# baurst/rbrt

Hardware: AMD Instinct MI355X
Metric: Mray-samples/sec (WxHxspp/s) on bunny scene; achieved HBM GB/s vs peak (higher is better)
Workload: dtype f32; 1 GPU; example_scene.yaml, 69451-triangle stand-in mesh, 1024x768, 50 spp, seed 1; parallelism=pixel tiles 8x8 dealt round-robin along skew lines over 1 GPU(s)

## Files before the change

include/rbrt_hip_debug.h:

```cpp
#ifndef RBRT_HIP_DEBUG_H
#define RBRT_HIP_DEBUG_H

#include "rbrt_hip.h"

#ifdef __cplusplus
extern "C" {
#endif

int rbrt_hip_scene_last_batching(rbrt_hip_scene_t* scene, uint32_t* samples_per_batch, uint32_t* n_batches);

int rbrt_hip_scene_adaptive_rounds(rbrt_hip_scene_t* scene, uint32_t* active_tiles, size_t n, uint32_t* n_rounds);

#define RBRT_DENOISE_TILE 16u

#define RBRT_GUIDED_TILE 16u
#define RBRT_GUIDED_STAGED_MAX_STEP 4u
int rbrt_hip_debug_guided_staging(int max_step);

#define RBRT_TEMPORAL_BLOCK 256u

#define RBRT_UPSAMPLE_TILE_W 32u
#define RBRT_UPSAMPLE_TILE_H 8u

#define RBRT_DESPIKE_TILE_W 32u
#define RBRT_DESPIKE_TILE_H 8u

#define RBRT_TONEMAP_BLOCK_PIXELS 1024u
#define RBRT_TONEMAP_MAX_BLOCKS 512u

#define RBRT_GLARE_TILE_W 16u
#define RBRT_GLARE_TILE_H 16u

int rbrt_hip_trace_rays(rbrt_hip_scene_t* scene, const float* rays, size_t n, float min_dist,
                        float max_dist, float* out_t, int32_t* out_obj, int32_t* out_tri,
                        float* out_dist);

int rbrt_hip_selftest_gate(const float lo[3], const float hi[3], const float* rays, size_t n, uint8_t* out_fast,
                           uint8_t* out_exact);

int rbrt_hip_selftest_ieee(uint64_t seed, size_t n, uint64_t counts[3]);

int rbrt_hip_debug_ieee(const float* x, size_t n, const float* v, size_t m, float* out_sqrt, uint8_t* out_sqrt_short,
                        float* out_norm, uint8_t* out_norm_short);

int rbrt_hip_selftest_sqrt_sweep(uint32_t first_bits, uint64_t n, uint64_t counts[3]);

int rbrt_hip_scene_debug_counters(rbrt_hip_scene_t* scene, uint64_t* out, size_t n);

int rbrt_hip_scene_debug_set_counter(rbrt_hip_scene_t* scene, size_t index, uint64_t value);

int rbrt_hip_bvh_build_host(const rbrt_mesh_t* mesh, void** nodes_out, size_t* n_nodes, void** tris_out,
                            size_t* n_tris, uint32_t* max_depth, float* max_e12);
void rbrt_hip_free_host(void* p);
int rbrt_hip_bvh_build_host_records(const void* records, size_t n, void** nodes_out, size_t* n_nodes, void** tris_out,
                                    size_t* n_tris, uint32_t* max_depth, float* max_e12);
int rbrt_hip_bvh_build_device(const rbrt_mesh_t* mesh, void** nodes_out, size_t* n_nodes, void** tris_out,
                              size_t* n_tris, uint32_t* max_depth, float* max_e12, int* built);

int rbrt_hip_debug_scatter(const rbrt_material_t* mats, const float* in_dir, const float* p, const float* normal,
                           const uint32_t* rng_state, size_t n, float* out_dir, uint8_t* out_ok, uint32_t* out_rng_state);

int rbrt_hip_debug_primary_cull(rbrt_hip_scene_t* scene, const rbrt_camera_t* cam, uint32_t* out_words, size_t n_words);
int rbrt_hip_debug_primary_cull_lens(rbrt_hip_scene_t* scene, const rbrt_camera_lens_t* lens, uint32_t* out_words, size_t n_words);
int rbrt_hip_debug_primary_cull_shutter(rbrt_hip_scene_t* scene, const rbrt_camera_t* cam, const rbrt_camera_lens_t* lens,
                                        const float travel[3], uint32_t* out_words, size_t n_words);
int rbrt_hip_debug_primary_cull_opts(rbrt_hip_scene_t* scene, const rbrt_camera_t* cam, const rbrt_render_opts_t* opts,
                                     uint32_t* out_words, size_t n_words);

int rbrt_hip_debug_shading_normals(rbrt_hip_scene_t* scene, const float* rays, size_t n, float min_dist, float max_dist,
                                   float* out_normal);

int rbrt_hip_debug_surface_albedo(rbrt_hip_scene_t* scene, const float* rays, size_t n, float min_dist, float max_dist,
                                  float* out_albedo);

int rbrt_hip_debug_environment(rbrt_hip_scene_t* scene, const float* dirs, size_t n, float* out_rgb);

int rbrt_hip_scene_set_timing(rbrt_hip_scene_t* scene, int enable);
int rbrt_hip_scene_kernel_ms(rbrt_hip_scene_t* scene, float* trace_ms_total, float* resolve_ms_total,
                             uint32_t* n_trace_launches);

int rbrt_hip_scene_launch_mix(rbrt_hip_scene_t* scene, uint32_t* n_full_grid, uint32_t* n_half_grid);

int rbrt_hip_scene_helper_launches(rbrt_hip_scene_t* scene, uint32_t* n);

int rbrt_hip_scene_set_short_paths(rbrt_hip_scene_t* scene, int mode);
int rbrt_hip_debug_short_masks(rbrt_hip_scene_t* scene, uint64_t* out_masks, size_t n, size_t* n_chunks);

typedef struct rbrt_hip_call_times {
    double hip_init_s;
    double upload_s;
    double bvh_build_s;
    double lanes_s;
    double create_s;
    double render_s;
    double copy_s;
    double destroy_s;
    double total_s;
    uint32_t meshes_device_built, meshes_host_built;
} rbrt_hip_call_times_t;
int rbrt_hip_scene_create_times(rbrt_hip_scene_t* scene, rbrt_hip_call_times_t* out);
int rbrt_hip_last_render_times(rbrt_hip_call_times_t* out);

int rbrt_hip_scene_refine_wait(rbrt_hip_scene_t* scene, double timeout_s, int* state, double* build_seconds);

#ifdef __cplusplus
}
#endif
#endif
```

rbrt_amd/__init__.py:

```python
from __future__ import annotations

import ctypes as C

import numpy as np

from . import abi
from .abi import (Camera, CameraLens, Material, RenderOpts, RbrtError, SceneData, MeshData, default_opts, load_hip,
                  material, MAT_DIELECTRIC, MAT_LAMBERTIAN, MAT_METAL)

__all__ = ["render_scene", "HipScene", "abi", "device_count"]


def device_count() -> int:
    return int(load_hip().rbrt_hip_device_count())


def _cam_arg(cam: abi.Camera, lens, opts: abi.RenderOpts):
    if lens is None:
        return C.byref(cam), cam
    if isinstance(lens, abi.CameraLens):
        lens = (tuple(lens.lens_u), tuple(lens.lens_v), lens.focus_scale)
    L = abi.camera_lens(cam, *lens)
    opts.flags |= abi.FLAG_THIN_LENS
    return C.byref(L.cam), L
# ... 19 lines not shown
    return rad, rgb


def _shading_ptr(scene):
    f = getattr(scene, "shading_ptr", None)
    return f() if f is not None else None


def _patterns_ptr(scene):
    f = getattr(scene, "patterns_ptr", None)
    return f() if f is not None else None


def last_render_times() -> dict:
    t = abi.CallTimes()
    abi.check(load_hip().rbrt_hip_last_render_times(C.byref(t)))
    return t.as_dict()


class HipScene:

    def __init__(self, scene: abi.SceneData, device: int = 0):
        self._lib = load_hip()
        self._h = C.c_void_p()
        self.device = device
        self.scene = scene
        shading, patterns = _shading_ptr(scene), _patterns_ptr(scene)
        if patterns is not None:
            abi.check(self._lib.rbrt_hip_scene_create_patterned(scene.ptr(), shading, patterns, device, C.byref(self._h)))
        elif shading is None:
            abi.check(self._lib.rbrt_hip_scene_create(scene.ptr(), device, C.byref(self._h)))
        else:
            abi.check(self._lib.rbrt_hip_scene_create_shaded(scene.ptr(), shading, device, C.byref(self._h)))

    def close(self):
        if self._h:
            self._lib.rbrt_hip_scene_destroy(self._h)
            self._h = C.c_void_p()

    def __del__(self):
        try:
            self.close()
        except Exception:
            pass

    def __enter__(self):
        return self

    def __exit__(self, *a):
        self.close()

    def render_device(self, cam: abi.Camera, opts: abi.RenderOpts, d_radiance: int | None, d_rgb8: int | None = None,
                      stream: int | None = None, lens=None):
        opts = _opts_copy(opts)
        cam_p, _keep = _cam_arg(cam, lens, opts)
        abi.check(self._lib.rbrt_hip_render_device(self._h, cam_p, C.byref(opts), C.c_void_p(stream or 0),
                                                   C.c_void_p(d_radiance or 0), C.c_void_p(d_rgb8 or 0)))

    def render_pass(self, cam: abi.Camera, opts: abi.RenderOpts, sample_begin: int, sample_end: int, d_accum: int,
                    d_radiance: int | None = None, d_rgb8: int | None = None, stream: int | None = None, lens=None):
        opts = _opts_copy(opts)
        cam_p, _keep = _cam_arg(cam, lens, opts)
        abi.check(self._lib.rbrt_hip_render_pass(self._h, cam_p, C.byref(opts), C.c_void_p(stream or 0), sample_begin,
                                                 sample_end, C.c_void_p(d_accum), C.c_void_p(d_radiance or 0),
                                                 C.c_void_p(d_rgb8 or 0)))

    def render_adaptive(self, cam: abi.Camera, opts: abi.RenderOpts, threshold: float, min_samples: int = 16, step: int = 64,
                        d_radiance: int | None = None, d_rgb8: int | None = None, d_tile_samples: int | None = None,
                        d_tile_error: int | None = None, stream: int | None = None, lens=None, reserved: int = 0) -> dict:
        opts = _opts_copy(opts)
        cam_p, _keep = _cam_arg(cam, lens, opts)
        a = abi.AdaptiveOpts(float(threshold), int(min_samples), int(step), int(reserved))
        res = abi.AdaptiveResult()
        abi.check(self._lib.rbrt_hip_render_adaptive(self._h, cam_p, C.byref(opts), C.byref(a), C.c_void_p(stream or 0),
                                                     C.c_void_p(d_radiance or 0), C.c_void_p(d_rgb8 or 0),
                                                     C.c_void_p(d_tile_samples or 0), C.c_void_p(d_tile_error or 0), C.byref(res)))
        return dict(rounds=int(res.rounds), samples=int(res.samples), samples_fixed=int(res.samples_fixed))

    def adaptive_rounds(self) -> list:
        n = C.c_uint32()
        abi.check(self._lib.rbrt_hip_scene_adaptive_rounds(self._h, None, 0, C.byref(n)))
        buf = (C.c_uint32 * max(n.value, 1))()
        abi.check(self._lib.rbrt_hip_scene_adaptive_rounds(self._h, buf, n.value, C.byref(n)))
        return [int(buf[i]) for i in range(n.value)]

    def denoise(self, d_radiance: int | None = None, d_rgb8: int | None = None, d_half_a: int | None = None,
                d_half_b: int | None = None, window_radius: int | None = None, patch_radius: int | None = None,
                strength: float | None = None, stream: int | None = None, reserved: int = 0):
        d = denoise_opts(window_radius, patch_radius, strength, reserved)
        abi.check(self._lib.rbrt_hip_scene_denoise(self._h, C.byref(d), C.c_void_p(stream or 0), C.c_void_p(d_radiance or 0),
                                                   C.c_void_p(d_rgb8 or 0), C.c_void_p(d_half_a or 0), C.c_void_p(d_half_b or 0)))

    def denoise_guided(self, d_albedo: int, d_normal: int, d_depth: int, d_coverage: int, d_workspace: int,
                       d_radiance: int | None = None, d_rgb8: int | None = None, opts: abi.GuidedOpts | None = None,
                       stream: int | None = None):
        g = opts if opts is not None else guided_opts()
        abi.check(self._lib.rbrt_hip_scene_denoise_guided(self._h, C.byref(g), C.c_void_p(stream or 0), C.c_void_p(d_albedo or 0),
                                                          C.c_void_p(d_normal or 0), C.c_void_p(d_depth or 0), C.c_void_p(d_coverage or 0),
                                                          C.c_void_p(d_workspace or 0), C.c_void_p(d_radiance or 0), C.c_void_p(d_rgb8 or 0)))

    def render_features(self, cam: abi.Camera, opts: abi.RenderOpts, samples: int | None = None, d_albedo: int | None = None,
                        d_normal: int | None = None, d_depth: int | None = None, d_coverage: int | None = None,
                        d_object: int | None = None, lens=None, stream: int | None = None, reserved=(0, 0, 0)):
        opts = _opts_copy(opts)
        cam_p, _keep = _cam_arg(cam, lens, opts)
        f = feature_opts(samples, reserved)
        abi.check(self._lib.rbrt_hip_render_features(self._h, cam_p, C.byref(opts), C.byref(f), C.c_void_p(stream or 0),
                                                     C.c_void_p(d_albedo or 0), C.c_void_p(d_normal or 0), C.c_void_p(d_depth or 0),
                                                     C.c_void_p(d_coverage or 0), C.c_void_p(d_object or 0)))

    def set_environment(self, nodes, *, n: int | None = None, reserved: int = 0):
        if nodes is None and n is None:
            abi.check(self._lib.rbrt_hip_scene_set_environment(self._h, None))
            return
        env = abi.Environment()
        if nodes is not None:
            nodes = np.ascontiguousarray(nodes, np.float32)
            if n is None:
                if nodes.ndim != 3 or nodes.shape[0] != nodes.shape[1] or nodes.shape[2] != 3 or nodes.shape[0] < 2:
                    raise ValueError("set_environment: nodes must have shape (N + 1, N + 1, 3)")
                n = nodes.shape[0] - 1
            env.nodes = abi.fptr(nodes)
        env.n, env.reserved = int(n), int(reserved)
        abi.check(self._lib.rbrt_hip_scene_set_environment(self._h, C.byref(env)))

    def set_shutter(self, travel, *, reserved: int = 0):
        if travel is None:
            abi.check(self._lib.rbrt_hip_scene_set_shutter(self._h, None))
            return
        sh = abi.Shutter()
        sh.travel[:] = [float(np.float32(v)) for v in travel]
        sh.reserved = int(reserved)
        abi.check(self._lib.rbrt_hip_scene_set_shutter(self._h, C.byref(sh)))

    def environment_lookup(self, dirs):
        dirs = np.ascontiguousarray(dirs, np.float32).reshape(-1, 3)
        out = np.zeros((dirs.shape[0], 3), np.float32)
        abi.check(self._lib.rbrt_hip_debug_environment(self._h, abi.fptr(dirs), dirs.shape[0], abi.fptr(out)))
        return out

    def set_pipeline(self, depth: int):
        abi.check(self._lib.rbrt_hip_scene_set_pipeline(self._h, int(depth)))

    def set_short_paths(self, mode: int = 1):
        abi.check(self._lib.rbrt_hip_scene_set_short_paths(self._h, int(mode)))

    def short_masks(self):
        n = C.c_size_t()
        abi.check(self._lib.rbrt_hip_debug_short_masks(self._h, None, 0, C.byref(n)))
        out = np.zeros(n.value, np.uint64)
        if n.value:
            abi.check(self._lib.rbrt_hip_debug_short_masks(self._h, out.ctypes.data_as(C.POINTER(C.c_uint64)), n.value, C.byref(n)))
        return out

    def set_timing(self, on: bool = True):
        abi.check(self._lib.rbrt_hip_scene_set_timing(self._h, int(on)))

    def kernel_ms(self):
        t, r, n = C.c_float(), C.c_float(), C.c_uint32()
        abi.check(self._lib.rbrt_hip_scene_kernel_ms(self._h, C.byref(t), C.byref(r), C.byref(n)))
        return t.value, r.value, n.value

    def launch_mix(self):
        a, b = C.c_uint32(), C.c_uint32()
        abi.check(self._lib.rbrt_hip_scene_launch_mix(self._h, C.byref(a), C.byref(b)))
        return a.value, b.value

    def helper_launches(self) -> int:
        n = C.c_uint32()
        abi.check(self._lib.rbrt_hip_scene_helper_launches(self._h, C.byref(n)))
        return n.value

    def create_times(self) -> dict:
        t = abi.CallTimes()
        abi.check(self._lib.rbrt_hip_scene_create_times(self._h, C.byref(t)))
        return t.as_dict()

    def refine_wait(self, timeout_s: float = 60.0):
        st, sec = C.c_int(), C.c_double()
        abi.check(self._lib.rbrt_hip_scene_refine_wait(self._h, float(timeout_s), C.byref(st), C.byref(sec)))
        return st.value, sec.value

    def info(self) -> dict:
        i = abi.SceneInfo()
        abi.check(self._lib.rbrt_hip_scene_info(self._h, C.byref(i)))
        return {k: int(getattr(i, k)) for k, _ in abi.SceneInfo._fields_}

    def check(self):
        abi.check(self._lib.rbrt_hip_scene_check(self._h))

    def last_batches(self):
        b, n = C.c_uint32(), C.c_uint32()
        abi.check(self._lib.rbrt_hip_scene_last_batching(self._h, C.byref(b), C.byref(n)))
        return b.value, n.value

    def stats(self) -> dict:
        st = abi.Stats()
        abi.check(self._lib.rbrt_hip_scene_stats(self._h, C.byref(st)))
        return {k: int(getattr(st, k)) for k, _ in abi.Stats._fields_}

    def set_debug_counter(self, index: int, value: int):
        abi.check(self._lib.rbrt_hip_scene_debug_set_counter(self._h, int(index), int(value)))

    def raw_debug_counters(self) -> list:
        buf = (C.c_uint64 * 64)()
        abi.check(self._lib.rbrt_hip_scene_debug_counters(self._h, buf, 64))
        return [int(x) for x in buf]

    def debug_counters(self) -> dict:
        buf = (C.c_uint64 * 64)()
        abi.check(self._lib.rbrt_hip_scene_debug_counters(self._h, buf, 64))
        names = ("empty", "trav", "term", "lamb", "metal", "diel")
        d = {f"passes_{n}": int(buf[i]) for i, n in enumerate(names)}
        d.update({f"slots_{n}": int(buf[6 + i]) for i, n in enumerate(names)})
        d.update(trav_wave_steps=int(buf[12]), trav_lane_steps=int(buf[13]), refill_rounds=int(buf[14]),
                 sched_rounds=int(buf[15]), cycles_trav=int(buf[16]), cycles_shade=int(buf[17]),
                 cycles_total=int(buf[18]), leaf_rounds=int(buf[19]), leaf_lanes=int(buf[20]),
                 walk_rounds=int(buf[21]), walk_lanes=int(buf[22]), shading_pass_free_lanes=int(buf[23]),
                 rt_first_start=int(buf[24]), rt_last_workout=int(buf[25]), rt_last_end=int(buf[26]),
                 rt_sum_wave_time=int(buf[27]), rt_first_workout=int(buf[28]),
                 path_len_hist=[int(buf[32 + i]) for i in range(8)],
                 long_path_objects=[int(buf[40 + i]) for i in range(8)],
                 long_path_total=int(buf[48]), long_path_dielectric=int(buf[47]), shade_extra_rounds=int(buf[29]),
                 drain_slowest=dict(us=int(buf[50]) >> 44, rounds=(int(buf[50]) >> 32) & 0xFFF,
                                    trav_steps=(int(buf[50]) >> 16) & 0xFFFF, passes=int(buf[50]) & 0xFFFF),
                 drain_sum=dict(rounds=int(buf[51]), trav_steps=int(buf[52]), passes=int(buf[53]),
                                lane_steps=int(buf[54])),
                 stack_pushes_beyond_lds=int(buf[30]), stack_deepest=int(buf[31]),
                 parked_at_burst_entry=int(buf[55]), fullest_shading_kind_at_burst_entry=int(buf[56]),
                 shared_entries_given=int(buf[59]), share_rounds=int(buf[60]), traversals_ending_at_root=int(buf[61]),
                 sphere_tail_runs=int(buf[62]), sphere_tail_lanes=int(buf[63]),
                 mixed_pass_8=dict(passes=int(buf[49]) >> 32, lanes=int(buf[49]) & 0xFFFFFFFF),
                 mixed_pass_16=dict(passes=int(buf[58]) >> 32, lanes=int(buf[58]) & 0xFFFFFFFF))
        return d

    def primary_cull(self, cam, opts=None, lens=None):
        tx, ty = (cam.img_width_pix + 7) // 8, (cam.img_height_pix + 7) // 8
        out = np.zeros(tx * ty, np.uint32)
        words = out.ctypes.data_as(C.POINTER(C.c_uint32))
        if opts is None and lens is None:
            abi.check(self._lib.rbrt_hip_debug_primary_cull(self._h, C.byref(cam), words, out.size))
        else:
            opts = _opts_copy(opts if opts is not None else abi.default_opts())
            cam_p, _keep = _cam_arg(cam, lens, opts)
            abi.check(self._lib.rbrt_hip_debug_primary_cull_opts(self._h, cam_p, C.byref(opts), words, out.size))
        return out.reshape(ty, tx)

    def primary_cull_lens(self, cam, lens):
        if not isinstance(lens, abi.CameraLens):
            lens = abi.camera_lens(cam, *lens)
        else:
            lens = abi.camera_lens(cam, tuple(lens.lens_u), tuple(lens.lens_v), lens.focus_scale)
        tx, ty = (cam.img_width_pix + 7) // 8, (cam.img_height_pix + 7) // 8
        out = np.zeros(tx * ty, np.uint32)
        abi.check(self._lib.rbrt_hip_debug_primary_cull_lens(self._h, C.byref(lens), out.ctypes.data_as(C.POINTER(C.c_uint32)),
                                                             out.size))
        return out.reshape(ty, tx)

    def primary_cull_shutter(self, cam, lens, travel):
        if lens is not None:
            if not isinstance(lens, abi.CameraLens):
                lens = abi.camera_lens(cam, *lens)
            else:
                lens = abi.camera_lens(cam, tuple(lens.lens_u), tuple(lens.lens_v), lens.focus_scale)
        tv = (C.c_float * 3)(*[float(np.float32(v)) for v in travel])
        tx, ty = (cam.img_width_pix + 7) // 8, (cam.img_height_pix + 7) // 8
        out = np.zeros(tx * ty, np.uint32)
        abi.check(self._lib.rbrt_hip_debug_primary_cull_shutter(self._h, C.byref(cam), C.byref(lens) if lens is not None else None, tv,
                                                                out.ctypes.data_as(C.POINTER(C.c_uint32)), out.size))
        return out.reshape(ty, tx)

    def surface_albedo(self, rays, min_dist=0.001, max_dist=2000.0):
        rays = np.ascontiguousarray(rays, np.float32).reshape(-1, 6)
        out = np.zeros((rays.shape[0], 3), np.float32)
        abi.check(self._lib.rbrt_hip_debug_surface_albedo(self._h, rays.ctypes.data_as(abi.f32p), rays.shape[0], min_dist,
                                                          max_dist, out.ctypes.data_as(abi.f32p)))
        return out

    def shading_normals(self, rays, min_dist=0.001, max_dist=2000.0):
        rays = np.ascontiguousarray(rays, np.float32).reshape(-1, 6)
        out = np.zeros((rays.shape[0], 3), np.float32)
        abi.check(self._lib.rbrt_hip_debug_shading_normals(self._h, rays.ctypes.data_as(abi.f32p), rays.shape[0], min_dist,
                                                           max_dist, out.ctypes.data_as(abi.f32p)))
        return out

    def trace_rays(self, rays, min_dist=0.001, max_dist=2000.0):
        rays = np.ascontiguousarray(rays, np.float32).reshape(-1, 6)
        n = rays.shape[0]
        t = np.zeros(n, np.float32)
        dist = np.zeros(n, np.float32)
        obj = np.zeros(n, np.int32)
        tri = np.zeros(n, np.int32)
        abi.check(self._lib.rbrt_hip_trace_rays(self._h, rays.ctypes.data_as(abi.f32p), n, min_dist, max_dist,
                                                t.ctypes.data_as(abi.f32p), obj.ctypes.data_as(abi.i32p),
                                                tri.ctypes.data_as(abi.i32p), dist.ctypes.data_as(abi.f32p)))
        return t, obj, tri, dist


def _opts_copy(opts: abi.RenderOpts) -> abi.RenderOpts:
    o = abi.RenderOpts()
    C.memmove(C.byref(o), C.byref(opts), C.sizeof(o))
    return o


def supported_flags() -> int:
    return int(load_hip().rbrt_hip_supported_flags())
# ... 249 lines not shown
```

rbrt_amd/abi.py:

```python
from __future__ import annotations

import ctypes as C
import os
from pathlib import Path

import numpy as np

ROOT = Path(__file__).resolve().parent.parent
LIB_HIP = ROOT / "rbrt_amd" / "lib" / "librbrt_hip.so"
LIB_HOST = ROOT / "rbrt_amd" / "lib" / "librbrt_host.so"

RBRT_OK = 0
RBRT_ERR_INVALID_ARG = -1
RBRT_ERR_NO_DEVICE = -2
RBRT_ERR_HIP = -3
RBRT_ERR_OOM = -4
RBRT_ERR_UNSUPPORTED = -5
RBRT_ERR_NAN = -6

MAT_LAMBERTIAN = 0
MAT_METAL = 1
MAT_DIELECTRIC = 2
MAT_EMISSIVE = 3

# ... 100 lines not shown
    _fields_ = [
        ("position", C.c_float * 3),
        ("right", C.c_float * 3),
        ("up", C.c_float * 3),
        ("img_center_point", C.c_float * 3),
        ("mm_per_pix_hor", C.c_float),
        ("mm_per_pix_vert", C.c_float),
        ("img_width_pix", C.c_uint32),
        ("img_height_pix", C.c_uint32),
    ]


class CameraLens(C.Structure):
    _fields_ = [
        ("cam", Camera),
        ("lens_u", C.c_float * 3),
        ("lens_v", C.c_float * 3),
        ("focus_scale", C.c_float),
        ("reserved", C.c_uint32),
    ]


def camera_lens(cam: Camera, lens_u, lens_v, focus_scale: float) -> CameraLens:
    L = CameraLens()
    C.memmove(C.byref(L.cam), C.byref(cam), C.sizeof(Camera))
    L.lens_u = _f3(lens_u)
    L.lens_v = _f3(lens_v)
    L.focus_scale = float(focus_scale)
    L.reserved = 0
    return L


class RenderOpts(C.Structure):
    _fields_ = [
        ("spp", C.c_uint32),
        ("max_depth", C.c_uint32),
        ("min_dist", C.c_float),
        ("max_dist", C.c_float),
        ("bg", C.c_float * 3),
        ("seed", C.c_uint64),
        ("tile_rank", C.c_uint32),
        ("tile_world", C.c_uint32),
        ("flags", C.c_uint32),
        ("reserved", C.c_uint32),
    ]


class AdaptiveOpts(C.Structure):
    _fields_ = [("threshold", C.c_float), ("min_samples", C.c_uint32), ("step", C.c_uint32), ("reserved", C.c_uint32)]


class AdaptiveResult(C.Structure):
    _fields_ = [("rounds", C.c_uint32), ("reserved", C.c_uint32), ("samples", C.c_uint64), ("samples_fixed", C.c_uint64)]


class DenoiseOpts(C.Structure):
    _fields_ = [("window_radius", C.c_uint32), ("patch_radius", C.c_uint32), ("strength", C.c_float), ("reserved", C.c_uint32)]


class TonemapOpts(C.Structure):
    _fields_ = [("curve", C.c_uint32), ("exposure", C.c_float), ("key", C.c_float), ("key_permille", C.c_uint32),
                ("white", C.c_float), ("white_permille", C.c_uint32), ("reserved", C.c_uint32 * 2)]


class TonemapResult(C.Structure):
    _fields_ = [("exposure", C.c_float), ("white", C.c_float), ("l_key", C.c_float), ("l_white", C.c_float),
                ("counted", C.c_uint32), ("reserved", C.c_uint32), ("pixels", C.c_uint64)]


class GlareOpts(C.Structure):
    _fields_ = [("threshold", C.c_float), ("intensity", C.c_float), ("levels", C.c_uint32), ("spread", C.c_float),
                ("reserved", C.c_uint32 * 4)]


class FeatureOpts(C.Structure):
    _fields_ = [("samples", C.c_uint32), ("reserved", C.c_uint32 * 3)]


class GuidedOpts(C.Structure):
    _fields_ = [("levels", C.c_uint32), ("colour", C.c_float), ("normal", C.c_float), ("depth", C.c_float), ("albedo", C.c_float),
                ("flags", C.c_uint32), ("reserved", C.c_uint32 * 2)]


class TemporalOpts(C.Structure):
    _fields_ = [("max_history", C.c_float), ("depth", C.c_float), ("normal", C.c_float), ("flags", C.c_uint32),
                ("reserved", C.c_uint32 * 4)]


class UpsampleOpts(C.Structure):
    _fields_ = [("factor", C.c_uint32), ("normal", C.c_float), ("depth", C.c_float), ("albedo", C.c_float), ("flags", C.c_uint32),
                ("reserved", C.c_uint32 * 3)]


class DespikeOpts(C.Structure):
    _fields_ = [("radius", C.c_uint32), ("rank", C.c_uint32), ("threshold", C.c_float), ("floor", C.c_float), ("flags", C.c_uint32),
                ("reserved", C.c_uint32 * 3)]


class DespikeResult(C.Structure):
    _fields_ = [("spikes_a", C.c_uint32), ("spikes_b", C.c_uint32), ("reserved", C.c_uint32 * 2)]


class CompareOpts(C.Structure):
    _fields_ = [("epsilon", C.c_float), ("flags", C.c_uint32), ("reserved", C.c_uint32 * 2)]


class CompareResult(C.Structure):
    _fields_ = [("sum_se", C.c_double), ("sum_ae", C.c_double), ("sum_rel", C.c_double), ("sum_ssim", C.c_double), ("max_abs", C.c_float),
                ("usable", C.c_uint32), ("skipped", C.c_uint32), ("reserved", C.c_uint32 * 5)]


class CompareSummary(C.Structure):
    _fields_ = [("mse", C.c_double), ("mae", C.c_double), ("relmse", C.c_double), ("psnr_db", C.c_double), ("ssim", C.c_double)]


class Environment(C.Structure):
    _fields_ = [("n", C.c_uint32), ("reserved", C.c_uint32), ("nodes", f32p)]


class Shutter(C.Structure):
    _fields_ = [("travel", C.c_float * 3), ("reserved", C.c_uint32)]


class Stats(C.Structure):
    _fields_ = [
        ("rays", C.c_uint64),
        ("mesh_gate_pass", C.c_uint64),
        ("nodes_visited", C.c_uint64),
        ("tris_tested", C.c_uint64),
        ("mesh_hits", C.c_uint64),
        ("samples", C.c_uint64),
        ("nan_discriminants", C.c_uint64),
        ("node_bytes", C.c_uint32),
        ("tri_bytes", C.c_uint32),
    ]


class SceneInfo(C.Structure):
    _fields_ = [
        ("n_spheres", C.c_uint32), ("n_meshes", C.c_uint32),
        ("n_meshes_device_built", C.c_uint32), ("bvh_stack_need", C.c_uint32),
        ("n_nodes", C.c_uint64), ("n_triangles", C.c_uint64),
        ("trace_waves", C.c_uint32), ("lds_bytes_per_wave", C.c_uint32),
        ("occupancy_api_waves_per_cu", C.c_uint32), ("n_cus", C.c_uint32),
    ]


class CallTimes(C.Structure):
    _fields_ = [(k, C.c_double) for k in ("hip_init_s", "upload_s", "bvh_build_s", "lanes_s", "create_s", "render_s", "copy_s",
                                          "destroy_s", "total_s")] + [("meshes_device_built", C.c_uint32), ("meshes_host_built", C.c_uint32)]

    def as_dict(self) -> dict:
        return {k: getattr(self, k) for k, _ in self._fields_}


HIP_SYMBOLS = {
    "rbrt_hip_render": (C.c_int, [C.POINTER(Camera), C.POINTER(Scene), C.POINTER(RenderOpts), f32p, u8p]),
    "rbrt_hip_scene_create": (C.c_int, [C.POINTER(Scene), C.c_int, C.POINTER(C.c_void_p)]),
    "rbrt_hip_scene_destroy": (C.c_int, [C.c_void_p]),
    "rbrt_hip_packed_pixels": (C.c_size_t, [C.c_uint32, C.c_uint32, C.c_uint32, C.c_uint32]),
    "rbrt_hip_tile_xy": (None, [C.c_uint32, C.c_uint32, C.POINTER(C.c_uint32), C.POINTER(C.c_uint32)]),
    "rbrt_hip_tile_number": (C.c_uint32, [C.c_uint32, C.c_uint32, C.c_uint32]),
    "rbrt_hip_render_device": (C.c_int, [C.c_void_p, C.POINTER(Camera), C.POINTER(RenderOpts), C.c_void_p,
                                         C.c_void_p, C.c_void_p]),
    "rbrt_hip_render_pass": (C.c_int, [C.c_void_p, C.POINTER(Camera), C.POINTER(RenderOpts), C.c_void_p, C.c_uint32, C.c_uint32,
                                       C.c_void_p, C.c_void_p, C.c_void_p]),
    "rbrt_hip_unpack_tiles": (C.c_int, [C.c_int, C.c_void_p, C.c_void_p, C.c_uint32, C.c_uint32, C.c_uint32,
                                        C.c_void_p, C.c_void_p]),
    "rbrt_hip_unpack_tiles_strided": (C.c_int, [C.c_int, C.c_void_p, C.c_void_p, C.c_uint32, C.c_uint32, C.c_uint32,
                                                C.c_size_t, C.c_void_p, C.c_void_p]),
    "rbrt_hip_scene_stats": (C.c_int, [C.c_void_p, C.POINTER(Stats)]),
    "rbrt_hip_scene_check": (C.c_int, [C.c_void_p]),
    "rbrt_render_opts_default": (None, [C.POINTER(RenderOpts)]),
    "rbrt_hip_device_count": (C.c_int, []),
    "rbrt_hip_last_error": (C.c_char_p, []),
    "rbrt_hip_abi_version": (C.c_int, []),
    "rbrt_hip_scene_set_pipeline": (C.c_int, [C.c_void_p, C.c_uint32]),
    "rbrt_hip_scene_info": (C.c_int, [C.c_void_p, C.POINTER(SceneInfo)]),
    "rbrt_hip_supported_flags": (C.c_uint32, []),
    "rbrt_hip_scene_create_shaded": (C.c_int, [C.POINTER(Scene), C.POINTER(SceneShading), C.c_int, C.POINTER(C.c_void_p)]),
    "rbrt_hip_scene_create_patterned": (C.c_int, [C.POINTER(Scene), C.POINTER(SceneShading), C.POINTER(ScenePatterns), C.c_int,
                                                  C.POINTER(C.c_void_p)]),
    "rbrt_hip_render_patterned": (C.c_int, [C.POINTER(Camera), C.POINTER(Scene), C.POINTER(SceneShading), C.POINTER(ScenePatterns),
                                            C.POINTER(RenderOpts), f32p, u8p]),
    "rbrt_hip_render_shaded": (C.c_int, [C.POINTER(Camera), C.POINTER(Scene), C.POINTER(SceneShading), C.POINTER(RenderOpts),
                                         f32p, u8p]),
    "rbrt_hip_render_adaptive": (C.c_int, [C.c_void_p, C.POINTER(Camera), C.POINTER(RenderOpts), C.POINTER(AdaptiveOpts), C.c_void_p,
                                           C.c_void_p, C.c_void_p, C.c_void_p, C.c_void_p, C.POINTER(AdaptiveResult)]),
    "rbrt_denoise_opts_default": (None, [C.POINTER(DenoiseOpts)]),
    "rbrt_hip_denoise_halves": (C.c_int, [C.c_int, C.c_void_p, C.c_void_p, C.c_void_p, C.c_void_p, C.c_uint32, C.c_uint32,
                                          C.POINTER(DenoiseOpts), C.c_void_p, C.c_void_p]),
    "rbrt_tonemap_opts_default": (None, [C.POINTER(TonemapOpts)]),
    "rbrt_hip_tonemap": (C.c_int, [C.c_int, C.c_void_p, C.c_void_p, C.c_size_t, C.POINTER(TonemapOpts), C.c_void_p, C.c_void_p,
                                   C.c_void_p]),
    "rbrt_glare_opts_default": (None, [C.POINTER(GlareOpts)]),
    "rbrt_hip_glare_workspace_bytes": (C.c_size_t, [C.c_uint32, C.c_uint32, C.c_uint32]),
    "rbrt_hip_glare": (C.c_int, [C.c_int, C.c_void_p, C.c_void_p, C.c_uint32, C.c_uint32, C.POINTER(GlareOpts), C.c_void_p, C.c_void_p,
                                 C.c_void_p]),
    "rbrt_hip_scene_denoise": (C.c_int, [C.c_void_p, C.POINTER(DenoiseOpts), C.c_void_p, C.c_void_p, C.c_void_p, C.c_void_p, C.c_void_p]),
    "rbrt_hip_scene_set_environment": (C.c_int, [C.c_void_p, C.POINTER(Environment)]),
    "rbrt_hip_scene_set_shutter": (C.c_int, [C.c_void_p, C.POINTER(Shutter)]),
    "rbrt_feature_opts_default": (None, [C.POINTER(FeatureOpts)]),
    "rbrt_hip_render_features": (C.c_int, [C.c_void_p, C.POINTER(Camera), C.POINTER(RenderOpts), C.POINTER(FeatureOpts), C.c_void_p,
                                           C.c_void_p, C.c_void_p, C.c_void_p, C.c_void_p, C.c_void_p]),
    "rbrt_guided_opts_default": (None, [C.POINTER(GuidedOpts)]),
    "rbrt_hip_guided_workspace_bytes": (C.c_size_t, [C.c_uint32, C.c_uint32]),
    "rbrt_hip_denoise_guided": (C.c_int, [C.c_int, C.c_void_p, C.c_void_p, C.c_void_p, C.c_void_p, C.c_void_p, C.c_void_p, C.c_void_p,
                                          C.c_void_p, C.c_uint32, C.c_uint32, C.POINTER(GuidedOpts), C.c_void_p, C.c_void_p, C.c_void_p]),
    "rbrt_hip_scene_denoise_guided": (C.c_int, [C.c_void_p, C.POINTER(GuidedOpts), C.c_void_p, C.c_void_p, C.c_void_p, C.c_void_p,
                                                C.c_void_p, C.c_void_p, C.c_void_p, C.c_void_p]),
    "rbrt_temporal_opts_default": (None, [C.POINTER(TemporalOpts)]),
    "rbrt_hip_temporal_history_bytes": (C.c_size_t, [C.c_uint32, C.c_uint32]),
    "rbrt_hip_temporal_accumulate": (C.c_int, [C.c_int, C.c_void_p, C.c_void_p, C.c_void_p, C.c_void_p, C.c_void_p, C.c_void_p,
                                               C.POINTER(Camera), C.POINTER(Camera), C.POINTER(TemporalOpts), C.c_void_p, C.c_void_p,
                                               C.c_void_p, C.c_void_p, C.c_void_p]),
    "rbrt_upsample_opts_default": (None, [C.POINTER(UpsampleOpts)]),
    "rbrt_hip_upsample_camera": (C.c_int, [C.POINTER(Camera), C.c_uint32, C.POINTER(Camera)]),
    "rbrt_hip_upsample_workspace_bytes": (C.c_size_t, [C.c_uint32, C.c_uint32, C.c_uint32]),
    "rbrt_hip_upsample_halves": (C.c_int, [C.c_int, C.c_void_p, C.c_void_p, C.c_void_p, C.c_void_p, C.c_void_p, C.c_void_p, C.c_void_p,
                                           C.c_void_p, C.c_uint32, C.c_uint32, C.POINTER(UpsampleOpts), C.c_void_p, C.c_void_p, C.c_void_p,
                                           C.c_void_p]),
    "rbrt_despike_opts_default": (None, [C.POINTER(DespikeOpts)]),
    "rbrt_hip_despike_halves": (C.c_int, [C.c_int, C.c_void_p, C.c_void_p, C.c_void_p, C.c_uint32, C.c_uint32, C.POINTER(DespikeOpts), C.c_void_p,
                                          C.c_void_p, C.c_void_p, C.c_void_p]),
    "rbrt_compare_opts_default": (None, [C.POINTER(CompareOpts)]),
    "rbrt_hip_compare_workspace_bytes": (C.c_size_t, [C.c_uint32, C.c_uint32]),
    "rbrt_hip_compare_images": (C.c_int, [C.c_int, C.c_void_p, C.c_void_p, C.c_void_p, C.c_uint32, C.c_uint32, C.POINTER(CompareOpts), C.c_void_p,
                                          C.c_void_p, C.c_void_p, C.c_void_p]),
    "rbrt_compare_summary": (None, [C.POINTER(CompareResult), C.c_uint32, C.c_uint32, C.c_double, C.POINTER(CompareSummary)]),
}
DEBUG_SYMBOLS = {
    "rbrt_hip_debug_guided_staging": (C.c_int, [C.c_int]),
    "rbrt_hip_scene_last_batching": (C.c_int, [C.c_void_p, C.POINTER(C.c_uint32), C.POINTER(C.c_uint32)]),
    "rbrt_hip_trace_rays": (C.c_int, [C.c_void_p, f32p, C.c_size_t, C.c_float, C.c_float, f32p, i32p, i32p, f32p]),
    "rbrt_hip_selftest_ieee": (C.c_int, [C.c_uint64, C.c_size_t, C.POINTER(C.c_uint64)]),
    "rbrt_hip_debug_ieee": (C.c_int, [f32p, C.c_size_t, f32p, C.c_size_t, f32p, u8p, f32p, u8p]),
    "rbrt_hip_selftest_sqrt_sweep": (C.c_int, [C.c_uint32, C.c_uint64, C.POINTER(C.c_uint64)]),
    "rbrt_hip_selftest_gate": (C.c_int, [f32p, f32p, f32p, C.c_size_t, u8p, u8p]),
    "rbrt_hip_bvh_build_host": (C.c_int, [C.POINTER(Mesh), C.POINTER(C.c_void_p), C.POINTER(C.c_size_t),
                                          C.POINTER(C.c_void_p), C.POINTER(C.c_size_t), C.POINTER(C.c_uint32),
                                          f32p]),
    "rbrt_hip_free_host": (None, [C.c_void_p]),
    "rbrt_hip_bvh_build_host_records": (C.c_int, [C.c_void_p, C.c_size_t, C.POINTER(C.c_void_p), C.POINTER(C.c_size_t),
                                                  C.POINTER(C.c_void_p), C.POINTER(C.c_size_t), C.POINTER(C.c_uint32), f32p]),
    "rbrt_hip_bvh_build_device": (C.c_int, [C.POINTER(Mesh), C.POINTER(C.c_void_p), C.POINTER(C.c_size_t),
                                            C.POINTER(C.c_void_p), C.POINTER(C.c_size_t), C.POINTER(C.c_uint32),
                                            f32p, C.POINTER(C.c_int)]),
    "rbrt_hip_scene_debug_counters": (C.c_int, [C.c_void_p, C.POINTER(C.c_uint64), C.c_size_t]),
    "rbrt_hip_scene_set_timing": (C.c_int, [C.c_void_p, C.c_int]),
    "rbrt_hip_scene_kernel_ms": (C.c_int, [C.c_void_p, f32p, f32p, C.POINTER(C.c_uint32)]),
    "rbrt_hip_scene_debug_set_counter": (C.c_int, [C.c_void_p, C.c_size_t, C.c_uint64]),
    "rbrt_hip_scene_launch_mix": (C.c_int, [C.c_void_p, C.POINTER(C.c_uint32), C.POINTER(C.c_uint32)]),
    "rbrt_hip_debug_scatter": (C.c_int, [C.POINTER(Material), f32p, f32p, f32p, C.POINTER(C.c_uint32), C.c_size_t, f32p, u8p,
                                        C.POINTER(C.c_uint32)]),
    "rbrt_hip_debug_primary_cull": (C.c_int, [C.c_void_p, C.POINTER(Camera), C.POINTER(C.c_uint32), C.c_size_t]),
    "rbrt_hip_debug_primary_cull_lens": (C.c_int, [C.c_void_p, C.POINTER(CameraLens), C.POINTER(C.c_uint32), C.c_size_t]),
    "rbrt_hip_debug_primary_cull_shutter": (C.c_int, [C.c_void_p, C.POINTER(Camera), C.POINTER(CameraLens), C.POINTER(C.c_float),
                                                      C.POINTER(C.c_uint32), C.c_size_t]),
    "rbrt_hip_debug_primary_cull_opts": (C.c_int, [C.c_void_p, C.POINTER(Camera), C.POINTER(RenderOpts), C.POINTER(C.c_uint32), C.c_size_t]),
    "rbrt_hip_scene_helper_launches": (C.c_int, [C.c_void_p, C.POINTER(C.c_uint32)]),
    "rbrt_hip_scene_create_times": (C.c_int, [C.c_void_p, C.POINTER(CallTimes)]),
    "rbrt_hip_last_render_times": (C.c_int, [C.POINTER(CallTimes)]),
    "rbrt_hip_scene_refine_wait": (C.c_int, [C.c_void_p, C.c_double, C.POINTER(C.c_int), C.POINTER(C.c_double)]),
    "rbrt_hip_debug_shading_normals": (C.c_int, [C.c_void_p, f32p, C.c_size_t, C.c_float, C.c_float, f32p]),
    "rbrt_hip_debug_surface_albedo": (C.c_int, [C.c_void_p, f32p, C.c_size_t, C.c_float, C.c_float, f32p]),
    "rbrt_hip_scene_adaptive_rounds": (C.c_int, [C.c_void_p, C.POINTER(C.c_uint32), C.c_size_t, C.POINTER(C.c_uint32)]),
    "rbrt_hip_debug_environment": (C.c_int, [C.c_void_p, f32p, C.c_size_t, f32p]),
    "rbrt_hip_scene_set_short_paths": (C.c_int, [C.c_void_p, C.c_int]),
    "rbrt_hip_debug_short_masks": (C.c_int, [C.c_void_p, C.POINTER(C.c_uint64), C.c_size_t, C.POINTER(C.c_size_t)]),
}


class RbrtError(RuntimeError):
    def __init__(self, code: int, msg: str):
        super().__init__(f"rbrt_hip error {code}: {msg}")
        self.code = code


_hip = None


def _preload_torch_hip_runtime() -> None:
    if os.environ.get("RBRT_NO_TORCH_PRELOAD"):
        return
    try:
        import importlib.util
        spec = importlib.util.find_spec("torch")
        if spec is None or not spec.origin:
            return
        cand = Path(spec.origin).parent / "lib" / "libamdhip64.so"
        if cand.exists():
            C.CDLL(str(cand), mode=getattr(os, "RTLD_GLOBAL", 0x100) | getattr(os, "RTLD_NOW", 2))
    except OSError:
        pass


def load_hip() -> C.CDLL:
    global _hip
    if _hip is not None:
        return _hip
    lib_path = Path(os.environ.get("RBRT_HIP_LIB", LIB_HIP))
    if not lib_path.exists():
        raise FileNotFoundError(
            f"{lib_path} is missing: build it with `make` (or __graft_entry__.build()). "
            "rbrt_amd has no CPU or pure-Python render path.")
    _preload_torch_hip_runtime()
    lib = C.CDLL(str(lib_path), mode=getattr(os, "RTLD_NOW", 2))
    for name, (res, args) in {**HIP_SYMBOLS, **DEBUG_SYMBOLS}.items():
        fn = getattr(lib, name)
        fn.restype = res
        fn.argtypes = args
    _hip = lib
    return lib


def check(code: int) -> None:
    if code != RBRT_OK:
        raise RbrtError(code, load_hip().rbrt_hip_last_error().decode(errors="replace"))



def _f3(v):
    return (C.c_float * 3)(*[float(x) for x in v])


def material(kind: int, albedo=(0.0, 0.0, 0.0), param: float = 0.0) -> Material:
    return Material(kind, _f3(albedo), float(param))


def fptr(a: np.ndarray):
    assert a.dtype == np.float32 and a.flags["C_CONTIGUOUS"]
    return a.ctypes.data_as(f32p)


class SceneData:

    def __init__(self, spheres=(), meshes=(), triangles=(), element_order=None, patterns=None):
        self.spheres = list(spheres)
        self.meshes = list(meshes)
        self.triangles = list(triangles)
        self.element_order = None if element_order is None else [int(x) for x in element_order]
        self._sph = (Sphere * max(1, len(self.spheres)))()
        for i, (c, r, m) in enumerate(self.spheres):
            self._sph[i] = Sphere(_f3(c), float(r), m)
        self._msh = (Mesh * max(1, len(self.meshes)))()
        for i, md in enumerate(self.meshes):
            self._msh[i] = md.struct
        self._tri = (Triangle * max(1, len(self.triangles)))()
        for i, (corners, m) in enumerate(self.triangles):
            for a in range(3):
                for b in range(3):
                    self._tri[i].corners[a][b] = float(corners[a][b])
            self._tri[i].mat = m
        self._order = None if self.element_order is None else (C.c_uint32 * len(self.element_order))(*self.element_order)
        self.struct = Scene(len(self.spheres), self._sph, len(self.meshes), self._msh, len(self.triangles), self._tri,
                            self._order if self._order is not None else C.POINTER(C.c_uint32)())
        self._nrm = (MeshNormals * max(1, len(self.meshes)))()
        for i, md in enumerate(self.meshes):
            if md.normals is not None:
                self._nrm[i] = md.normals_struct
        self.shading = (SceneShading(len(self.meshes), 0, self._nrm)
                        if any(md.normals is not None for md in self.meshes) else None)
        self.pattern_of = dict(patterns or {})
        n_obj = len(self.spheres) + len(self.triangles) + len(self.meshes)
        self._pat = (Pattern * max(1, n_obj))()
        for k, p in self.pattern_of.items():
            self._pat[int(k)] = p
        self.patterns = ScenePatterns(n_obj, 0, self._pat) if self.pattern_of else None

    def ptr(self):
        return C.byref(self.struct)

    def shading_ptr(self):
        return None if self.shading is None else C.byref(self.shading)

    def patterns_ptr(self):
        return None if self.patterns is None else C.byref(self.patterns)


class MeshData:

    FIELDS = ("v0x", "v0y", "v0z", "e1x", "e1y", "e1z", "e2x", "e2y", "e2z", "nx", "ny", "nz")

    def __init__(self, arrays: dict, is_padding: np.ndarray, n_real: int, bbox_lo, bbox_hi, mat: Material, normals=None):
        self.arrays = {k: np.ascontiguousarray(arrays[k], dtype=np.float32) for k in self.FIELDS}
        self.is_padding = np.ascontiguousarray(is_padding, dtype=np.uint8)
        n_total = len(self.is_padding)
        for k in self.FIELDS:
            assert len(self.arrays[k]) == n_total, k
        self.n_total, self.n_real = n_total, int(n_real)
        self.bbox_lo, self.bbox_hi = np.float32(bbox_lo), np.float32(bbox_hi)
        self.struct = Mesh()
        self.struct.n_total = n_total
        self.struct.n_real = self.n_real
        for k in self.FIELDS:
            setattr(self.struct, k, fptr(self.arrays[k]))
        self.struct.is_padding = self.is_padding.ctypes.data_as(u8p)
        self.struct.bbox_lo = _f3(bbox_lo)
        self.struct.bbox_hi = _f3(bbox_hi)
        self.struct.mat = mat
        self.normals = None
        self.normals_struct = MeshNormals()
        if normals is not None:
            self.normals = {k: np.ascontiguousarray(normals[k], dtype=np.float32) for k in NORMAL_FIELDS}
            for k in NORMAL_FIELDS:
                assert len(self.normals[k]) == n_total, k
                setattr(self.normals_struct, k, fptr(self.normals[k]))

    def with_normals(self, normals):
        return MeshData(self.arrays, self.is_padding, self.n_real, self.bbox_lo, self.bbox_hi, self.struct.mat, normals)


def default_opts(spp: int = 5, seed: int = 1, **kw) -> RenderOpts:
    o = RenderOpts()
    o.spp, o.max_depth, o.min_dist, o.max_dist = spp, 50, 0.001, 2000.0
    o.bg = _f3((0.05, 0.05, 0.8))
    o.seed, o.tile_rank, o.tile_world, o.flags, o.reserved = seed, 0, 1, 0, 0
    for k, v in kw.items():
        if k == "bg":
            o.bg = _f3(v)
        else:
            setattr(o, k, v)
# ... 202 lines not shown
```

rbrt_amd/csrc/api.cpp:

```cpp
#include <hip/hip_runtime_api.h>

#include <algorithm>
#include <chrono>
#include <cmath>
#include <cstdio>
#include <cstdlib>
#include <cstring>
#include <atomic>
#include <condition_variable>
#include <limits>
#include <memory>
#include <mutex>
#include <string>
#include <thread>
#include <vector>

#include "api_common.h"
#include "bvh.h"
#include "bvh_device.h"
#include "device_types.h"
#include "../../include/rbrt_hip_debug.h"

namespace rbrt {
hipError_t launch_trace_megakernel(const TraceParams& P, uint32_t n_waves, bool stats, hipStream_t stream);
hipError_t launch_trace_helper(const TraceParams& P, uint32_t n_waves, hipStream_t stream);
size_t megakernel_gseq_bytes(uint32_t n_waves);
size_t megakernel_gstack_bytes(uint32_t n_waves);
size_t megakernel_lds_bytes(uint32_t stack_entries, uint32_t n_spheres, uint32_t n_meshes, uint32_t n_elem_tris, uint32_t thin_lens,
                            uint32_t environment, uint32_t pattern_dw, uint32_t shutter);
int megakernel_occupancy_per_cu(size_t lds_bytes);
hipError_t launch_primary_cull(const TraceParams& P, hipStream_t stream);
hipError_t launch_sky_resolve(const TraceParams& P, const ResolveParams& R, hipStream_t stream);
hipError_t launch_short_paths(const TraceParams& P, uint32_t n_waves, hipStream_t stream);
hipError_t launch_code_load(hipStream_t stream);
hipError_t launch_resolve(const ResolveParams& R, hipStream_t stream);
hipError_t launch_resolve_even(const TraceParams& P, const ResolveParams& R, uint32_t n_active_tiles, hipStream_t stream);
hipError_t launch_adaptive_lists(const AdaptiveParams& A, hipStream_t stream);
hipError_t launch_tile_error(const AdaptiveParams& A, uint32_t n_active_tiles, hipStream_t stream);
hipError_t launch_adaptive_finish(const AdaptiveParams& A, hipStream_t stream);
hipError_t launch_denoise_halves(const DenoiseHalvesParams& Q, hipStream_t stream);
hipError_t launch_unpack(const float* gathered, uint32_t width, uint32_t height, uint32_t world,
                         size_t rank_stride_pixels, float* out_radiance, uint8_t* out_rgb8, hipStream_t stream);
hipError_t launch_trace_rays(const TraceParams& P, const float* rays, size_t n, float* out_t, int32_t* out_obj,
                             int32_t* out_tri, float* out_dist, hipStream_t stream);
hipError_t launch_shading_normals(const TraceParams& P, const float* rays, size_t n, float* out_normal, hipStream_t stream);
hipError_t launch_surface_albedo(const TraceParams& P, const float* rays, size_t n, float* out_albedo, hipStream_t stream);
hipError_t launch_environment_lookup(const EnvTexel* nodes, uint32_t n_env, const float* dirs, size_t n, float* out_rgb, hipStream_t stream);
hipError_t launch_features(const TraceParams& P, const FeatureParams& F, hipStream_t stream);
hipError_t launch_scatter_debug(const DevMaterial* d_mats, const float* d_in_dir, const float* d_p, const float* d_normal,
                                 const uint32_t* d_rng, size_t n, float* d_out_dir, uint8_t* d_out_ok, uint32_t* d_out_rng);
uint64_t host_splitmix64(uint64_t x);
}

using namespace rbrt;

namespace {
thread_local std::string g_last_error;
}

namespace rbrt {

int fail(int code, const std::string& msg) {
    g_last_error = msg;
    return code;
}

int hip_fail(hipError_t e, const std::string& what) {
    const int code = (e == hipErrorOutOfMemory) ? RBRT_ERR_OOM
                     : (e == hipErrorNoDevice || e == hipErrorInvalidDevice) ? RBRT_ERR_NO_DEVICE
                                                                             : RBRT_ERR_HIP;
    return fail(code, what + ": " + hipGetErrorString(e));
}

int hook_result(hipError_t e, const char* who) {
    return e == hipSuccess ? RBRT_OK : fail(RBRT_ERR_HIP, std::string(who) + ": " + hipGetErrorString(e));
}

int ensure_device(int device) {
    int n = 0;
    hipError_t e = hipGetDeviceCount(&n);
    if (e != hipSuccess || n <= 0)
        return fail(RBRT_ERR_NO_DEVICE, std::string("no HIP device available: ") +
                                            (e != hipSuccess ? hipGetErrorString(e) : "device count is 0"));
    if (device < 0 || device >= n) return fail(RBRT_ERR_INVALID_ARG, "device index out of range");
    HIP_TRY(hipSetDevice(device));
    return RBRT_OK;
}

}

namespace {

thread_local rbrt_hip_call_times_t g_last_render_times{};

const uint32_t g_hw_queues_at_load = [] {
    if (const char* q = std::getenv("GPU_MAX_HW_QUEUES")) {
        char* end = nullptr;
        const long v = std::strtol(q, &end, 10);
        if (end != q && *end == '\0' && v >= 1 && v <= 64) return uint32_t(v);
    }
    return 4u;
}();

double now_s() { return std::chrono::duration<double>(std::chrono::steady_clock::now().time_since_epoch()).count(); }

uint32_t local_tiles_of(uint32_t n_tiles, uint32_t rank, uint32_t world) {
    return rank < n_tiles ? (n_tiles - rank + world - 1u) / world : 0u;
}

const char* lab_env(const char* name) {
    const char* lab = std::getenv("RBRT_HIP_LAB");
    return (lab && lab[0] == '1') ? std::getenv(name) : nullptr;
}
bool lab_u32(const char* name, long long lo, long long hi, uint32_t& dst, std::string& err) {
    const char* e = lab_env(name);
    if (!e) return true;
    char* end = nullptr;
    const long long v = std::strtoll(e, &end, 10);
    if (end == e || *end != '\0' || v < lo || v > hi) {
        err = std::string("lab knob ") + name + "=" + e + " is not valid (see include/rbrt_hip_debug.h)";
        return false;
    }
    dst = uint32_t(v);
    return true;
}
bool lab_f32(const char* name, float lo, bool lo_open, float hi, float& dst, std::string& err) {
    const char* e = lab_env(name);
    if (!e) return true;
    char* end = nullptr;
    const float v = std::strtof(e, &end);
    if (end == e || *end != '\0' || !std::isfinite(v) || v < lo || (lo_open && v == lo) || v > hi) {
        err = std::string("lab knob ") + name + "=" + e + " is not valid (see include/rbrt_hip_debug.h)";
        return false;
    }
    dst = v;
    return true;
}

struct BvhKnobs {
    BvhBuildOptions host;
    int device_algo = 0;
    uint32_t ploc_radius = kPlocRadius;
};
bool lab_bvh_knobs(BvhKnobs& k, std::string& err) {
    if (!lab_f32("RBRT_BVH_CT", 0.0f, true, 1000.0f, k.host.cost_traverse, err) ||
        !lab_f32("RBRT_BVH_SPATIAL", 0.0f, false, kSpatialBudget, k.host.spatial_budget, err) ||
        !lab_u32("RBRT_PLOC_RADIUS", 1, 256, k.ploc_radius, err))
        return false;
    if (const char* a = lab_env("RBRT_BVH_DEVICE_ALGO")) {
        if (!std::strcmp(a, "ploc") || !std::strcmp(a, "lbvh")) {
            k.device_algo = a[0] == 'l' ? 1 : 0;
        } else {
            err = std::string("lab knob RBRT_BVH_DEVICE_ALGO=") + a + " is not valid (see include/rbrt_hip_debug.h)";
            return false;
        }
    }
    return true;
}

size_t workspace_cap_bytes() {
    size_t mb = 1024;
    if (const char* e = std::getenv("RBRT_HIP_WORKSPACE_MB")) {
        long v = std::atol(e);
        if (v > 0) mb = size_t(v);
    }
    return mb << 20;
}

void rebase_leaf_links(std::vector<BvhNode4>& nodes, uint32_t tri_base) {
    if (tri_base == 0) return;
    for (BvhNode4& nd : nodes)
        for (int c = 0; c < 4; ++c)
            if (nd.child[c] < 0 && nd.child[c] != kNoChild) {
                const uint32_t leaf = uint32_t(~nd.child[c]);
                nd.child[c] = ~int32_t((((leaf >> kLeafBits) + tri_base) << kLeafBits) | (leaf & uint32_t(kLeafMax - 1)));
            }
}

int copy_out(const BvhBuildResult& r, const char* who, void** nodes_out, size_t* n_nodes, void** tris_out, size_t* n_tris,
             uint32_t* max_depth, float* max_e12) {
    *n_nodes = r.nodes.size(), *n_tris = r.tris.size();
    *nodes_out = std::malloc(std::max<size_t>(1, r.nodes.size() * sizeof(BvhNode4)));
    *tris_out = std::malloc(std::max<size_t>(1, r.tris.size() * sizeof(BvhTri)));
    if (!*nodes_out || !*tris_out) {
        std::free(*nodes_out), std::free(*tris_out);
        *nodes_out = *tris_out = nullptr;
        return fail(RBRT_ERR_OOM, std::string(who) + ": malloc failed");
    }
    std::memcpy(*nodes_out, r.nodes.data(), r.nodes.size() * sizeof(BvhNode4));
    std::memcpy(*tris_out, r.tris.data(), r.tris.size() * sizeof(BvhTri));
    if (max_depth) *max_depth = r.max_depth;
    if (max_e12) *max_e12 = r.max_e12;
    return RBRT_OK;
}

void set_tree(DevMesh& dm, const BvhNode4* d_nodes, float max_e12, size_t n_nodes, size_t n_tris) {
    dm.nodes = d_nodes, dm.max_e12 = max_e12, dm.n_nodes = uint32_t(n_nodes), dm.n_tris = uint32_t(n_tris);
}

}

constexpr uint32_t kStripesAuto = 0xFFFFFFFFu;

struct rbrt_hip_scene {
    int device = 0;
    uint32_t n_spheres = 0, n_meshes = 0, n_elem_tris = 0;
    uint32_t n_patterns = 0;
    std::vector<void*> allocs;
    char* slab_cur = nullptr;
    size_t slab_left = 0;
    DevSphere* d_spheres = nullptr;
    DevTriangle* d_elem_tris = nullptr;
    uint32_t* d_elems = nullptr;
    DevMaterial* d_materials = nullptr;
    DevMesh* d_meshes = nullptr;
    BvhTri* d_tris = nullptr;
    DevCounters* d_counters = nullptr;
    EnvTexel* d_env = nullptr;
    uint32_t env_n = 0;
    bool has_shutter = false;
    float travel[3] = {0.0f, 0.0f, 0.0f};
    struct Lane {
        hipStream_t stream = nullptr;
        int stream_pool_key = -1;
        struct Buf {
            float* d_sample_buf = nullptr;
            size_t sample_buf_bytes = 0;
            unsigned long long* d_work_counter = nullptr;
            unsigned long long* d_short_masks = nullptr;
            hipEvent_t ev_resolved = nullptr;
            bool in_use = false;
        } bufs[1];
        uint32_t* d_gseq = nullptr;
        uint32_t* d_gstack = nullptr;
        struct TileKey {
            rbrt_camera_t cam;
            uint32_t rank, world;
            uint32_t list_mode;
            float min_dist;
            uint32_t thin_lens;
            float lens_u[3], lens_v[3], focus_scale;
            uint32_t shutter;
            float travel[3];
        };
        struct TileSet {
            uint32_t* d_cull = nullptr;
            uint32_t* d_lists = nullptr;
            hipEvent_t ev_lists = nullptr;
            hipEvent_t ev_free = nullptr;
            bool free_recorded = false;
            bool key_valid = false;
            TileKey key;
            uint64_t last_used = 0;
        } tiles[2];
        size_t tile_cull_words = 0, tile_lists_words = 0;
        hipEvent_t ev_traced = nullptr;
        bool in_use = false;
        uint32_t* d_helper_words = nullptr;
        uint32_t seq = 0;
        hipEvent_t ev_helper = nullptr;
        hipEvent_t ev_carried = nullptr;
        bool helper_carried = false;
        bool helper_pending = false;
        hipEvent_t ev_ready = nullptr;
        struct Open {
            bool valid = false;
            TraceParams P;
            uint32_t grid = 0, helper_waves = 0, rounds = 0;
            uint64_t seq = 0;
        } open;
    };
    std::vector<Lane> lanes;
    std::mutex mu;
    std::condition_variable cv;
    std::thread watcher;
    bool watcher_stop = false;
    double last_call_s = 0.0;
    uint64_t open_seq = 0;
    uint32_t helpers_mode = 1;
    uint32_t n_helper_launches = 0;
    uint32_t helper_min_items = 4096;
    uint32_t helper_min_free_per_cu = 1;
    uint32_t helper_min_launch_mi = 16;
    uint32_t helper_rounds = 4;
    hipStream_t prep_stream = nullptr;
    bool one_shot = false;
    hipStream_t aux_stream = nullptr;
    void* h_zeros = nullptr;
    uint64_t launch_no = 0;
    bool streaming_hint = false;
    uint32_t pipeline = 0;
    uint32_t scratch_waves = 0;
    uint32_t n_cus = 256;
    uint32_t hw_queues = 4;
    bool waves_fixed = false;
    uint32_t overlap_waves_per_cu = 0;
    uint32_t next_lane = 0;
    float* d_acc = nullptr;
    size_t acc_bytes = 0;
    struct Adaptive {
        float *d_sum = nullptr, *d_sum_even = nullptr;
        size_t sum_floats = 0;
        uint32_t *d_cull = nullptr, *d_lists = nullptr, *d_active = nullptr, *d_tile_samples = nullptr, *d_n_active = nullptr;
        float* d_tile_error = nullptr;
        size_t cull_words = 0, local_tiles = 0;
        hipEvent_t ev_lists = nullptr;
        std::vector<uint32_t> round_active;
        struct Last {
            bool any = false, complete = false;
            uint32_t width = 0, height = 0, world = 1, spp = 0, tiles_x = 0;
        } last;
        float *d_half_a = nullptr, *d_half_b = nullptr, *d_wa = nullptr;
        size_t half_pixels = 0;
    } adaptive;
    bool poison_samples = false;
    struct Bound {
        float lo[3], hi[3];
    };
    std::vector<Bound> h_bounds;
    uint32_t stack_need = 1;
    uint32_t n_waves = 0;
    uint32_t stack_entries = kLdsStack;
    uint32_t y_low_water = 28;
    uint32_t y_high_water = 28, y_high_min_parked = 16;
    uint32_t leaf_round = 6;
    uint32_t leaf_leaves = 16;
    uint32_t share_idle = 4;
    uint32_t work_stripes = 16;
    uint32_t work_stripes_overlap = kStripesAuto;
    bool trace_launches = false;
    bool trace_create = false;
    uint32_t tile_tail_div = 8;
    uint32_t primary_cull = 1;
    uint32_t short_paths = 1;
    struct LastShort {
        const unsigned long long* d_masks = nullptr;
        const uint32_t* d_lists = nullptr;
        uint32_t batch = 0;
    } last_short;
    uint32_t shade_rounds = 1;
    uint32_t shade_cont_min = 8;
    rbrt_hip_stats_t stats{};
    bool stats_pending = false;
    bool timing = false;
    std::vector<hipEvent_t> events;
    size_t events_used = 0;
    bool timing_overflow = false;
    uint32_t last_batch = 0, last_n_batches = 0;
    uint32_t n_full_grid = 0, n_half_grid = 0;
    uint64_t total_nodes = 0, total_tris = 0;
    uint32_t n_device_built = 0;
    rbrt_hip_call_times_t create_times{};
    std::unique_ptr<struct Refine> refine;
    uint32_t n_refined = 0;
};

struct Refine {
    std::thread th;
    std::atomic<int> state{0};
    std::atomic<bool> cancel{false};
    int device = 0;
    const BvhTri* d_tris = nullptr;
    size_t tri_total = 0;
    std::vector<DevMesh> meshes;
    std::vector<uint32_t> tri_base, n_valid;
    std::vector<uint8_t> wanted;
    unsigned max_threads = 0;
    BvhBuildOptions shape;
    std::vector<void*> allocs;
    BvhTri* d_tris_new = nullptr;
    DevMesh* d_meshes_new = nullptr;
    uint32_t stack_need = 1, n_done = 0;
    uint64_t nodes_delta_plus = 0, nodes_delta_minus = 0;
    double seconds = 0.0;
    std::string error;

    void run() {
        const double t0 = now_s();
        hipStream_t st = nullptr;
        std::vector<BvhTri> h;
        const auto finish = [&](const std::string& why) {
            if (st) (void)hipStreamDestroy(st);
            if (!why.empty()) {
                for (void* p : allocs) (void)hipFree(p);
                allocs.clear();
                error = why;
            }
            seconds = now_s() - t0;
            state.store(why.empty() ? 1 : 2, std::memory_order_release);
        };
        const auto hip = [&](hipError_t e, const char* what) -> bool {
            if (e == hipSuccess) return true;
            finish(std::string(what) + ": " + hipGetErrorString(e));
            return false;
        };
        if (!hip(hipSetDevice(device), "hipSetDevice")) return;
        if (!hip(hipStreamCreateWithFlags(&st, hipStreamNonBlocking), "hipStreamCreate")) return;
        h.resize(tri_total);
        if (!hip(hipMemcpyAsync(h.data(), d_tris, tri_total * sizeof(BvhTri), hipMemcpyDeviceToHost, st), "read-back of the records")) return;
        if (!hip(hipStreamSynchronize(st), "read-back of the records")) return;
        std::vector<BvhBuildResult> built(meshes.size());
        BvhBuildOptions opt = shape;
        opt.max_threads = max_threads, opt.cancel = &cancel;
        for (size_t i = 0; i < meshes.size(); ++i) {
            if (!wanted[i]) continue;
            built[i] = build_bvh_from_records(h.data() + tri_base[i], n_valid[i], opt);
            if (built[i].cancelled || cancel.load()) return finish("cancelled");
            BvhBuildResult& b = built[i];
            const size_t cap = size_t(i + 1 < meshes.size() ? tri_base[i + 1] : uint32_t(tri_total)) - tri_base[i];
            if (b.tris.size() > cap || b.nodes.empty()) return finish("the host builder's tree does not fit the mesh's records");
            rebase_leaf_links(b.nodes, tri_base[i]);
            void* p = nullptr;
            if (!hip(hipMalloc(&p, b.nodes.size() * sizeof(BvhNode4)), "hipMalloc(nodes)")) return;
            allocs.push_back(p);
            if (!hip(hipMemcpyAsync(p, b.nodes.data(), b.nodes.size() * sizeof(BvhNode4), hipMemcpyHostToDevice, st), "upload of the nodes")) return;
            std::copy(b.tris.begin(), b.tris.end(), h.begin() + tri_base[i]);
            nodes_delta_minus += meshes[i].n_nodes, nodes_delta_plus += b.nodes.size();
            set_tree(meshes[i], static_cast<const BvhNode4*>(p), b.max_e12, b.nodes.size(), b.tris.size());
            stack_need = std::max(stack_need, b.stack_need);
            ++n_done;
        }
        void* p = nullptr;
        if (!hip(hipMalloc(&p, std::max<size_t>(tri_total * sizeof(BvhTri), 64)), "hipMalloc(records)")) return;
        allocs.push_back(p);
        d_tris_new = static_cast<BvhTri*>(p);
        if (!hip(hipMemcpyAsync(p, h.data(), tri_total * sizeof(BvhTri), hipMemcpyHostToDevice, st), "upload of the records")) return;
        for (DevMesh& dm : meshes) dm.tris = d_tris_new;
        if (!hip(hipMalloc(&p, std::max<size_t>(meshes.size() * sizeof(DevMesh), 16)), "hipMalloc(mesh table)")) return;
        allocs.push_back(p);
        d_meshes_new = static_cast<DevMesh*>(p);
        if (!hip(hipMemcpyAsync(p, meshes.data(), meshes.size() * sizeof(DevMesh), hipMemcpyHostToDevice, st), "upload of the mesh table")) return;
        if (!hip(hipStreamSynchronize(st), "upload of the refined trees")) return;
        finish("");
    }
};

namespace {

constexpr size_t kSlabBytes = 32u << 20, kSlabMaxPiece = 8u << 20, kSlabAlign = 512;
hipError_t dev_alloc(rbrt_hip_scene* s, size_t bytes, void** out, bool own_piece = false) {
    bytes = (std::max<size_t>(bytes, 1) + kSlabAlign - 1) & ~(kSlabAlign - 1);
    *out = nullptr;
    if (bytes > kSlabMaxPiece || own_piece) {
        const hipError_t e = hipMalloc(out, bytes);
        if (e == hipSuccess) s->allocs.push_back(*out);
        return e;
    }
    if (bytes > s->slab_left) {
        void* p = nullptr;
        const hipError_t e = hipMalloc(&p, kSlabBytes);
        if (e != hipSuccess) return e;
        s->allocs.push_back(p);
        s->slab_cur = static_cast<char*>(p), s->slab_left = kSlabBytes;
    }
    *out = s->slab_cur;
    s->slab_cur += bytes, s->slab_left -= bytes;
    return hipSuccess;
}

hipError_t dev_release(rbrt_hip_scene* s, void* p) {
    const auto it = std::find(s->allocs.begin(), s->allocs.end(), p);
    if (it == s->allocs.end()) return hipErrorInvalidValue;
    s->allocs.erase(it);
    return hipFree(p);
}

template <class T>
int upload(rbrt_hip_scene* s, const std::vector<T>& host, T** out) {
    void* d = nullptr;
    size_t bytes = std::max<size_t>(host.size() * sizeof(T), 16);
    HIP_TRY(dev_alloc(s, bytes, &d));
    if (!host.empty()) HIP_TRY(hipMemcpy(d, host.data(), host.size() * sizeof(T), hipMemcpyHostToDevice));
    *out = static_cast<T*>(d);
    return RBRT_OK;
}

hipError_t device_build_mesh(const rbrt_mesh_t& m, BvhTri* d_tris_out, uint32_t tri_base, Normal4* d_normals, DeviceBvhResult* r,
                             const BvhKnobs& knobs, double* upload_s = nullptr) {
    const double t_up0 = now_s();
    const float* src[12] = {m.v0x, m.v0y, m.v0z, m.e1x, m.e1y, m.e1z, m.e2x, m.e2y, m.e2z, m.nx, m.ny, m.nz};
    DevBuf<float> soa_buf;
    DevBuf<uint8_t> pad_buf;
    const size_t stride = (size_t(m.n_total) + 63u) & ~size_t(63);
    hipError_t e = soa_buf.alloc(stride * 12u);
    if (e == hipSuccess) e = pad_buf.alloc(m.n_total);
    float* const d_soa = soa_buf.get();
    uint8_t* const d_pad = pad_buf.get();
// ... 875 lines not shown
    if (s->h_zeros) (void)hipHostFree(s->h_zeros);
    if (s->adaptive.ev_lists) (void)hipEventDestroy(s->adaptive.ev_lists);
    const double td4 = now_s();
    for (void* p : s->allocs) (void)hipFree(p);
    if (s->d_acc) (void)hipFree(s->d_acc);
    const double td5 = now_s();
    for (hipEvent_t e : s->events) (void)hipEventDestroy(e);
    if (trace_destroy)
        std::fprintf(stderr, "[rbrt_hip] scene_destroy: sync %.3f ms, lanes %.3f (sample buffers %.3f), streams %.3f, pinned %.3f, %zu allocations %.3f, %zu events %.3f\n",
                     (td1 - td0) * 1e3, (td2 - td1) * 1e3, t_big * 1e3, (td3 - td2) * 1e3, (td4 - td3) * 1e3, s->allocs.size(), (td5 - td4) * 1e3,
                     s->events.size(), (now_s() - td5) * 1e3);
    delete s;
    return RBRT_OK;
}

int rbrt_hip_scene_set_timing(rbrt_hip_scene_t* s, int enable) {
    if (!s) return fail(RBRT_ERR_INVALID_ARG, "null scene");
    std::lock_guard<std::mutex> watcher_lock(s->mu);
    s->timing = enable != 0;
    s->timing_overflow = false;
    s->events_used = 0;
    s->n_full_grid = s->n_half_grid = 0;
    s->n_helper_launches = 0;
    return RBRT_OK;
}

int rbrt_hip_scene_launch_mix(rbrt_hip_scene_t* s, uint32_t* n_full_grid, uint32_t* n_half_grid) {
    if (!s) return fail(RBRT_ERR_INVALID_ARG, "null scene");
    if (n_full_grid) *n_full_grid = s->n_full_grid;
    if (n_half_grid) *n_half_grid = s->n_half_grid;
    return RBRT_OK;
}

int rbrt_hip_scene_helper_launches(rbrt_hip_scene_t* s, uint32_t* n) {
    if (!s || !n) return fail(RBRT_ERR_INVALID_ARG, "helper_launches: null argument");
    std::lock_guard<std::mutex> watcher_lock(s->mu);
    *n = s->n_helper_launches;
    return RBRT_OK;
}

int rbrt_hip_scene_kernel_ms(rbrt_hip_scene_t* s, float* trace_ms, float* resolve_ms, uint32_t* n_launches) {
    if (!s) return fail(RBRT_ERR_INVALID_ARG, "null scene");
    if (!s->timing) return fail(RBRT_ERR_INVALID_ARG, "timing is not enabled on this scene");
    HIP_TRY(hipSetDevice(s->device));
    float tsum = 0.0f, rsum = 0.0f;
    uint32_t n = 0;
    for (size_t b = 0; b + 3 <= s->events_used; b += 3) {
        HIP_TRY(hipEventSynchronize(s->events[b + 2]));
        float t = 0.0f, r = 0.0f;
        HIP_TRY(hipEventElapsedTime(&t, s->events[b], s->events[b + 1]));
        HIP_TRY(hipEventElapsedTime(&r, s->events[b + 1], s->events[b + 2]));
        tsum += t;
        rsum += r;
        ++n;
    }
    if (trace_ms) *trace_ms = tsum;
    if (resolve_ms) *resolve_ms = rsum;
    if (n_launches) *n_launches = n;
    return RBRT_OK;
}

namespace {

struct CallPlan {
    hipStream_t stream = nullptr;
    uint32_t s_begin = 0, s_end = 0, world = 1, tiles_x = 0, tiles_y = 0, n_tiles = 0, n_local = 0, depth = 1;
    size_t npix = 0, per_sample = 0, batch = 0, need = 0, n_batches = 0;
    bool stats = false, busy_at_call = false, streams_now = false, tile_pass = false, timing = false;
    const struct AdaptiveRound* round = nullptr;
};

struct AdaptiveRound {
    uint32_t* d_cull;
    uint32_t* d_lists;
    float* d_sum_even;
    uint32_t n_active;
    hipEvent_t ev_lists;
};

bool plan_call(const rbrt_hip_scene* s, const rbrt_camera_t* cam, const rbrt_render_opts_t* o, CallPlan& c) {
    c.world = o->tile_world ? o->tile_world : 1;
    c.tiles_x = (cam->img_width_pix + RBRT_TILE - 1) / RBRT_TILE, c.tiles_y = (cam->img_height_pix + RBRT_TILE - 1) / RBRT_TILE;
    c.n_tiles = c.tiles_x * c.tiles_y, c.n_local = local_tiles_of(c.n_tiles, o->tile_rank, c.world);
    c.npix = size_t(c.n_local) * 64u;
    if (c.npix == 0) return false;
    c.per_sample = c.npix * 3u * sizeof(float);
    c.batch = workspace_cap_bytes() / c.per_sample;
    if (c.batch * c.npix > 0xFFF00000ull) c.batch = 0xFFF00000ull / c.npix;
    if (c.batch < 1) c.batch = 1;
    if (c.batch > c.s_end - c.s_begin) c.batch = c.s_end - c.s_begin;
    c.need = c.batch * c.per_sample, c.n_batches = (size_t(c.s_end - c.s_begin) + c.batch - 1) / c.batch;
    c.stats = (o->flags & RBRT_FLAG_COLLECT_STATS) != 0;
    const uint32_t depth_full = depth_for(s, c.need);
    c.busy_at_call = other_launch_in_flight(s, nullptr);
    c.streams_now = !c.stats && depth_full > 1 && (s->streaming_hint || c.busy_at_call);
    c.depth = c.streams_now ? depth_full : std::min<uint32_t>(depth_full, uint32_t(std::max<size_t>(s->lanes.size(), 1)));
    c.tile_pass = s->primary_cull != 0;
    return true;
}

int sync_lanes(rbrt_hip_scene* s, hipStream_t stream) {
    HIP_TRY(hipStreamSynchronize(stream));
    for (auto& L : s->lanes) HIP_TRY(hipStreamSynchronize(L.stream));
    if (s->aux_stream) HIP_TRY(hipStreamSynchronize(s->aux_stream));
    return RBRT_OK;
}

int prepare_call(rbrt_hip_scene* s, CallPlan& c, const float* acc) {
    const hipStream_t stream = c.stream;
    const size_t per_sample = c.per_sample;
    if (!acc && c.batch < c.s_end - c.s_begin && per_sample > s->acc_bytes) {
        if (s->d_acc) {
            if (int rc = sync_lanes(s, stream)) return rc;
            HIP_TRY(hipFree(s->d_acc));
            s->d_acc = nullptr, s->acc_bytes = 0;
        }
        void* p = nullptr;
        HIP_TRY(hipMalloc(&p, per_sample));
        s->d_acc = static_cast<float*>(p), s->acc_bytes = per_sample;
    }
    if (c.stats) {
        HIP_TRY(hipMemsetAsync(s->d_counters, 0, sizeof(DevCounters), stream));
        const unsigned long long ones = ~0ull;
        HIP_TRY(hipMemcpyAsync(&s->d_counters->diag[24], &ones, sizeof(ones), hipMemcpyHostToDevice, stream));
        HIP_TRY(hipMemcpyAsync(&s->d_counters->diag[28], &ones, sizeof(ones), hipMemcpyHostToDevice, stream));
        s->stats_pending = true;
    }
    s->last_batch = uint32_t(c.batch), s->last_n_batches = uint32_t(c.n_batches);
    if (s->timing && s->events_used + 3 * c.n_batches > kMaxTimedLaunches * 3) s->timing_overflow = true;
    c.timing = s->timing && !s->timing_overflow;
    while (c.timing && s->events.size() < s->events_used + 3 * c.n_batches) {
        hipEvent_t e;
        HIP_TRY(hipEventCreate(&e));
        s->events.push_back(e);
    }
    return RBRT_OK;
}

TraceParams call_params(const rbrt_hip_scene* s, const rbrt_camera_t* cam, const rbrt_render_opts_t* o, const CallPlan& c) {
    TraceParams P;
    fill_trace_params(s, cam, o, P);
    P.tiles_x = c.tiles_x, P.tiles_y = c.tiles_y, P.n_tiles = c.n_tiles, P.tiles_x_magic = div_magic_of(c.tiles_x);
    P.tiles_reversed = empty_end_is_first(s, *cam, c.tiles_x, o->tile_rank, c.world, c.n_local) ? 1u : 0u;
    P.tile_rank = o->tile_rank, P.tile_world = c.world, P.n_local_tiles = c.n_local, P.tile_tail_div = s->tile_tail_div;
    P.stack_entries = s->stack_entries, P.share_idle = s->share_idle;
    P.y_low_water = s->y_low_water, P.y_high_min_parked = s->y_high_min_parked;
    P.y_high_water = s->y_high_water < s->y_low_water ? s->y_low_water : s->y_high_water;
    P.leaf_round = s->leaf_round, P.leaf_leaves = s->leaf_leaves;
    P.work_stripes = s->work_stripes;
    P.shade_rounds = s->shade_rounds, P.shade_cont_min = s->shade_cont_min;
    return P;
}

int size_lane(rbrt_hip_scene* s, const CallPlan& c, uint32_t li) {
    rbrt_hip_scene::Lane& L = s->lanes[li];
    const size_t need = c.need, n_tiles = c.n_tiles, lists_need = size_t(kTileListHeader) + 2u * size_t(c.n_local);
    if (!L.d_gseq) {
        void* p = nullptr;
        const size_t gseq_bytes = (megakernel_gseq_bytes(s->scratch_waves) + kSlabAlign - 1) & ~(kSlabAlign - 1);
        HIP_TRY(dev_alloc(s, gseq_bytes + megakernel_gstack_bytes(s->scratch_waves), &p));
        L.d_gseq = static_cast<uint32_t*>(p);
        L.d_gstack = reinterpret_cast<uint32_t*>(static_cast<char*>(p) + gseq_bytes);
    }
    for (auto& B : L.bufs) {
        if (need <= B.sample_buf_bytes) continue;
        if (B.d_sample_buf) {
            if (int rc = sync_lanes(s, c.stream)) return rc;
            HIP_TRY(hipFree(B.d_sample_buf));
            if (s->last_short.d_masks == B.d_short_masks) s->last_short = {};
            B.d_sample_buf = nullptr, B.sample_buf_bytes = 0, B.d_short_masks = nullptr;
        }
        void* p = nullptr;
        const size_t chunk_bytes = 64u * 3u * sizeof(float);
        HIP_TRY(hipMalloc(&p, need + need / chunk_bytes * sizeof(unsigned long long)));
        B.d_sample_buf = static_cast<float*>(p), B.sample_buf_bytes = need;
        B.d_short_masks = reinterpret_cast<unsigned long long*>(static_cast<char*>(p) + need);
    }
    if (c.tile_pass && !c.round && (n_tiles > L.tile_cull_words || lists_need > L.tile_lists_words)) {
        if (L.tiles[0].d_cull || L.tiles[0].d_lists) {
            if (int rc = sync_lanes(s, c.stream)) return rc;
            if (s->prep_stream) HIP_TRY(hipStreamSynchronize(s->prep_stream));
        }
        for (auto& T : L.tiles) {
            T.d_cull = T.d_lists = nullptr;
            T.key_valid = false, T.free_recorded = false;
            void* p = nullptr;
            HIP_TRY(dev_alloc(s, size_t(n_tiles) * sizeof(uint32_t), &p));
            T.d_cull = static_cast<uint32_t*>(p);
            HIP_TRY(dev_alloc(s, lists_need * sizeof(uint32_t), &p));
            T.d_lists = static_cast<uint32_t*>(p);
            if (!T.ev_lists) HIP_TRY(hipEventCreateWithFlags(&T.ev_lists, hipEventDisableTiming));
            if (!T.ev_free) HIP_TRY(hipEventCreateWithFlags(&T.ev_free, hipEventDisableTiming));
        }
        L.tile_cull_words = n_tiles, L.tile_lists_words = lists_need;
    }
    return RBRT_OK;
}

int ensure_prep_stream(rbrt_hip_scene* s) {
    if (s->prep_stream) return RBRT_OK;
    int prio_low = 0, prio_high = 0;
    (void)hipDeviceGetStreamPriorityRange(&prio_low, &prio_high);
    HIP_TRY(hipStreamCreateWithPriority(&s->prep_stream, hipStreamNonBlocking, prio_high));
    return RBRT_OK;
}

rbrt_hip_scene::Lane::TileKey tile_key(const TraceParams& P, uint32_t list_mode) {
    rbrt_hip_scene::Lane::TileKey k;
    std::memset(&k, 0, sizeof(k));
    k.cam = P.cam, k.rank = P.tile_rank, k.world = P.tile_world, k.list_mode = list_mode, k.min_dist = P.min_dist;
    k.thin_lens = P.thin_lens, k.focus_scale = P.focus_scale;
    for (int c = 0; c < 3; ++c) k.lens_u[c] = P.lens_u[c], k.lens_v[c] = P.lens_v[c];
    k.shutter = P.shutter;
    for (int c = 0; c < 3; ++c) k.travel[c] = P.travel[c];
    return k;
}

rbrt_hip_scene::Lane::TileSet* find_tile_set(rbrt_hip_scene::Lane& L, const rbrt_hip_scene::Lane::TileKey& k) {
    rbrt_hip_scene::Lane::TileSet* S = nullptr;
    for (auto& C : L.tiles)
        if (C.key_valid && std::memcmp(&k, &C.key, sizeof(k)) == 0) S = &C;
    return S;
}

int fill_tile_set(rbrt_hip_scene::Lane::TileSet* S, const TraceParams& base, uint32_t list_mode, bool wide, hipStream_t cs) {
    if (S->free_recorded) HIP_TRY(hipStreamWaitEvent(cs, S->ev_free, 0));
    if (S->key_valid) HIP_TRY(hipStreamWaitEvent(cs, S->ev_lists, 0));
    TraceParams P = base;
    P.tile_cull = S->d_cull, P.tile_lists = S->d_lists, P.tile_list_mode = list_mode, P.tile_lists_wide = wide ? 1u : 0u;
    HIP_TRY(launch_primary_cull(P, cs));
    HIP_TRY(hipEventRecord(S->ev_lists, cs));
    S->key = tile_key(P, list_mode), S->key_valid = true;
    return RBRT_OK;
}

int warm_tile_tables(rbrt_hip_scene* s, const CallPlan& c, const TraceParams& P) {
    const uint32_t mode = list_mode_for(true), iso_mode = list_mode_for(false);
    for (uint32_t li = 0; li < c.depth; ++li) {
        rbrt_hip_scene::Lane& L = s->lanes[li];
        if (L.tiles[0].key_valid || L.tiles[1].key_valid) continue;
        if (int rc = fill_tile_set(&L.tiles[0], P, mode, false, c.stream)) return rc;
        if (li == s->next_lane % c.depth && iso_mode != mode)
            if (int rc = fill_tile_set(&L.tiles[1], P, iso_mode, false, c.stream)) return rc;
    }
    return RBRT_OK;
}

int issue_batches(rbrt_hip_scene* s, const CallPlan& c, const rbrt_render_opts_t* o, const TraceParams& P_call, ResolveParams R) {
    const hipStream_t stream = c.stream;
    const bool stats = c.stats, piped = c.depth > 1 && !stats;
    const size_t ev0 = s->events_used;
    bool call_streams = false;
    uint32_t prev_lane = ~0u;
    for (size_t b = 0; b < c.n_batches; ++b) {
        const uint32_t base = c.s_begin + uint32_t(b * c.batch);
        const uint32_t nb = uint32_t(std::min<size_t>(c.batch, c.s_end - base));
        TraceParams P = P_call;
        uint32_t lane_no = stats ? 0u : s->next_lane % c.depth;
        if (!stats && c.depth > 1 && c.tile_pass && !c.round && !s->streaming_hint && b == 0 && !c.busy_at_call) {
            const auto want = tile_key(P, list_mode_for(false));
            for (uint32_t li = 0; li < c.depth; ++li)
                if (find_tile_set(s->lanes[li], want)) lane_no = li;
        } else if (!stats) {
            ++s->next_lane;
            if (b != 0 && c.depth > 1 && lane_no == prev_lane) lane_no = s->next_lane++ % c.depth;
        }
        prev_lane = lane_no;
        if (int rc = size_lane(s, c, lane_no)) return rc;
        rbrt_hip_scene::Lane& L = s->lanes[lane_no];
        hipStream_t ts = piped ? L.stream : stream;
        rbrt_hip_scene::Lane::Buf& B = L.bufs[0];
        if (piped) {
            if (B.in_use) HIP_TRY(hipStreamWaitEvent(L.stream, B.ev_resolved, 0));
        } else if (c.depth > 1) {
            if (int rc = sync_lanes(s, stream)) return rc;
        }
        L.open.valid = false;
        if (L.helper_pending) {
            constexpr size_t counter_bytes = sizeof(unsigned long long) * kWorkShards * kWorkCounterStride;
            if (!s->h_zeros) {
                HIP_TRY(hipHostMalloc(&s->h_zeros, counter_bytes, hipHostMallocDefault));
                std::memset(s->h_zeros, 0, counter_bytes);
            }
            HIP_TRY(hipStreamWaitEvent(ts, L.ev_helper, 0));
            HIP_TRY(hipMemcpyAsync(B.d_work_counter, s->h_zeros, counter_bytes, hipMemcpyHostToDevice, ts));
            L.helper_pending = false;
        }
        P.sample_base = base, P.batch = nb, P.batch_magic = div_magic_of(nb);
        P.n_items = (c.round ? uint64_t(c.round->n_active) * 64u : uint64_t(c.npix)) * nb;
        const bool busy = piped && other_launch_in_flight(s, &L);
        if (b == 0) call_streams = busy || (piped && s->streaming_hint);
        const uint32_t to_come = uint32_t(c.n_batches - 1 - b);
        const bool overlapped = call_streams || (piped && to_come != 0u);
        if (b == 0) s->streaming_hint = busy;
        P.work_stripes = !overlapped ? s->work_stripes
                         : s->work_stripes_overlap != kStripesAuto ? s->work_stripes_overlap
                         : 0u;
        P.sample_buf = B.d_sample_buf, P.work_counter = B.d_work_counter, P.gseq = L.d_gseq, P.gstack = L.d_gstack;
        P.helper_words = L.d_helper_words, P.helper_seq = ++L.seq, P.wave_base = 0u;
        rbrt_hip_scene::Lane::TileSet* S = nullptr;
        if (c.round) {
            P.tile_cull = c.round->d_cull, P.tile_lists = c.round->d_lists, P.tile_list_mode = 0u;
            if (piped) HIP_TRY(hipStreamWaitEvent(ts, c.round->ev_lists, 0));
        } else if (c.tile_pass) {
            const uint32_t list_mode = list_mode_for(overlapped && !stats);
            S = find_tile_set(L, tile_key(P, list_mode));
            if (!S) {
                S = L.tiles[0].last_used <= L.tiles[1].last_used ? &L.tiles[0] : &L.tiles[1];
                if (overlapped)
                    if (int rc = ensure_prep_stream(s)) return rc;
                if (int rc = fill_tile_set(S, P, list_mode, !overlapped, overlapped ? s->prep_stream : ts)) return rc;
                if (s->trace_launches) std::fprintf(stderr, "[rbrt_hip] tile pass on the prep stream: lane %u set %d list_mode %u\n",
                                                    unsigned(&L - s->lanes.data()), int(S - L.tiles), list_mode);
            }
            S->last_used = ++s->launch_no;
            if (s->trace_launches)
                std::fprintf(stderr, "[rbrt_hip] t %.3f ms launch %llu lane %u %s grid list_mode %u set %d\n", now_s() * 1e3, (unsigned long long)s->launch_no,
                             unsigned(&L - s->lanes.data()), overlapped ? "half" : "full", S->key.list_mode, int(S - L.tiles));
            P.tile_cull = S->d_cull, P.tile_lists = S->d_lists, P.tile_list_mode = S->key.list_mode;
            if (S->key.list_mode != 0u) P.tiles_reversed = 0u;
        }
        if (s->poison_samples) HIP_TRY(hipMemsetAsync(B.d_sample_buf, 0xFF, B.sample_buf_bytes, ts));
        if (c.timing) HIP_TRY(hipEventRecord(s->events[ev0 + 3 * b], ts));
        if (S) HIP_TRY(hipStreamWaitEvent(ts, S->ev_lists, 0));
        uint32_t grid = stats ? s->n_waves : grid_for(s, overlapped, c.depth, call_streams, to_come, P.n_items);
        if (c.round) grid = uint32_t(std::min<uint64_t>(grid, std::max<uint64_t>(P.n_items / 64u, 1u)));
        (grid < s->n_waves ? s->n_half_grid : s->n_full_grid) += 1;
        if (s->trace_launches)
            std::fprintf(stderr, "[rbrt_hip] trace launch: grid %u waves on %u CUs (%u waves per CU)\n", grid, s->n_cus, s->n_waves / s->n_cus);
        if (S && !stats && s->n_meshes <= 7u && (s->short_paths == 2u || (s->short_paths == 1u && overlapped))) {
            P.short_masks = B.d_short_masks;
            HIP_TRY(launch_short_paths(P, std::min<uint32_t>(c.n_local, kShortMaxWaves), ts));
            s->last_short.d_masks = B.d_short_masks, s->last_short.d_lists = P.tile_lists, s->last_short.batch = nb;
        }
        if (piped) HIP_TRY(hipEventRecord(L.ev_ready, ts));
        HIP_TRY(launch_trace_megakernel(P, grid, stats, ts));
        if (piped && s->helpers_mode != 0u && !c.round) {
            L.open.valid = true, L.open.P = P, L.open.grid = grid, L.open.helper_waves = 0u, L.open.rounds = 0u, L.open.seq = ++s->open_seq;
            if (s->helpers_mode == 2u) {
                if (!s->aux_stream) HIP_TRY(hipStreamCreateWithFlags(&s->aux_stream, hipStreamNonBlocking));
                if (int rc = issue_helper(s, L, s->n_cus, s->aux_stream)) return rc;
            }
        }
        if (c.timing) HIP_TRY(hipEventRecord(s->events[ev0 + 3 * b + 1], ts));
        R.sample_buf = B.d_sample_buf, R.work_counter = B.d_work_counter, R.tile_lists = P.tile_lists;
        R.batch = nb, R.first_batch = base == 0, R.last_batch = !c.round && base + nb == o->spp;
        R.sample_base = base;
        R.helper_words = P.helper_words, R.helper_seq = P.helper_seq;
        if (piped) {
            HIP_TRY(hipEventRecord(L.ev_traced, ts));
            L.in_use = true;
            HIP_TRY(hipStreamWaitEvent(stream, L.ev_traced, 0));
        }
        if (c.round) HIP_TRY(launch_resolve_even(P, R, c.round->n_active, stream));
        else HIP_TRY(launch_resolve(R, stream));
        if (c.tile_pass && !c.round) HIP_TRY(launch_sky_resolve(P, R, stream));
        if (S) {
            HIP_TRY(hipEventRecord(S->ev_free, stream));
            S->free_recorded = true;
        }
        if (c.depth > 1) {
            HIP_TRY(hipEventRecord(B.ev_resolved, stream));
            B.in_use = true;
        }
        if (c.timing) {
            HIP_TRY(hipEventRecord(s->events[ev0 + 3 * b + 2], stream));
            s->events_used = ev0 + 3 * (b + 1);
        }
    }
    return RBRT_OK;
}

}

static int check_render_args(const rbrt_hip_scene_t* s, const rbrt_camera_t* cam, const rbrt_render_opts_t* o, uint32_t s_begin,
                             uint32_t s_end) {
    if (!s || !cam || !o) return fail(RBRT_ERR_INVALID_ARG, "render: null argument");
    if (o->spp == 0) return fail(RBRT_ERR_INVALID_ARG, "spp must be >= 1");
    if (s_begin >= s_end || s_end > o->spp) return fail(RBRT_ERR_INVALID_ARG, "sample range must satisfy begin < end <= spp");
    if (o->max_depth > uint32_t(kMaxPathDepth))
        return fail(RBRT_ERR_UNSUPPORTED, "max_depth above the kernel limit of 64");
    if (cam->img_width_pix == 0 || cam->img_height_pix == 0)
        return fail(RBRT_ERR_INVALID_ARG, "image has zero pixels");
    if (uint64_t(cam->img_width_pix) * cam->img_height_pix >= (1ull << 32))
        return fail(RBRT_ERR_UNSUPPORTED, "image has 2^32 or more pixels");
    if (o->tile_rank >= (o->tile_world ? o->tile_world : 1)) return fail(RBRT_ERR_INVALID_ARG, "tile_rank >= tile_world");
    return lens_invalid(cam, o);
}

static int render_samples(rbrt_hip_scene_t* s, const rbrt_camera_t* cam, const rbrt_render_opts_t* o, void* stream_v,
                   uint32_t s_begin, uint32_t s_end, float* acc, float* d_radiance, uint8_t* d_rgb8,
                   const AdaptiveRound* round = nullptr) {
    if (int rc = check_render_args(s, cam, o, s_begin, s_end)) return rc;
    HIP_TRY(hipSetDevice(s->device));
    std::lock_guard<std::mutex> watcher_lock(s->mu);
    adopt_refined(s);
    CallPlan c{static_cast<hipStream_t>(stream_v), s_begin, s_end};
    c.round = round;
    if (!plan_call(s, cam, o, c)) return RBRT_OK;
    if (int rc = ensure_lanes(s, c.depth)) return rc;
    if (int rc = prepare_call(s, c, acc)) return rc;
    const TraceParams P = call_params(s, cam, o, c);
    ResolveParams R;
    std::memset(&R, 0, sizeof(R));
    R.width = cam->img_width_pix, R.height = cam->img_height_pix, R.tiles_x = c.tiles_x, R.n_tiles = c.n_tiles;
    R.tile_rank = o->tile_rank, R.tile_world = c.world, R.n_local_tiles = c.n_local;
    R.inv_spp = 1.0f / float(o->spp);
    R.acc = acc ? acc : s->d_acc, R.out_radiance = d_radiance, R.out_rgb8 = d_rgb8;
    R.acc_even = round ? round->d_sum_even : nullptr;
    R.counters = c.stats ? s->d_counters : nullptr, R.error_flag = &s->d_counters->diag[57];
    if (c.streams_now)
        for (uint32_t li = 0; li < c.depth; ++li)
            if (int rc = size_lane(s, c, li)) return rc;
    if (c.tile_pass && !s->one_shot)
        if (int rc = ensure_prep_stream(s)) return rc;
    if (c.tile_pass && c.streams_now && !round)
        if (int rc = warm_tile_tables(s, c, P)) return rc;
    if (int rc = issue_batches(s, c, o, P, R)) return rc;

    s->last_call_s = now_s();
    if (s->helpers_mode == 1u && c.depth > 1 && !c.stats && !round) {
        if (!s->watcher.joinable() && c.streams_now) {
            try {
                s->watcher = std::thread([s]() {
                    try {
                        watcher_main(s);
                    } catch (...) {
                    }
                });
            } catch (...) {
            }
        }
        s->cv.notify_one();
    }
    return RBRT_OK;
}

int rbrt_hip_render_device(rbrt_hip_scene_t* s, const rbrt_camera_t* cam, const rbrt_render_opts_t* o,
                           void* stream, float* d_radiance, uint8_t* d_rgb8) {
    return render_samples(s, cam, o, stream, 0, o ? o->spp : 0, nullptr, d_radiance, d_rgb8);
}

int rbrt_hip_render_pass(rbrt_hip_scene_t* s, const rbrt_camera_t* cam, const rbrt_render_opts_t* o, void* stream,
                         uint32_t sample_begin, uint32_t sample_end, float* d_accum, float* d_radiance, uint8_t* d_rgb8) {
    if (!d_accum) return fail(RBRT_ERR_INVALID_ARG, "render_pass: d_accum is null");
    return render_samples(s, cam, o, stream, sample_begin, sample_end, d_accum, d_radiance, d_rgb8);
}

namespace {

int size_adaptive(rbrt_hip_scene* s, const CallPlan& c) {
    auto& A = s->adaptive;
    void* p = nullptr;
    const size_t sum_floats = c.npix * 3u;
    if (sum_floats > A.sum_floats) {
        HIP_TRY(dev_alloc(s, sum_floats * sizeof(float), &p));
        A.d_sum = static_cast<float*>(p);
        HIP_TRY(dev_alloc(s, sum_floats * sizeof(float), &p));
        A.d_sum_even = static_cast<float*>(p);
        A.sum_floats = sum_floats;
    }
    if (c.n_tiles > A.cull_words) {
        HIP_TRY(dev_alloc(s, size_t(c.n_tiles) * sizeof(uint32_t), &p));
        A.d_cull = static_cast<uint32_t*>(p), A.cull_words = c.n_tiles;
    }
    if (c.n_local > A.local_tiles) {
        const size_t n = c.n_local, words = size_t(kTileListHeader) + 2u * n + 3u * n + 1u;
        HIP_TRY(dev_alloc(s, words * sizeof(uint32_t), &p));
        A.d_lists = static_cast<uint32_t*>(p);
        A.d_active = A.d_lists + kTileListHeader + 2u * n;
        A.d_tile_samples = A.d_active + n;
        A.d_tile_error = reinterpret_cast<float*>(A.d_tile_samples + n);
// ... 49 lines not shown
    A.n_max = N, A.threshold = a->threshold;
    A.tile_cull = c.tile_pass ? S.d_cull : nullptr, A.tile_lists = S.d_lists, A.active = S.d_active, A.n_active = S.d_n_active;
    A.tile_samples = S.d_tile_samples, A.tile_error = S.d_tile_error, A.acc = S.d_sum, A.acc_even = S.d_sum_even;
    A.out_radiance = d_radiance, A.out_rgb8 = d_rgb8;

    uint32_t n_prev = 0, n_k = std::min(a->min_samples, N), n_active = c.n_local;
    for (;;) {
        A.n = n_k, A.first_round = res.rounds == 0u ? 1u : 0u;
        HIP_TRY(launch_adaptive_lists(A, stream));
        HIP_TRY(hipEventRecord(S.ev_lists, stream));
        const AdaptiveRound round{A.tile_cull ? S.d_cull : nullptr, S.d_lists, S.d_sum_even, n_active, S.ev_lists};
        if (int rc = render_samples(s, cam, o, stream_v, n_prev, n_k, S.d_sum, nullptr, nullptr, &round)) return rc;
        HIP_TRY(launch_tile_error(A, n_active, stream));
        S.round_active.push_back(n_active);
        ++res.rounds;
        uint32_t left = 0;
        HIP_TRY(hipMemcpyAsync(&left, S.d_n_active, sizeof(left), hipMemcpyDeviceToHost, stream));
        HIP_TRY(hipStreamSynchronize(stream));
        n_active = left;
        if (n_active == 0u || n_k >= N) break;
        n_prev = n_k, n_k = uint32_t(std::min<uint64_t>(uint64_t(n_k) + a->step, N));
    }
    HIP_TRY(launch_adaptive_finish(A, stream));
    const size_t n = c.n_local;
    if (d_tile_samples) HIP_TRY(hipMemcpyAsync(d_tile_samples, S.d_tile_samples, n * sizeof(uint32_t), hipMemcpyDeviceToDevice, stream));
    if (d_tile_error) HIP_TRY(hipMemcpyAsync(d_tile_error, S.d_tile_error, n * sizeof(float), hipMemcpyDeviceToDevice, stream));
    std::vector<uint32_t> counts(n);
    HIP_TRY(hipMemcpyAsync(counts.data(), S.d_tile_samples, n * sizeof(uint32_t), hipMemcpyDeviceToHost, stream));
    HIP_TRY(hipStreamSynchronize(stream));
    for (size_t tl = 0; tl < n; ++tl) {
        uint32_t ty = 0, tx = 0;
        rbrt_hip_tile_xy(uint32_t(tl) * c.world + o->tile_rank, c.tiles_x, &ty, &tx);
        const uint64_t inside = uint64_t(std::min(RBRT_TILE, A.height - ty * RBRT_TILE)) * std::min(RBRT_TILE, A.width - tx * RBRT_TILE);
        res.samples += inside * counts[tl], res.samples_fixed += inside * N;
    }
    if (out) *out = res;
    S.last.complete = true;
    return RBRT_OK;
}

static int check_last_adaptive(rbrt_hip_scene_t* s, const char* call) {
    const auto& S = s->adaptive;
    const std::string c(call);
    if (!S.last.any) return fail(RBRT_ERR_INVALID_ARG, c + ": no adaptive render on this scene yet");
    if (S.last.world > 1u)
        return fail(RBRT_ERR_UNSUPPORTED, c + ": the last adaptive render had tile_world > 1 (a rank lacks its neighbours' pixels)");
    if (S.last.spp < 2u) return fail(RBRT_ERR_INVALID_ARG, c + ": the last adaptive render had spp < 2 (a half would be empty)");
    if (!S.last.complete) return fail(RBRT_ERR_INVALID_ARG, c + ": the last adaptive render did not complete");
    return RBRT_OK;
}

static int scene_halves(rbrt_hip_scene_t* s, hipStream_t stream, float* d_half_a, float* d_half_b) {
    auto& S = s->adaptive;
    HIP_TRY(hipSetDevice(s->device));
    const size_t npix = size_t(S.last.width) * S.last.height;
    {
        std::lock_guard<std::mutex> watcher_lock(s->mu);
        if (npix > S.half_pixels) {
            void* p = nullptr;
            HIP_TRY(dev_alloc(s, npix * 7u * sizeof(float), &p));
            S.d_half_a = static_cast<float*>(p), S.d_half_b = S.d_half_a + npix * 3u, S.d_wa = S.d_half_b + npix * 3u;
            S.half_pixels = npix;
        }
    }
    DenoiseHalvesParams Q;
    std::memset(&Q, 0, sizeof(Q));
    Q.acc = S.d_sum, Q.acc_even = S.d_sum_even, Q.tile_samples = S.d_tile_samples;
    Q.width = S.last.width, Q.height = S.last.height, Q.tiles_x = S.last.tiles_x;
    Q.a = S.d_half_a, Q.b = S.d_half_b, Q.wa = S.d_wa, Q.out_a = d_half_a, Q.out_b = d_half_b;
    HIP_TRY(launch_denoise_halves(Q, stream));
    return RBRT_OK;
}

int rbrt_hip_scene_denoise(rbrt_hip_scene_t* s, const rbrt_denoise_opts_t* d, void* stream_v, float* d_radiance, uint8_t* d_rgb8,
                           float* d_half_a, float* d_half_b) {
    if (!s || !d) return fail(RBRT_ERR_INVALID_ARG, "scene_denoise: null argument");
    if (int rc = check_denoise_opts(d)) return rc;
    if (int rc = check_last_adaptive(s, "scene_denoise")) return rc;
    auto& S = s->adaptive;
    const hipStream_t stream = static_cast<hipStream_t>(stream_v);
    if (int rc = scene_halves(s, stream, d_half_a, d_half_b)) return rc;
    if (!d_radiance && !d_rgb8) return RBRT_OK;
    HIP_TRY(launch_denoise(denoise_params(S.d_half_a, S.d_half_b, S.d_wa, S.last.width, S.last.height, d, d_radiance, d_rgb8), stream));
    return RBRT_OK;
}

int rbrt_hip_scene_denoise_guided(rbrt_hip_scene_t* s, const rbrt_guided_opts_t* g, void* stream_v, const float* d_albedo,
                                  const float* d_normal, const float* d_depth, const float* d_coverage, void* d_workspace,
                                  float* d_radiance, uint8_t* d_rgb8) {
    if (!s) return fail(RBRT_ERR_INVALID_ARG, "scene_denoise_guided: null argument");
    if (int rc = check_guided_args(g, d_albedo, d_normal, d_depth, d_coverage, d_workspace)) return rc;
    if (int rc = check_last_adaptive(s, "scene_denoise_guided")) return rc;
    auto& S = s->adaptive;
    if (uint64_t(S.last.width) * S.last.height >= (1ull << 31)) return fail(RBRT_ERR_UNSUPPORTED, "scene_denoise_guided: 2^31 or more pixels");
    if (!d_radiance && !d_rgb8) return RBRT_OK;
    const hipStream_t stream = static_cast<hipStream_t>(stream_v);
    if (int rc = scene_halves(s, stream, nullptr, nullptr)) return rc;
    HIP_TRY(launch_guided(guided_params(S.d_half_a, S.d_half_b, S.d_wa, d_albedo, d_normal, d_depth, d_coverage, S.last.width, S.last.height, g,
                                        d_workspace, d_radiance, d_rgb8),
                          guided_staged_max_step(), stream));
    return RBRT_OK;
}

void rbrt_feature_opts_default(rbrt_feature_opts_t* f) {
    if (!f) return;
    f->samples = 4u;
    f->reserved[0] = f->reserved[1] = f->reserved[2] = 0u;
}

int rbrt_hip_render_features(rbrt_hip_scene_t* s, const rbrt_camera_t* cam, const rbrt_render_opts_t* o, const rbrt_feature_opts_t* f,
                             void* stream, float* d_albedo, float* d_normal, float* d_depth, float* d_coverage, int32_t* d_object) {
    if (!s || !cam || !o || !f) return fail(RBRT_ERR_INVALID_ARG, "render_features: null argument");
    if (f->samples == 0u || f->samples > 65536u) return fail(RBRT_ERR_INVALID_ARG, "render_features: samples must be 1..65536");
    if (f->reserved[0] != 0u || f->reserved[1] != 0u || f->reserved[2] != 0u)
        return fail(RBRT_ERR_INVALID_ARG, "render_features: reserved must be 0");
    if (o->flags & RBRT_FLAG_COLLECT_STATS)
        return fail(RBRT_ERR_INVALID_ARG, "render_features: RBRT_FLAG_COLLECT_STATS belongs to the render calls");
    if (cam->img_width_pix == 0 || cam->img_height_pix == 0) return fail(RBRT_ERR_INVALID_ARG, "render_features: image has zero pixels");
    if (o->tile_rank >= (o->tile_world ? o->tile_world : 1)) return fail(RBRT_ERR_INVALID_ARG, "render_features: tile_rank >= tile_world");
    if (int rc = lens_invalid(cam, o)) return rc;
    if (o->tile_world > 1u) return fail(RBRT_ERR_UNSUPPORTED, "render_features: tile_world > 1 (features are made of the whole frame)");
    if (uint64_t(cam->img_width_pix) * cam->img_height_pix >= (1ull << 32))
        return fail(RBRT_ERR_UNSUPPORTED, "render_features: image has 2^32 or more pixels");
    if (!d_albedo && !d_normal && !d_depth && !d_coverage && !d_object) return RBRT_OK;
    HIP_TRY(hipSetDevice(s->device));
    TraceParams P;
    fill_trace_params(s, cam, o, P);
    P.tiles_x = (cam->img_width_pix + RBRT_TILE - 1) / RBRT_TILE, P.tiles_y = (cam->img_height_pix + RBRT_TILE - 1) / RBRT_TILE;
    P.n_tiles = P.tiles_x * P.tiles_y;
    FeatureParams F;
    std::memset(&F, 0, sizeof(F));
    F.samples = f->samples, F.inv_n = 1.0f / float(f->samples), F.stack_entries = s->stack_need;
    F.albedo = d_albedo, F.normal = d_normal, F.depth = d_depth, F.coverage = d_coverage, F.object = d_object;
    HIP_TRY(launch_features(P, F, static_cast<hipStream_t>(stream)));
    return RBRT_OK;
}

int rbrt_hip_scene_adaptive_rounds(rbrt_hip_scene_t* s, uint32_t* active_tiles, size_t n, uint32_t* n_rounds) {
    if (!s || !n_rounds || (n != 0 && !active_tiles)) return fail(RBRT_ERR_INVALID_ARG, "adaptive_rounds: null argument");
    const auto& r = s->adaptive.round_active;
    *n_rounds = uint32_t(r.size());
    for (size_t i = 0; i < n && i < r.size(); ++i) active_tiles[i] = r[i];
    return RBRT_OK;
}

int rbrt_hip_scene_set_short_paths(rbrt_hip_scene_t* s, int mode) {
    if (!s) return fail(RBRT_ERR_INVALID_ARG, "set_short_paths: null scene");
    if (mode < 0 || mode > 2) return fail(RBRT_ERR_INVALID_ARG, "set_short_paths: mode must be 0 (off), 1 (automatic) or 2 (every launch)");
    std::lock_guard<std::mutex> watcher_lock(s->mu);
    s->short_paths = uint32_t(mode);
    return RBRT_OK;
}

int rbrt_hip_debug_short_masks(rbrt_hip_scene_t* s, uint64_t* out_masks, size_t n, size_t* n_chunks) {
    if (!s || !n_chunks || (n != 0 && !out_masks)) return fail(RBRT_ERR_INVALID_ARG, "debug_short_masks: null argument");
    HIP_TRY(hipSetDevice(s->device));
    std::lock_guard<std::mutex> watcher_lock(s->mu);
    *n_chunks = 0;
    const auto& ls = s->last_short;
    if (!ls.d_masks) return RBRT_OK;
    HIP_TRY(hipDeviceSynchronize());
    uint32_t n_work = 0;
    HIP_TRY(hipMemcpy(&n_work, ls.d_lists, sizeof(n_work), hipMemcpyDeviceToHost));
    *n_chunks = size_t(n_work) * ls.batch;
    const size_t m = std::min(n, *n_chunks);
    if (m != 0) HIP_TRY(hipMemcpy(out_masks, ls.d_masks, m * sizeof(uint64_t), hipMemcpyDeviceToHost));
    return RBRT_OK;
}

int rbrt_hip_scene_set_pipeline(rbrt_hip_scene_t* s, uint32_t depth) {
    if (!s) return fail(RBRT_ERR_INVALID_ARG, "set_pipeline: null scene");
    if (depth > kMaxPipeline) return fail(RBRT_ERR_INVALID_ARG, "set_pipeline: depth must be 0 (automatic) or 1..8");
    HIP_TRY(hipSetDevice(s->device));
    std::lock_guard<std::mutex> watcher_lock(s->mu);
    HIP_TRY(hipDeviceSynchronize());
    s->pipeline = depth;
    s->next_lane = 0;
    return ensure_lanes(s, depth ? depth : 2u);
}

int rbrt_hip_scene_set_environment(rbrt_hip_scene_t* s, const rbrt_environment_t* env) {
    if (!s) return fail(RBRT_ERR_INVALID_ARG, "set_environment: null scene");
    std::vector<EnvTexel> texels;
    if (env) {
        if (env->n == 0u || env->n > 4096u) return fail(RBRT_ERR_INVALID_ARG, "set_environment: n must be 1..4096");
        if (env->reserved != 0u) return fail(RBRT_ERR_INVALID_ARG, "set_environment: reserved must be 0");
        if (!env->nodes) return fail(RBRT_ERR_INVALID_ARG, "set_environment: null nodes");
        const size_t count = size_t(env->n + 1u) * (env->n + 1u);
        texels.resize(count);
        for (size_t k = 0; k < count; ++k) {
            const float* v = env->nodes + 3 * k;
            for (int c = 0; c < 3; ++c)
                if (!std::isfinite(v[c]) || v[c] < 0.0f)
                    return fail(RBRT_ERR_INVALID_ARG, "set_environment: node " + std::to_string(k) + " has a non-finite or negative component");
            texels[k] = EnvTexel{v[0], v[1], v[2], 0.0f};
        }
    }
    HIP_TRY(hipSetDevice(s->device));
    std::lock_guard<std::mutex> watcher_lock(s->mu);
    HIP_TRY(hipDeviceSynchronize());
    void* p = nullptr;
    if (env) {
        const hipError_t e = dev_alloc(s, texels.size() * sizeof(EnvTexel), &p, true);
        if (e != hipSuccess) return fail(e == hipErrorOutOfMemory ? RBRT_ERR_OOM : RBRT_ERR_HIP, std::string("set_environment: ") + hipGetErrorString(e));
        const hipError_t c = hipMemcpy(p, texels.data(), texels.size() * sizeof(EnvTexel), hipMemcpyHostToDevice);
        if (c != hipSuccess) {
            (void)dev_release(s, p);
            return fail(RBRT_ERR_HIP, std::string("set_environment: ") + hipGetErrorString(c));
        }
    }
    if (s->d_env) HIP_TRY(dev_release(s, s->d_env));
    s->d_env = static_cast<EnvTexel*>(p), s->env_n = env ? env->n : 0u;
    return RBRT_OK;
}

static int travel_invalid(const float* travel, const char* who) {
    for (int c = 0; c < 3; ++c)
        if (!std::isfinite(travel[c])) return fail(RBRT_ERR_INVALID_ARG, std::string(who) + ": travel must be finite");
    return RBRT_OK;
}
int rbrt_hip_scene_set_shutter(rbrt_hip_scene_t* s, const rbrt_shutter_t* shutter) {
    if (!s) return fail(RBRT_ERR_INVALID_ARG, "set_shutter: null scene");
    if (shutter) {
        if (int rc = travel_invalid(shutter->travel, "set_shutter")) return rc;
        if (shutter->reserved != 0u) return fail(RBRT_ERR_INVALID_ARG, "set_shutter: reserved must be 0");
    }
    std::lock_guard<std::mutex> watcher_lock(s->mu);
    s->has_shutter = shutter != nullptr;
    for (int c = 0; c < 3; ++c) s->travel[c] = shutter ? shutter->travel[c] : 0.0f;
    return RBRT_OK;
}

int rbrt_hip_scene_stats(rbrt_hip_scene_t* s, rbrt_hip_stats_t* out) {
    if (!s || !out) return fail(RBRT_ERR_INVALID_ARG, "stats: null argument");
    HIP_TRY(hipSetDevice(s->device));
    HIP_TRY(hipDeviceSynchronize());
    DevCounters c;
    HIP_TRY(hipMemcpy(&c, s->d_counters, sizeof(c), hipMemcpyDeviceToHost));
    s->stats.rays = c.rays;
    s->stats.mesh_gate_pass = c.mesh_gate_pass;
    s->stats.nodes_visited = c.nodes_visited;
    s->stats.tris_tested = c.tris_tested;
    s->stats.mesh_hits = c.mesh_hits;
    s->stats.samples = c.samples;
    s->stats.nan_discriminants = c.nan_discriminants;
    s->stats.node_bytes = sizeof(BvhNode4);
    s->stats.tri_bytes = sizeof(BvhTri);
    *out = s->stats;
    if (c.diag[57])
        return fail(RBRT_ERR_HIP, "the trace kernel detected corrupt internal state (a path slot without a valid sample index)");
    return RBRT_OK;
}

int rbrt_hip_scene_check(rbrt_hip_scene_t* s) {
    if (!s) return fail(RBRT_ERR_INVALID_ARG, "check: null scene");
    HIP_TRY(hipSetDevice(s->device));
    HIP_TRY(hipDeviceSynchronize());
    unsigned long long nan = 0, corrupt = 0;
    HIP_TRY(hipMemcpy(&nan, &s->d_counters->nan_discriminants, sizeof(nan), hipMemcpyDeviceToHost));
    HIP_TRY(hipMemcpy(&corrupt, &s->d_counters->diag[57], sizeof(corrupt), hipMemcpyDeviceToHost));
    if (nan) HIP_TRY(hipMemset(&s->d_counters->nan_discriminants, 0, sizeof(nan)));
    if (corrupt) HIP_TRY(hipMemset(&s->d_counters->diag[57], 0, sizeof(corrupt)));
    if (corrupt)
        return fail(RBRT_ERR_HIP, "the trace kernel detected corrupt internal state (a path slot without a valid sample index)");
    if (nan)
        return fail(RBRT_ERR_NAN, "a sphere discriminant was NaN " + std::to_string(nan) +
                                      " times (the reference panics: sphere.rs:33); those rays were treated as misses");
    return RBRT_OK;
}

int rbrt_hip_scene_create_times(rbrt_hip_scene_t* s, rbrt_hip_call_times_t* out) {
    if (!s || !out) return fail(RBRT_ERR_INVALID_ARG, "create_times: null argument");
    *out = s->create_times;
    return RBRT_OK;
}

int rbrt_hip_last_render_times(rbrt_hip_call_times_t* out) {
    if (!out) return fail(RBRT_ERR_INVALID_ARG, "last_render_times: null argument");
    *out = g_last_render_times;
    return RBRT_OK;
}

int rbrt_hip_scene_refine_wait(rbrt_hip_scene_t* s, double timeout_s, int* state, double* build_seconds) {
    if (!s) return fail(RBRT_ERR_INVALID_ARG, "refine_wait: null scene");
    int st = 0;
    if (Refine* r = s->refine.get()) {
        const double t0 = now_s();
        while (r->state.load(std::memory_order_acquire) == 0 && now_s() - t0 < timeout_s) std::this_thread::sleep_for(std::chrono::microseconds(200));
        HIP_TRY(hipSetDevice(s->device));
        adopt_refined(s);
        const int rs = r->state.load(std::memory_order_acquire);
        st = rs == 0 ? 3 : s->n_refined != 0 ? 1 : 2;
        if (build_seconds) *build_seconds = rs == 0 ? 0.0 : r->seconds;
        if (st == 2 && r->th.joinable()) r->th.join();
        if (st == 2) g_last_error = "background BVH build: " + r->error;
    } else if (build_seconds) {
        *build_seconds = 0.0;
    }
    if (state) *state = st;
    return RBRT_OK;
}

int rbrt_hip_scene_info(rbrt_hip_scene_t* s, rbrt_hip_scene_info_t* out) {
    if (!s || !out) return fail(RBRT_ERR_INVALID_ARG, "scene_info: null argument");
    adopt_refined(s);
    std::memset(out, 0, sizeof(*out));
// ... 365 lines not shown
```

rbrt_amd/csrc/device_types.h:

```cpp
#pragma once
#include <stdint.h>

#include "../../include/rbrt_hip.h"

namespace rbrt {

#if defined(__HIPCC__)
#define RBRT_HOST_DEVICE __host__ __device__
#else
#define RBRT_HOST_DEVICE
#endif
RBRT_HOST_DEVICE inline void tile_xy(uint32_t tile, uint32_t tiles_x, uint32_t& ty, uint32_t& tx) {
    ty = tile / tiles_x;
    tx = uint32_t((uint64_t(tile - ty * tiles_x) + uint64_t(RBRT_TILE_SKEW) * ty) % tiles_x);
}
RBRT_HOST_DEVICE inline uint32_t tile_number(uint32_t ty, uint32_t tx, uint32_t tiles_x) {
    const uint32_t rot = uint32_t((uint64_t(RBRT_TILE_SKEW) * ty) % tiles_x);
    return ty * tiles_x + (tx + tiles_x - rot) % tiles_x;
}
constexpr uint32_t kTileListHeader = 4;
constexpr int kBlock = 256;
constexpr int kSmallBlock = 64;
constexpr int kMaxBvhDepth = 20;
constexpr int kStackMax = 3 * (kMaxBvhDepth + 1) + 1;
constexpr int kMaxPathDepth = 64;
constexpr int kMaxObjects = 255;
constexpr int kLeafBits = 2;
constexpr int kLeafMax = 1 << kLeafBits;
constexpr int kPool = 128;
constexpr uint32_t kWorkShards = 8;
constexpr uint32_t kWorkCounterStride = 16;
constexpr uint32_t kMaxShadeRounds = 64;
constexpr int kLdsStack = 8;

constexpr int32_t kNoChild = INT32_MIN;
struct alignas(128) BvhNode4 {
    float lo_x[4], lo_y[4], lo_z[4];
    float hi_x[4], hi_y[4], hi_z[4];
    int32_t child[4];
    float max_e12[4];
};
static_assert(sizeof(BvhNode4) == 128, "node must be 128 B");

struct alignas(16) BvhTri {
    float v0[3];
    float e1x;
    float e1yz[2];
    float e2xy[2];
    float e2z;
    uint32_t index;
    uint32_t pad[2];
};
static_assert(sizeof(BvhTri) == 48, "tri must be 48 B");

struct alignas(16) Normal4 {
    float x, y, z, w;
};
struct alignas(16) SmoothRec {
    float v0[3], e1[3], e2[3];
    float n0[3], n1[3], n2[3];
    float pad[2];
};
static_assert(sizeof(SmoothRec) == 80 && sizeof(SmoothRec) % sizeof(Normal4) == 0, "smooth record must be 80 B");

struct DevSphere {
    float center[3];
    float radius;
};

struct DevTriangle {
    float v0[3], e0[3], e1[3], normal[3];
};

struct DevMaterial {
    float albedo[3];
    float param;
    int32_t kind;
};
constexpr int32_t kDevMatEmissive = -1;
RBRT_HOST_DEVICE inline int32_t dev_material_kind(int32_t kind) { return kind == RBRT_MAT_EMISSIVE ? kDevMatEmissive : kind; }

struct DevPattern {
    float origin[3];
    float inv;
};
constexpr uint32_t kPatternLinkShift = 8;
RBRT_HOST_DEVICE inline uint32_t pattern_table_dwords(uint32_t n_pat) {
    return n_pat * uint32_t((sizeof(DevMaterial) + sizeof(DevPattern)) / 4);
}
constexpr int kMaxMaterialEntries = 256;

struct DevMesh {
    const BvhNode4* nodes;
    const BvhTri* tris;
    const Normal4* normals;
    float bbox_lo[3];
    float bbox_hi[3];
    float center[3];
    float radius;
    float max_e12;
    uint32_t n_nodes;
    uint32_t n_tris;
};

struct DevCounters {
    unsigned long long rays, mesh_gate_pass, nodes_visited, tris_tested, mesh_hits, samples,
        nan_discriminants;
    unsigned long long diag[64];
};

struct alignas(16) EnvTexel {
    float r, g, b, pad;
};

struct TraceParams {
    rbrt_camera_t cam;
    float min_dist, max_dist, eps_frac;
    float bg[3];
    uint32_t max_depth;
    uint32_t constant_bg;
    uint64_t seed_key;
    uint32_t n_spheres, n_meshes;
    uint32_t n_elem_tris;
    const DevSphere* spheres;
    const DevTriangle* elem_tris;
    const uint32_t* elems;
    const DevMaterial* materials;
    const DevMesh* meshes;
    const BvhTri* tris;
    uint32_t tiles_x, tiles_y, n_tiles;
    uint32_t tile_rank, tile_world, n_local_tiles;
    uint32_t sample_base;
    uint32_t batch;
    uint32_t tiles_reversed;
    uint32_t batch_magic, tiles_x_magic;
    uint64_t n_items;
    float* sample_buf;
    DevCounters* counters;
    unsigned long long* work_counter;
    uint32_t* gseq;
    uint32_t stack_entries;
    uint32_t* gstack;
    uint32_t y_low_water;
    uint32_t y_high_water, y_high_min_parked;
    uint32_t leaf_round;
    uint32_t share_idle;
    uint32_t leaf_leaves;
    uint32_t work_stripes;
    uint32_t shade_rounds;
    uint32_t shade_cont_min;
    uint32_t* tile_cull;
    uint32_t* tile_lists;
    uint32_t tile_list_mode;
    uint32_t tile_tail_div;
    uint32_t tile_lists_wide;
    uint32_t* helper_words;
    uint32_t helper_seq;
    uint32_t wave_base;
    uint32_t helper_min_items;
    uint32_t thin_lens;
    float lens_u[3], lens_v[3], focus_scale;
    uint32_t shutter;
    float travel[3];
    const EnvTexel* env_nodes;
    uint32_t env_n;
    unsigned long long* short_masks;
    uint32_t pattern_dw;
};

struct ResolveParams {
    uint32_t width, height, tiles_x, n_tiles;
    uint32_t tile_rank, tile_world, n_local_tiles;
    uint32_t batch;
    uint32_t first_batch, last_batch;
    float inv_spp;
    const float* sample_buf;
    float* acc;
    float* out_radiance;
    uint8_t* out_rgb8;
    unsigned long long* work_counter;
    const uint32_t* tile_lists;
    DevCounters* counters;
    uint32_t* helper_words;
    uint32_t helper_seq;
    unsigned long long* error_flag;
    float* acc_even;
    uint32_t sample_base;
};

struct FeatureParams {
    uint32_t samples;
    float inv_n;
    uint32_t stack_entries;
    float* albedo;
    float* normal;
    float* depth;
    float* coverage;
    int32_t* object;
};

struct AdaptiveParams {
    uint32_t width, height, tiles_x;
    uint32_t tile_rank, tile_world, n_local_tiles;
    uint32_t n, n_max;
    float threshold;
    uint32_t first_round;
    const uint32_t* tile_cull;
    uint32_t* tile_lists;
    uint32_t* active;
    uint32_t* n_active;
    uint32_t* tile_samples;
    float* tile_error;
    const float* acc;
    const float* acc_even;
    float* out_radiance;
    uint8_t* out_rgb8;
};

struct DenoiseParams {
    const float* a;
    const float* b;
    const float* wa;
    uint32_t width, height;
    int32_t window_radius, patch_radius;
    float k2;
    float* out_radiance;
    uint8_t* out_rgb8;
};

struct DenoiseHalvesParams {
    const float* acc;
    const float* acc_even;
    const uint32_t* tile_samples;
    uint32_t width, height, tiles_x;
    float* a;
    float* b;
    float* wa;
    float* out_a;
    float* out_b;
};

struct TonemapParams {
    const float* in;
    uint32_t n;
    uint32_t curve;
    float exposure, white;
    float key;
    uint32_t key_permille, white_permille;
    uint32_t* hist;
    float* out_radiance;
    uint8_t* out_rgb8;
};

struct GlareParams {
    const float* in;
    uint32_t width, height;
    uint32_t levels;
    float threshold, intensity, spread;
    float a;
    void* workspace;
    float* out_radiance;
    uint8_t* out_rgb8;
};

struct GuidedParams {
    const float* a;
    const float* b;
    const float* wa;
    const float* albedo;
    const float* normal;
    const float* depth;
    const float* coverage;
    uint32_t width, height;
    uint32_t levels;
    uint32_t flags;
    float kc2, kz2, in, ia;
    void* workspace;
    float* out_radiance;
    uint8_t* out_rgb8;
};

struct TemporalParams {
    const float* a;
    const float* b;
    const float* normal;
    const float* depth;
    const float* coverage;
    const void* history_in;
    void* history_out;
    float* out_a;
    float* out_b;
    float* out_length;
    uint32_t width, height;
    float max_history, kz, kn2;
    float pos[3], right[3], up[3], center[3];
    float mm_hor, mm_vert;
    float pos_prev[3], right_prev[3], up_prev[3];
    float n[3], w[3];
    float wn, rr, uu, ru, det, sx, sy, hx, hy;
};

struct UpsampleParams {
    const float* a;
    const float* b;
    const float* wa;
    const float* albedo;
    const float* normal;
    const float* depth;
    const float* coverage;
    void* workspace;
    float* out_a;
    float* out_b;
    float* out_wa;
    uint32_t width, height;
    uint32_t low_width, low_height;
    uint32_t factor, flags;
    float in, ia, kz2, invf;
};

struct DespikeParams {
    const float* a;
// ... 32 lines not shown
```

rbrt_amd/csrc/kernels.hip:

```cpp
#include <hip/hip_runtime.h>
#include <stdint.h>

#include "device_types.h"

#pragma clang fp contract(off)

namespace rbrt {

struct V3 {
    float x, y, z;
};
__device__ __forceinline__ V3 mk(float x, float y, float z) { return V3{x, y, z}; }
__device__ __forceinline__ V3 mk(const float* p) { return V3{p[0], p[1], p[2]}; }
__device__ __forceinline__ V3 operator+(V3 a, V3 b) { return V3{a.x + b.x, a.y + b.y, a.z + b.z}; }
__device__ __forceinline__ V3 operator-(V3 a, V3 b) { return V3{a.x - b.x, a.y - b.y, a.z - b.z}; }
__device__ __forceinline__ V3 operator*(V3 a, V3 b) { return V3{a.x * b.x, a.y * b.y, a.z * b.z}; }
__device__ __forceinline__ V3 operator*(float s, V3 b) { return V3{s * b.x, s * b.y, s * b.z}; }
__device__ __forceinline__ V3 operator*(V3 a, float s) { return V3{a.x * s, a.y * s, a.z * s}; }
__device__ __forceinline__ float dot(V3 a, V3 b) { return (a.x * b.x + a.y * b.y) + a.z * b.z; }

__device__ __forceinline__ float sqrt_core(float x) {
    const float r = __builtin_amdgcn_sqrtf(x);
    const float r_dn = __uint_as_float(__float_as_uint(r) - 1u), r_up = __uint_as_float(__float_as_uint(r) + 1u);
    const float e_dn = __builtin_fmaf(-r_dn, r, x), e_up = __builtin_fmaf(-r_up, r, x);
// ... 629 lines not shown
    } else if (!R.last_batch || !packed) {
        return;
    }
    const size_t o = packed ? j * 3u : (size_t(row) * R.width + col) * 3u;
    if (R.out_radiance) {
        R.out_radiance[o + 0] = ax;
        R.out_radiance[o + 1] = ay;
        R.out_radiance[o + 2] = az;
    }
    if (R.out_rgb8) {
        R.out_rgb8[o + 0] = quantise(ax);
        R.out_rgb8[o + 1] = quantise(ay);
        R.out_rgb8[o + 2] = quantise(az);
    }
}

__global__ __launch_bounds__(kSmallBlock) void resolve_kernel(const ResolveParams R) {
    const size_t npix = size_t(R.tile_lists ? R.tile_lists[0] : R.n_local_tiles) * 64u;
    const size_t i = size_t(blockIdx.x) * kSmallBlock + threadIdx.x;
    if (R.helper_words) {
        if (threadIdx.x == 0 && __hip_atomic_load(R.helper_words, __ATOMIC_RELAXED, __HIP_MEMORY_SCOPE_AGENT) != 0u) {
            uint32_t spins = 0;
            while (__hip_atomic_load(R.helper_words, __ATOMIC_ACQUIRE, __HIP_MEMORY_SCOPE_AGENT) != 0u) {
                __builtin_amdgcn_s_sleep(16);
                if (++spins > (1u << 23)) {
                    atomicAdd(R.error_flag, 1ull);
                    break;
                }
            }
            __builtin_amdgcn_fence(__ATOMIC_ACQUIRE, "agent");
        }
        __syncthreads();
    }
    if (blockIdx.x == 0) {
        if (R.helper_words && threadIdx.x == 0) {
            __hip_atomic_store(R.helper_words + 1, R.helper_seq, __ATOMIC_RELEASE, __HIP_MEMORY_SCOPE_AGENT);
            __builtin_amdgcn_fence(__ATOMIC_RELEASE, "agent");
        }
        __syncthreads();
        for (uint32_t w = threadIdx.x; w < kWorkShards * kWorkCounterStride; w += kSmallBlock) R.work_counter[w] = 0ull;
    }
    if (i >= npix) return;
    const uint32_t p = uint32_t(i & 63u);
    const uint32_t tile_local = R.tile_lists ? R.tile_lists[kTileListHeader + (i >> 6)] : uint32_t(i >> 6);
    const size_t j = size_t(tile_local) * 64u + p;
    const uint32_t tile = tile_local * R.tile_world + R.tile_rank;
    uint32_t ty, tx;
    tile_xy(tile, R.tiles_x, ty, tx);
    const uint32_t row = ty * RBRT_TILE + (p >> 3), col = tx * RBRT_TILE + (p & 7u);
    const bool valid = row < R.height && col < R.width;
    float ax = 0.0f, ay = 0.0f, az = 0.0f;
    if (valid) {
        if (!R.first_batch) {
            ax = R.acc[j * 3 + 0];
            ay = R.acc[j * 3 + 1];
            az = R.acc[j * 3 + 2];
        }
        for (uint32_t s = 0; s < R.batch; ++s) {
            const float* sp = R.sample_buf + (size_t(s) * npix + i) * 3u;
            ax = ax + sp[0];
            ay = ay + sp[1];
            az = az + sp[2];
        }
    }
    resolve_store(R, j, row, col, valid, ax, ay, az);
}

__global__ __launch_bounds__(kSmallBlock) void sky_resolve_kernel(const TraceParams P, const ResolveParams R) {
    const size_t i = size_t(blockIdx.x) * kSmallBlock + threadIdx.x;
    if (i >= size_t(R.tile_lists[1]) * 64u) return;
    const uint32_t p = uint32_t(i & 63u);
    const uint32_t tile_local = R.tile_lists[kTileListHeader + R.n_local_tiles + (i >> 6)];
    const size_t j = size_t(tile_local) * 64u + p;
    const uint32_t tile = tile_local * R.tile_world + R.tile_rank;
    uint32_t ty, tx;
    tile_xy(tile, R.tiles_x, ty, tx);
    const uint32_t row = ty * RBRT_TILE + (p >> 3), col = tx * RBRT_TILE + (p & 7u);
    const bool valid = row < R.height && col < R.width;
    float ax = 0.0f, ay = 0.0f, az = 0.0f;
    if (valid) {
        if (!R.first_batch) {
            ax = R.acc[j * 3 + 0];
            ay = R.acc[j * 3 + 1];
            az = R.acc[j * 3 + 2];
        }
        const V3 pos = mk(P.cam.position), center = mk(P.cam.img_center_point), right = mk(P.cam.right), up = mk(P.cam.up);
        for (uint32_t s = 0; s < R.batch; ++s) {
            Rng rng;
            rng.init(P.seed_key, row * R.width + col, P.sample_base + s);
            V3 o = pos, f = camera_target(center, right, up, P.cam.mm_per_pix_hor, P.cam.mm_per_pix_vert, R.width, R.height, row, col, rng);
            if (P.thin_lens) {
                const float lens[7] = {P.lens_u[0], P.lens_u[1], P.lens_u[2], P.lens_v[0], P.lens_v[1], P.lens_v[2], P.focus_scale};
                lens_point(o, f, lens, rng);
            }
            const V3 d = normalize(f - o);
            const V3 c = P.env_nodes ? environment_radiance(P.env_nodes, P.env_n, d) : background(d.y, P.bg, P.constant_bg);
            ax = ax + c.x;
            ay = ay + c.y;
            az = az + c.z;
        }
        if (R.counters) {
            atomicAdd(&R.counters->rays, (unsigned long long)R.batch);
            atomicAdd(&R.counters->samples, (unsigned long long)R.batch);
            atomicAdd(&R.counters->diag[32], (unsigned long long)R.batch);
        }
    }
    resolve_store(R, j, row, col, valid, ax, ay, az);
}

struct D3 {
    double x, y, z;
};
__device__ __forceinline__ D3 d3(const float* p) { return D3{double(p[0]), double(p[1]), double(p[2])}; }
__device__ __forceinline__ D3 operator+(D3 a, D3 b) { return D3{a.x + b.x, a.y + b.y, a.z + b.z}; }
__device__ __forceinline__ D3 operator-(D3 a, D3 b) { return D3{a.x - b.x, a.y - b.y, a.z - b.z}; }
__device__ __forceinline__ D3 operator*(double s, D3 a) { return D3{s * a.x, s * a.y, s * a.z}; }
__device__ __forceinline__ double ddot(D3 a, D3 b) { return a.x * b.x + a.y * b.y + a.z * b.z; }
__device__ __forceinline__ D3 dcross(D3 a, D3 b) { return D3{a.y * b.z - a.z * b.y, a.z * b.x - a.x * b.z, a.x * b.y - a.y * b.x}; }
__device__ __forceinline__ double dlen(D3 a) { return sqrt(ddot(a, a)); }
__device__ __forceinline__ D3 unit_or_nan(D3 v) { return (1.0 / dlen(v)) * v; }
__device__ __forceinline__ double angle_between(D3 u, D3 v) {
    const double c = ddot(u, v);
    return acos(c > 1.0 ? 1.0 : c < -1.0 ? -1.0 : c);
}

struct CullSlab {
    D3 n_lo, n_hi;
    __device__ __forceinline__ bool outside(D3 q, double reach) const {
        const double g0 = ddot(n_lo, q), g1 = ddot(n_hi, q);
        return (g0 > reach && g1 > reach) || (g0 < -reach && g1 < -reach);
    }
};
struct CullCone {
    D3 mid;
    double cos_rho, sin_rho;
    __device__ __forceinline__ bool misses(D3 qhat, double l, double R, double sign) const {
        if (!(R < l)) return false;
        const double sa = R / l, ca = sqrt(1.0 - sa * sa);
        return sign * ddot(mid, qhat) < ca * cos_rho - sa * sin_rho;
    }
    D3 corner[4];
    double cos_w, sin_w;
    __device__ __forceinline__ bool backward_deep(D3 qhat, double l, double r_in) const {
        if (!(r_in > 0.0 && r_in < l)) return false;
        const double sa = r_in / l, ca = sqrt(1.0 - sa * sa);
        if (!(sa > sin_w)) return false;
        const double cos_cap = ca * cos_w + sa * sin_w;
        bool in = true;
        for (uint32_t k = 0; k < 4u; ++k) in = in && -ddot(corner[k], qhat) > cos_cap;
        return in;
    }
};

constexpr int kCullBlock = 64;
constexpr uint32_t kCullLanes = 4;
__global__ __launch_bounds__(kCullBlock, 4) void primary_cull_kernel(const TraceParams P) {
    const uint32_t cull_world = P.tile_world > 1u ? P.tile_world : 1u;
    const uint32_t tile_local = (blockIdx.x * kCullBlock + threadIdx.x) / kCullLanes;
    const uint32_t tile = tile_local * cull_world + (cull_world > 1u ? P.tile_rank : 0u);
    const uint32_t quad_lane = threadIdx.x % kCullLanes, quad_shift = threadIdx.x & ~(kCullLanes - 1u);
    if (tile >= P.n_tiles) return;
    uint32_t ty, tx;
    tile_xy(tile, P.tiles_x, ty, tx);
    const rbrt_camera_t& c = P.cam;
    const uint32_t W = c.img_width_pix, H = c.img_height_pix;
    const D3 pos = d3(c.position), right = d3(c.right), up = d3(c.up), ctr = d3(c.img_center_point);
    const D3 a = ctr - pos;
    const double pad = 1e-3 + double(W > H ? W : H) * (1.0 / 4194304.0);
    const uint32_t c0 = tx * RBRT_TILE, r0 = ty * RBRT_TILE;
    const uint32_t c1 = (c0 + RBRT_TILE < W ? c0 + RBRT_TILE : W) - 1u, r1 = (r0 + RBRT_TILE < H ? r0 + RBRT_TILE : H) - 1u;
    const double mmh = double(c.mm_per_pix_hor), mmv = double(c.mm_per_pix_vert);
    const double cm0 = (double(c0) - double(W / 2u) - 0.5 - pad) * mmh, cm1 = (double(c1) - double(W / 2u) + 0.5 + pad) * mmh;
    const double rm0 = (double(r0) - double(H / 2u) - 0.5 - pad) * mmv, rm1 = (double(r1) - double(H / 2u) + 0.5 + pad) * mmv;
    const double cm_abs = fabs(cm0) > fabs(cm1) ? fabs(cm0) : fabs(cm1), rm_abs = fabs(rm0) > fabs(rm1) ? fabs(rm0) : fabs(rm1);
    const double err = 8.0 * (1.0 / 8388608.0) * (dlen(ctr) + dlen(pos) + 0.001 * cm_abs * dlen(right) + 0.001 * rm_abs * dlen(up));
    const double plane_dist = fabs(ddot(a, unit_or_nan(dcross(right, up))));
    double angle = 2.0 * err / plane_dist + 1e-6;
    double lens_a = 0.0, lens_beta = 0.0;
    if (P.thin_lens) {
        const D3 lu = d3(P.lens_u), lv = d3(P.lens_v);
        const double fs = double(P.focus_scale), nu = dlen(lu), nv = dlen(lv);
        const double u16 = 16.0 * (1.0 / 16777216.0);
        double tmax = 0.0;
        for (uint32_t k = 0; k < 4u; ++k) {
            const double t = dlen(a + (0.001 * (k & 1u ? cm1 : cm0)) * right - (0.001 * (k & 2u ? rm1 : rm0)) * up);
            tmax = t > tmax || !(t == t) ? t : tmax;
        }
        lens_a = sqrt(nu * nu + nv * nv) + u16 * (dlen(pos) + nu + nv);
        const double f_min = fs * plane_dist;
        const double err_f = fs * err + u16 * (dlen(pos) + 2.0 * fs * tmax + lens_a);
        angle = 2.0 * err_f / (f_min - lens_a) + 1e-6;
        const double sb = lens_a / f_min;
        lens_beta = sb / sqrt(1.0 - sb * sb);
        if (!(sb < 1.0) || !(lens_beta == lens_beta)) angle = __builtin_nan("");
    }
    double org_a = lens_a;
    if (P.shutter) {
        const double tl = dlen(d3(P.travel));
        org_a = lens_a + tl + 16.0 * (1.0 / 16777216.0) * (dlen(pos) + lens_a + tl);
        if (!(org_a == org_a)) angle = __builtin_nan("");
    }
    CullSlab cols, rows;
    cols.n_lo = unit_or_nan(dcross(a + (0.001 * cm0) * right, up));
    cols.n_hi = unit_or_nan(dcross(a + (0.001 * cm1) * right, up));
    rows.n_lo = unit_or_nan(dcross(a - (0.001 * rm0) * up, right));
    rows.n_hi = unit_or_nan(dcross(a - (0.001 * rm1) * up, right));
    CullCone cone;
    cone.mid = unit_or_nan(a + (0.0005 * (cm0 + cm1)) * right - (0.0005 * (rm0 + rm1)) * up);
    double rho = 0.0;
    for (uint32_t k = 0; k < 4u; ++k) {
        const D3 u = unit_or_nan(a + (0.001 * (k & 1u ? cm1 : cm0)) * right - (0.001 * (k & 2u ? rm1 : rm0)) * up);
        cone.corner[k] = u;
        const double t = angle_between(cone.mid, u);
        rho = t > rho || !(t == t) ? t : rho;
    }
    const double w_dir = angle + lens_beta;
    rho += w_dir;
    if (!(rho < 1.5)) rho = __builtin_nan("");
    cone.cos_rho = cos(rho), cone.sin_rho = sin(rho);
    cone.cos_w = cos(w_dir), cone.sin_w = sin(w_dir);

    const uint32_t n_elem = P.n_spheres + P.n_elem_tris;
    uint32_t word = 0;
    bool all = n_elem <= 24u && P.n_meshes <= 7u && P.n_elem_tris == 0u;
    for (uint32_t e = 0; e < n_elem && e < 24u; ++e) {
        const uint32_t desc = P.elems ? P.elems[e] : e;
        bool out = false;
        if (!(desc >> 31)) {
            const DevSphere sp = P.spheres[desc];
            const D3 q = d3(sp.center) - pos;
            const double r = double(sp.radius), l = dlen(q);
            if (r > 0.0 && r < 1e30 && l < 1e30) {
                const double lo = l + org_a;
                const double slack = 1e-5 * r + 1e-5 * (lo * lo + r * r) / r + 1e-6 * lo;
                const double reach = r + slack + org_a + w_dir * (l + r + org_a);
                const double r_out = r + slack + org_a, r_in = r - slack - org_a;
                const D3 qhat = (1.0 / l) * q;
                out = cols.outside(q, reach) || rows.outside(q, reach) ||
                      (cone.misses(qhat, l, r_out, 1.0) && (cone.misses(qhat, l, r_out, -1.0) || cone.backward_deep(qhat, l, r_in)));
            }
        }
        if (out) word |= 1u << e;
        else all = false;
    }
    const auto box_unreachable = [&](D3 lo, D3 hi, double slack, double far) -> bool {
        const D3 q = 0.5 * (lo + hi) - pos;
        const double l = dlen(q);
        if (cone.misses((1.0 / l) * q, l, 0.5 * dlen(hi - lo) * 1.001 + slack + org_a, 1.0)) return true;
        const double reach = slack + org_a + w_dir * (far + org_a);
        for (uint32_t slab = 0; slab < 2u; ++slab) {
            const CullSlab& sl = slab ? rows : cols;
            bool pos_side = true, neg_side = true;
            for (uint32_t k = 0; k < 8u; ++k) {
                const D3 v = D3{k & 1u ? hi.x : lo.x, k & 2u ? hi.y : lo.y, k & 4u ? hi.z : lo.z} - pos;
                const double g0 = ddot(sl.n_lo, v), g1 = ddot(sl.n_hi, v);
                pos_side = pos_side && g0 > reach && g1 > reach;
                neg_side = neg_side && g0 < -reach && g1 < -reach;
            }
            if (pos_side || neg_side) return true;
        }
        return false;
    };
    for (uint32_t m = 0; m < P.n_meshes && m < 7u; ++m) {
        const DevMesh& md = P.meshes[m];
        double far = 0.0;
        bool finite = true;
        for (uint32_t k = 0; k < 8u; ++k) {
            const D3 q = D3{double(k & 1u ? md.bbox_hi[0] : md.bbox_lo[0]), double(k & 2u ? md.bbox_hi[1] : md.bbox_lo[1]),
                            double(k & 4u ? md.bbox_hi[2] : md.bbox_lo[2])} - pos;
            const double l = dlen(q);
            finite = finite && l < 1e30;
            far = l > far ? l : far;
        }
        const double slack = 16.0 * (1.0 / 16777216.0) * (far + org_a);
        const bool out = finite && box_unreachable(d3(md.bbox_lo), d3(md.bbox_hi), slack, far);
        if (out) word |= 1u << (24u + m);
        const D3 mc = d3(md.center) - pos;
        const double o_inf = fmax(fmax(fabs(pos.x), fabs(pos.y)), fabs(pos.z));
        const double pad_base = 64.0 * (1.0 / 16777216.0) * (dlen(mc) + double(md.radius) + o_inf + org_a);
        bool mesh_free = out;
        if (!out && all && finite && md.n_nodes != 0u) {
            constexpr uint32_t kCullLevels = 6;
            uint32_t stack[3 * kCullLevels + 4];
            uint32_t sp = 0;
            stack[sp++] = 0u;
            mesh_free = true;
            while (sp != 0u && mesh_free) {
                const uint32_t e = stack[--sp];
                const BvhNode4& nd = md.nodes[e >> 3];
                const uint32_t c = quad_lane;
                const int32_t link = nd.child[c];
                uint32_t state = 0u;
                if (link != kNoChild) {
                    const D3 lo = D3{double(nd.lo_x[c]), double(nd.lo_y[c]), double(nd.lo_z[c])};
                    const D3 hi = D3{double(nd.hi_x[c]), double(nd.hi_y[c]), double(nd.hi_z[c])};
                    if (!(dlen(lo - pos) < 1e30 && dlen(hi - pos) < 1e30)) state = 2u;
                    else if (!box_unreachable(lo, hi, pad_base * (double(nd.max_e12[c]) * 1.001 * double(P.eps_frac) + 1.0), far))
                        state = (link >= 0 && (e & 7u) + 1u < kCullLevels) ? 1u : 2u;
                }
                const uint32_t open = uint32_t(__builtin_amdgcn_ballot_w64(state == 1u) >> quad_shift) & 15u;
                const uint32_t stay = uint32_t(__builtin_amdgcn_ballot_w64(state == 2u) >> quad_shift) & 15u;
                if (stay != 0u) mesh_free = false;
                for (uint32_t k = 0; k < 4u && mesh_free; ++k) {
                    if (!((open >> k) & 1u)) continue;
                    if (sp < 3u * kCullLevels + 4u) stack[sp++] = (uint32_t(nd.child[k]) << 3) | ((e & 7u) + 1u);
                    else mesh_free = false;
                }
            }
        }
        if (!mesh_free) all = false;
    }
    if (all) word |= 1u << 31;
    if (quad_lane == 0u) P.tile_cull[tile] = word;
}

template <int kListBlock>
__global__ __launch_bounds__(kListBlock) void tile_lists_kernel(const TraceParams P) {
    const uint32_t n = P.n_local_tiles, t = threadIdx.x;
    const uint32_t per = (n + kListBlock - 1) / kListBlock;
    const uint32_t lo = t * per < n ? t * per : n, hi = lo + per < n ? lo + per : n;
    const uint32_t el_mask = (1u << (P.n_spheres < 24u ? P.n_spheres : 24u)) - 1u, me_mask = (1u << (P.n_meshes < 7u ? P.n_meshes : 7u)) - 1u;
    const auto class_of = [&](uint32_t word) -> uint32_t {
        if (word >> 31) return 2u;
        if (P.tile_list_mode == 0u) return 0u;
        const bool light = ((word >> 24) & me_mask) == me_mask && __popc(~word & el_mask) <= 1 && P.n_spheres <= 24u && P.n_meshes <= 7u &&
                           P.n_elem_tris == 0u;
        return light ? 1u : 0u;
    };
    constexpr uint32_t kBatch = 8;
    const auto load_batch = [&](uint32_t tl0, uint32_t (&w)[kBatch]) {
#pragma unroll
        for (uint32_t j = 0; j < kBatch; ++j) w[j] = tl0 + j < hi ? P.tile_cull[(tl0 + j) * P.tile_world + P.tile_rank] : 0x80000000u;
    };
    uint32_t mine[2] = {0u, 0u};
    for (uint32_t tl0 = lo; tl0 < hi; tl0 += kBatch) {
        uint32_t w[kBatch];
        load_batch(tl0, w);
#pragma unroll
        for (uint32_t j = 0; j < kBatch; ++j) {
            const uint32_t c = class_of(w[j]);
            if (tl0 + j < hi && c < 2u) ++mine[c];
        }
    }
    uint32_t incl[2] = {mine[0], mine[1]};
    const uint32_t wlane = t & 63u;
    for (uint32_t d = 1; d < 64u; d <<= 1) {
        const uint32_t v0 = uint32_t(__shfl_up(int(incl[0]), d, 64)), v1 = uint32_t(__shfl_up(int(incl[1]), d, 64));
        if (wlane >= d) incl[0] += v0, incl[1] += v1;
    }
    uint32_t n_heavy = uint32_t(__shfl(int(incl[0]), 63, 64)), n_light = uint32_t(__shfl(int(incl[1]), 63, 64));
    if (kListBlock > 64) {
        __shared__ uint32_t wave_total[2][kListBlock / 64];
        if (wlane == 63u) wave_total[0][t >> 6] = n_heavy, wave_total[1][t >> 6] = n_light;
        __syncthreads();
        n_heavy = n_light = 0u;
        for (uint32_t w = 0; w < uint32_t(kListBlock / 64); ++w) {
            if (w < (t >> 6)) incl[0] += wave_total[0][w], incl[1] += wave_total[1][w];
            n_heavy += wave_total[0][w], n_light += wave_total[1][w];
        }
    }
    const uint32_t n_work = n_heavy + n_light;
    uint32_t r[2] = {incl[0] - mine[0], incl[1] - mine[1]};
    uint32_t k = lo - r[0] - r[1];
    uint32_t* const work = P.tile_lists + kTileListHeader;
    uint32_t* const sky = work + n;
    uint32_t n_tail = n_work / (P.tile_tail_div != 0u ? P.tile_tail_div : 8u);
    n_tail = n_tail < n_light ? n_tail : n_light;
    const uint32_t n_front_light = n_light - n_tail;
    for (uint32_t tl0 = lo; tl0 < hi; tl0 += kBatch) {
      uint32_t w[kBatch];
      load_batch(tl0, w);
#pragma unroll
      for (uint32_t j = 0; j < kBatch; ++j) {
        const uint32_t tl = tl0 + j;
        if (tl >= hi) continue;
        const uint32_t c = class_of(w[j]);
        if (c == 2u) {
            sky[k++] = tl;
            continue;
        }
        uint32_t pos;
        if (P.tile_list_mode == 4u) {
            const bool rev = P.tiles_reversed != 0u;
            const uint32_t h = c == 0u ? (rev ? n_heavy - 1u - r[0] : r[0]) : (rev ? n_heavy - r[0] : r[0]);
            const uint32_t l = c == 1u ? (rev ? n_light - 1u - r[1] : r[1]) : (rev ? n_light - r[1] : r[1]);
            if (c == 1u && l >= n_front_light) pos = (n_work - n_tail) + (l - n_front_light);
            else pos = h + (l < n_front_light ? l : n_front_light);
            ++r[c];
        } else {
            pos = r[0]++;
        }
        work[pos] = tl;
      }
    }
    if (t == kListBlock - 1) {
        P.tile_lists[0] = n_work;
        P.tile_lists[1] = n - n_work;
        P.tile_lists[2] = n_light, P.tile_lists[3] = 0u;
    }
}

__host__ __device__ inline uint32_t local_tiles_of(uint32_t n_tiles, uint32_t rank, uint32_t world) {
    return rank < n_tiles ? (n_tiles - rank + world - 1u) / world : 0u;
}


__global__ __launch_bounds__(kSmallBlock) void resolve_even_kernel(const ResolveParams R) {
    const size_t npix = size_t(R.tile_lists[0]) * 64u;
    const size_t i = size_t(blockIdx.x) * kSmallBlock + threadIdx.x;
    if (blockIdx.x == 0) {
        if (R.helper_words && threadIdx.x == 0) {
            __hip_atomic_store(R.helper_words + 1, R.helper_seq, __ATOMIC_RELEASE, __HIP_MEMORY_SCOPE_AGENT);
            __builtin_amdgcn_fence(__ATOMIC_RELEASE, "agent");
        }
        __syncthreads();
        for (uint32_t w = threadIdx.x; w < kWorkShards * kWorkCounterStride; w += kSmallBlock) R.work_counter[w] = 0ull;
    }
    if (i >= npix) return;
    const uint32_t p = uint32_t(i & 63u);
    const uint32_t tile_local = R.tile_lists[kTileListHeader + (i >> 6)];
    const size_t j = size_t(tile_local) * 64u + p;
    const uint32_t tile = tile_local * R.tile_world + R.tile_rank;
    uint32_t ty, tx;
    tile_xy(tile, R.tiles_x, ty, tx);
    const uint32_t row = ty * RBRT_TILE + (p >> 3), col = tx * RBRT_TILE + (p & 7u);
    if (!(row < R.height && col < R.width)) return;
    float ax = 0.0f, ay = 0.0f, az = 0.0f, ex = 0.0f, ey = 0.0f, ez = 0.0f;
    if (!R.first_batch) {
        ax = R.acc[j * 3 + 0], ay = R.acc[j * 3 + 1], az = R.acc[j * 3 + 2];
        ex = R.acc_even[j * 3 + 0], ey = R.acc_even[j * 3 + 1], ez = R.acc_even[j * 3 + 2];
    }
    for (uint32_t s = 0; s < R.batch; ++s) {
        const float* sp = R.sample_buf + (size_t(s) * npix + i) * 3u;
        const float cx = sp[0], cy = sp[1], cz = sp[2];
        ax = ax + cx;
        ay = ay + cy;
        az = az + cz;
        if (((R.sample_base + s) & 1u) == 0u) {
            ex = ex + cx;
            ey = ey + cy;
            ez = ez + cz;
        }
    }
    R.acc[j * 3 + 0] = ax, R.acc[j * 3 + 1] = ay, R.acc[j * 3 + 2] = az;
    R.acc_even[j * 3 + 0] = ex, R.acc_even[j * 3 + 1] = ey, R.acc_even[j * 3 + 2] = ez;
}

__global__ __launch_bounds__(kSmallBlock) void sky_resolve_even_kernel(const TraceParams P, const ResolveParams R) {
    const size_t i = size_t(blockIdx.x) * kSmallBlock + threadIdx.x;
    if (i >= size_t(R.tile_lists[1]) * 64u) return;
    const uint32_t p = uint32_t(i & 63u);
    const uint32_t tile_local = R.tile_lists[kTileListHeader + R.n_local_tiles + (i >> 6)];
    const size_t j = size_t(tile_local) * 64u + p;
    const uint32_t tile = tile_local * R.tile_world + R.tile_rank;
    uint32_t ty, tx;
    tile_xy(tile, R.tiles_x, ty, tx);
    const uint32_t row = ty * RBRT_TILE + (p >> 3), col = tx * RBRT_TILE + (p & 7u);
    if (!(row < R.height && col < R.width)) return;
    float ax = 0.0f, ay = 0.0f, az = 0.0f, ex = 0.0f, ey = 0.0f, ez = 0.0f;
    if (!R.first_batch) {
        ax = R.acc[j * 3 + 0], ay = R.acc[j * 3 + 1], az = R.acc[j * 3 + 2];
        ex = R.acc_even[j * 3 + 0], ey = R.acc_even[j * 3 + 1], ez = R.acc_even[j * 3 + 2];
    }
    const V3 pos = mk(P.cam.position), center = mk(P.cam.img_center_point), right = mk(P.cam.right), up = mk(P.cam.up);
    for (uint32_t s = 0; s < R.batch; ++s) {
        Rng rng;
        rng.init(P.seed_key, row * R.width + col, P.sample_base + s);
        V3 o = pos, f = camera_target(center, right, up, P.cam.mm_per_pix_hor, P.cam.mm_per_pix_vert, R.width, R.height, row, col, rng);
        if (P.thin_lens) {
            const float lens[7] = {P.lens_u[0], P.lens_u[1], P.lens_u[2], P.lens_v[0], P.lens_v[1], P.lens_v[2], P.focus_scale};
            lens_point(o, f, lens, rng);
        }
        const V3 d = normalize(f - o);
        const V3 c = P.env_nodes ? environment_radiance(P.env_nodes, P.env_n, d) : background(d.y, P.bg, P.constant_bg);
        ax = ax + c.x;
        ay = ay + c.y;
        az = az + c.z;
        if (((P.sample_base + s) & 1u) == 0u) {
            ex = ex + c.x;
            ey = ey + c.y;
            ez = ez + c.z;
        }
    }
    R.acc[j * 3 + 0] = ax, R.acc[j * 3 + 1] = ay, R.acc[j * 3 + 2] = az;
    R.acc_even[j * 3 + 0] = ex, R.acc_even[j * 3 + 1] = ey, R.acc_even[j * 3 + 2] = ez;
}

__global__ __launch_bounds__(64) void adaptive_lists_kernel(const AdaptiveParams A) {
    const uint32_t n = A.n_local_tiles, t = threadIdx.x;
    const uint32_t per = (n + 63u) / 64u;
    const uint32_t lo = t * per < n ? t * per : n, hi = lo + per < n ? lo + per : n;
    const auto class_of = [&](uint32_t tl) -> uint32_t {
        if (!A.first_round && A.active[tl] == 0u) return 2u;
        return A.tile_cull ? A.tile_cull[tl * A.tile_world + A.tile_rank] >> 31 : 0u;
    };
    uint32_t mine[2] = {0u, 0u};
    for (uint32_t tl = lo; tl < hi; ++tl) {
        const uint32_t c = class_of(tl);
        if (c < 2u) ++mine[c];
    }
    uint32_t incl[2] = {mine[0], mine[1]};
    for (uint32_t d = 1; d < 64u; d <<= 1) {
        const uint32_t v0 = uint32_t(__shfl_up(int(incl[0]), d, 64)), v1 = uint32_t(__shfl_up(int(incl[1]), d, 64));
        if (t >= d) incl[0] += v0, incl[1] += v1;
    }
    const uint32_t n_work = uint32_t(__shfl(int(incl[0]), 63, 64)), n_sky = uint32_t(__shfl(int(incl[1]), 63, 64));
    uint32_t r[2] = {incl[0] - mine[0], incl[1] - mine[1]};
    uint32_t* const work = A.tile_lists + kTileListHeader;
    uint32_t* const sky = work + n;
    for (uint32_t tl = lo; tl < hi; ++tl) {
        const uint32_t c = class_of(tl);
        if (c == 0u) work[r[0]++] = tl;
        else if (c == 1u) sky[r[1]++] = tl;
    }
    if (t == 63u) {
        A.tile_lists[0] = n_work;
        A.tile_lists[1] = n_sky;
        A.tile_lists[2] = 0u, A.tile_lists[3] = 0u;
        *A.n_active = 0u;
    }
}

__global__ __launch_bounds__(64) void tile_error_kernel(const AdaptiveParams A) {
    const uint32_t w = blockIdx.x, p = threadIdx.x;
    const uint32_t n_work = A.tile_lists[0], n_sky = A.tile_lists[1];
    if (w >= n_work + n_sky) return;
    const uint32_t tile_local = w < n_work ? A.tile_lists[kTileListHeader + w] : A.tile_lists[kTileListHeader + A.n_local_tiles + (w - n_work)];
    const size_t j = size_t(tile_local) * 64u + p;
    const uint32_t tile = tile_local * A.tile_world + A.tile_rank;
    uint32_t ty, tx;
    tile_xy(tile, A.tiles_x, ty, tx);
    const uint32_t row = ty * RBRT_TILE + (p >> 3), col = tx * RBRT_TILE + (p & 7u);
    const uint32_t h = (A.n + 1u) / 2u;
    const float inv_n = 1.0f / float(A.n), inv_h = 1.0f / float(h);
    float q = 0.0f;
    if (row < A.height && col < A.width) {
        const float ir = A.acc[j * 3 + 0] * inv_n, ig = A.acc[j * 3 + 1] * inv_n, ib = A.acc[j * 3 + 2] * inv_n;
        const float ar = A.acc_even[j * 3 + 0] * inv_h, ag = A.acc_even[j * 3 + 1] * inv_h, ab = A.acc_even[j * 3 + 2] * inv_h;
        const float e = (__builtin_fabsf(ir - ar) + __builtin_fabsf(ig - ag)) + __builtin_fabsf(ib - ab);
        q = e / (__builtin_sqrtf((ir + ig) + ib) + 0.0001f);
    }
    float v = q;
    for (uint32_t d = 1; d < 64u; d <<= 1) v = v + __shfl_xor(v, int(d), 64);
    const uint32_t rows_in = A.height - ty * RBRT_TILE < RBRT_TILE ? A.height - ty * RBRT_TILE : RBRT_TILE;
    const uint32_t cols_in = A.width - tx * RBRT_TILE < RBRT_TILE ? A.width - tx * RBRT_TILE : RBRT_TILE;
    const float err = v / float(rows_in * cols_in);
    if (p == 0u) {
        const bool go_on = A.n < A.n_max && !(err < A.threshold);
        A.tile_samples[tile_local] = A.n;
        A.tile_error[tile_local] = err;
        A.active[tile_local] = go_on ? 1u : 0u;
        if (go_on) atomicAdd(A.n_active, 1u);
// ... 440 lines not shown
```

Before: 11980 Mray-samples/s.

## Build per-tile BVH entry nodes so traversal starts below the root

Adds a tile_entries kernel that, per work tile and per mesh, walks the BVH top levels against the tile's ray cone and writes a synthetic 4-wide entry node made of the reachable subtrees. Mesh trees are copied into one allocation next to the entry rows so child links can be addressed relative to the rows. The tracer is given the per-tile entries, so rays for a tile can skip the shared upper levels of traversal. It costs an extra kernel per tile pass plus extra device memory and host-side copies when the mesh table changes. The cull code is refactored into shared helpers.

```diff
diff --git a/include/rbrt_hip_debug.h b/include/rbrt_hip_debug.h
--- a/include/rbrt_hip_debug.h
+++ b/include/rbrt_hip_debug.h
@@ -86,6 +86,16 @@
 int rbrt_hip_scene_set_short_paths(rbrt_hip_scene_t* scene, int mode);
 int rbrt_hip_debug_short_masks(rbrt_hip_scene_t* scene, uint64_t* out_masks, size_t n, size_t* n_chunks);
 
+int rbrt_hip_scene_set_tile_entries(rbrt_hip_scene_t* scene, int mode);
+typedef struct {
+    uint32_t made;
+    uint32_t n_work;
+    uint32_t n_meshes;
+    uint32_t used_meshes;
+} rbrt_hip_tile_entries_info_t;
+int rbrt_hip_debug_tile_entries(rbrt_hip_scene_t* scene, rbrt_hip_tile_entries_info_t* info, uint32_t* out_tiles, size_t n_tiles,
+                                void* out_nodes, size_t n_nodes);
+
 typedef struct rbrt_hip_call_times {
     double hip_init_s;
     double upload_s;
diff --git a/rbrt_amd/__init__.py b/rbrt_amd/__init__.py
--- a/rbrt_amd/__init__.py
+++ b/rbrt_amd/__init__.py
@@ -195,6 +195,20 @@
         if n.value:
             abi.check(self._lib.rbrt_hip_debug_short_masks(self._h, out.ctypes.data_as(C.POINTER(C.c_uint64)), n.value, C.byref(n)))
         return out
+
+    def set_tile_entries(self, mode: int = 1):
+        abi.check(self._lib.rbrt_hip_scene_set_tile_entries(self._h, int(mode)))
+
+    def tile_entries(self):
+        info = abi.TileEntriesInfo()
+        abi.check(self._lib.rbrt_hip_debug_tile_entries(self._h, C.byref(info), None, 0, None, 0))
+        if not info.made:
+            return None
+        tiles = np.zeros(info.n_work, np.uint32)
+        nodes = np.zeros((info.n_meshes, info.n_work, 32), np.uint32)
+        abi.check(self._lib.rbrt_hip_debug_tile_entries(self._h, C.byref(info), tiles.ctypes.data_as(C.POINTER(C.c_uint32)), tiles.size,
+                                                        nodes.ctypes.data_as(C.c_void_p), info.n_meshes * info.n_work))
+        return {"tiles": tiles, "nodes": nodes, "used_meshes": int(info.used_meshes)}
 
     def set_timing(self, on: bool = True):
         abi.check(self._lib.rbrt_hip_scene_set_timing(self._h, int(on)))
diff --git a/rbrt_amd/abi.py b/rbrt_amd/abi.py
--- a/rbrt_amd/abi.py
+++ b/rbrt_amd/abi.py
@@ -276,6 +276,10 @@
 
     def as_dict(self) -> dict:
         return {k: getattr(self, k) for k, _ in self._fields_}
+
+
+class TileEntriesInfo(C.Structure):
+    _fields_ = [("made", C.c_uint32), ("n_work", C.c_uint32), ("n_meshes", C.c_uint32), ("used_meshes", C.c_uint32)]
 
 
 HIP_SYMBOLS = {
@@ -392,6 +396,8 @@
     "rbrt_hip_debug_environment": (C.c_int, [C.c_void_p, f32p, C.c_size_t, f32p]),
     "rbrt_hip_scene_set_short_paths": (C.c_int, [C.c_void_p, C.c_int]),
     "rbrt_hip_debug_short_masks": (C.c_int, [C.c_void_p, C.POINTER(C.c_uint64), C.c_size_t, C.POINTER(C.c_size_t)]),
+    "rbrt_hip_scene_set_tile_entries": (C.c_int, [C.c_void_p, C.c_int]),
+    "rbrt_hip_debug_tile_entries": (C.c_int, [C.c_void_p, C.POINTER(TileEntriesInfo), C.POINTER(C.c_uint32), C.c_size_t, C.c_void_p, C.c_size_t]),
 }
 
 
diff --git a/rbrt_amd/csrc/api.cpp b/rbrt_amd/csrc/api.cpp
--- a/rbrt_amd/csrc/api.cpp
+++ b/rbrt_amd/csrc/api.cpp
@@ -30,6 +30,7 @@
                             uint32_t environment, uint32_t pattern_dw, uint32_t shutter);
 int megakernel_occupancy_per_cu(size_t lds_bytes);
 hipError_t launch_primary_cull(const TraceParams& P, hipStream_t stream);
+hipError_t launch_tile_entries(const TraceParams& P, hipStream_t stream);
 hipError_t launch_sky_resolve(const TraceParams& P, const ResolveParams& R, hipStream_t stream);
 hipError_t launch_short_paths(const TraceParams& P, uint32_t n_waves, hipStream_t stream);
 hipError_t launch_code_load(hipStream_t stream);
@@ -242,10 +243,16 @@
             float lens_u[3], lens_v[3], focus_scale;
             uint32_t shutter;
             float travel[3];
+            const DevMesh* meshes;
+            uint32_t entries_mode;
         };
         struct TileSet {
             uint32_t* d_cull = nullptr;
             uint32_t* d_lists = nullptr;
+            BvhNode4* d_entries = nullptr;
+            uint32_t entry_meshes = 0;
+            const DevMesh* d_entry_meshes = nullptr;
+            uint32_t entries_in_range = 0;
             hipEvent_t ev_lists = nullptr;
             hipEvent_t ev_free = nullptr;
             bool free_recorded = false;
@@ -253,7 +260,9 @@
             TileKey key;
             uint64_t last_used = 0;
         } tiles[2];
-        size_t tile_cull_words = 0, tile_lists_words = 0;
+        size_t tile_cull_words = 0, tile_lists_words = 0, tile_entry_nodes = 0;
+        void* d_entry_piece = nullptr;
+        const DevMesh* entries_made_for = nullptr;
         hipEvent_t ev_traced = nullptr;
         bool in_use = false;
         uint32_t* d_helper_words = nullptr;
@@ -332,7 +341,14 @@
     bool trace_create = false;
     uint32_t tile_tail_div = 8;
     uint32_t primary_cull = 1;
+    uint32_t tile_entries = 1;
     uint32_t short_paths = 1;
+    struct LastEntries {
+        const BvhNode4* d_entries = nullptr;
+        const uint32_t* d_lists = nullptr;
+        uint32_t entry_meshes = 0, n_local = 0;
+        bool made = false;
+    } last_entries;
     struct LastShort {
         const unsigned long long* d_masks = nullptr;
         const uint32_t* d_lists = nullptr;
@@ -1514,9 +1530,12 @@
     return P;
 }
 
+uint32_t entry_meshes_in_range(const std::vector<const BvhNode4*>& trees, const BvhNode4* d_entries, size_t n_rows);
+
 int size_lane(rbrt_hip_scene* s, const CallPlan& c, uint32_t li) {
     rbrt_hip_scene::Lane& L = s->lanes[li];
     const size_t need = c.need, n_tiles = c.n_tiles, lists_need = size_t(kTileListHeader) + 2u * size_t(c.n_local);
+    const size_t entries_need = size_t(std::min<uint32_t>(s->n_meshes, kTileEntryMeshes)) * c.n_local;
     if (!L.d_gseq) {
         void* p = nullptr;
         const size_t gseq_bytes = (megakernel_gseq_bytes(s->scratch_waves) + kSlabAlign - 1) & ~(kSlabAlign - 1);
@@ -1546,6 +1565,7 @@
         for (auto& T : L.tiles) {
             T.d_cull = T.d_lists = nullptr;
             T.key_valid = false, T.free_recorded = false;
+            s->last_entries = {};
             void* p = nullptr;
             HIP_TRY(dev_alloc(s, size_t(n_tiles) * sizeof(uint32_t), &p));
             T.d_cull = static_cast<uint32_t*>(p);
@@ -1556,6 +1576,42 @@
         }
         L.tile_cull_words = n_tiles, L.tile_lists_words = lists_need;
     }
+    if (c.tile_pass && !c.round && entries_need != 0 && s->tile_entries != 0u && (entries_need > L.tile_entry_nodes || L.entries_made_for != s->d_meshes)) {
+        if (L.d_entry_piece) {
+            if (int rc = sync_lanes(s, c.stream)) return rc;
+            if (s->prep_stream) HIP_TRY(hipStreamSynchronize(s->prep_stream));
+            HIP_TRY(dev_release(s, L.d_entry_piece));
+            L.d_entry_piece = nullptr;
+        }
+        const uint32_t n_ent = std::min<uint32_t>(s->n_meshes, kTileEntryMeshes);
+        std::vector<DevMesh> table(s->n_meshes);
+        HIP_TRY(hipMemcpy(table.data(), s->d_meshes, table.size() * sizeof(DevMesh), hipMemcpyDeviceToHost));
+        size_t tree_nodes = 0;
+        for (uint32_t m = 0; m < n_ent; ++m) tree_nodes += table[m].n_nodes;
+        const size_t table_nodes = (table.size() * sizeof(DevMesh) + sizeof(BvhNode4) - 1) / sizeof(BvhNode4);
+        void* piece = nullptr;
+        HIP_TRY(dev_alloc(s, (tree_nodes + table_nodes + 2u * entries_need) * sizeof(BvhNode4), &piece, true));
+        BvhNode4* at = static_cast<BvhNode4*>(piece);
+        std::vector<const BvhNode4*> trees;
+        for (uint32_t m = 0; m < n_ent; ++m) {
+            if (table[m].n_nodes != 0u) HIP_TRY(hipMemcpy(at, table[m].nodes, size_t(table[m].n_nodes) * sizeof(BvhNode4), hipMemcpyDeviceToDevice));
+            table[m].nodes = at;
+            trees.push_back(at);
+            at += table[m].n_nodes;
+        }
+        HIP_TRY(hipMemcpy(at, table.data(), table.size() * sizeof(DevMesh), hipMemcpyHostToDevice));
+        HIP_TRY(hipDeviceSynchronize());
+        const DevMesh* const d_table = reinterpret_cast<const DevMesh*>(at);
+        at += table_nodes;
+        for (int k = 0; k < 2; ++k) {
+            rbrt_hip_scene::Lane::TileSet& T = L.tiles[k];
+            T.d_entries = at + size_t(k) * entries_need, T.d_entry_meshes = d_table;
+            T.entries_in_range = entry_meshes_in_range(trees, T.d_entries, entries_need);
+            T.entry_meshes = 0u, T.key_valid = false;
+        }
+        s->last_entries = {};
+        L.d_entry_piece = piece, L.tile_entry_nodes = entries_need, L.entries_made_for = s->d_meshes;
+    }
     return RBRT_OK;
 }
 
@@ -1567,7 +1623,7 @@
     return RBRT_OK;
 }
 
-rbrt_hip_scene::Lane::TileKey tile_key(const TraceParams& P, uint32_t list_mode) {
+rbrt_hip_scene::Lane::TileKey tile_key(const rbrt_hip_scene* s, const TraceParams& P, uint32_t list_mode) {
     rbrt_hip_scene::Lane::TileKey k;
     std::memset(&k, 0, sizeof(k));
     k.cam = P.cam, k.rank = P.tile_rank, k.world = P.tile_world, k.list_mode = list_mode, k.min_dist = P.min_dist;
@@ -1575,6 +1631,7 @@
     for (int c = 0; c < 3; ++c) k.lens_u[c] = P.lens_u[c], k.lens_v[c] = P.lens_v[c];
     k.shutter = P.shutter;
     for (int c = 0; c < 3; ++c) k.travel[c] = P.travel[c];
+    k.meshes = P.meshes, k.entries_mode = s->tile_entries;
     return k;
 }
 
@@ -1585,14 +1642,30 @@
     return S;
 }
 
-int fill_tile_set(rbrt_hip_scene::Lane::TileSet* S, const TraceParams& base, uint32_t list_mode, bool wide, hipStream_t cs) {
+uint32_t entry_meshes_in_range(const std::vector<const BvhNode4*>& trees, const BvhNode4* d_entries, size_t n_rows) {
+    uint32_t mask = 0;
+    for (uint32_t m = 0; m < trees.size() && m < kTileEntryMeshes; ++m) {
+        const uintptr_t rows = reinterpret_cast<uintptr_t>(d_entries), nodes = reinterpret_cast<uintptr_t>(trees[m]);
+        if (!nodes || rows <= nodes || (rows - nodes) % sizeof(BvhNode4) != 0) continue;
+        if ((rows - nodes) / sizeof(BvhNode4) + n_rows < (uint64_t(1) << 31)) mask |= 1u << m;
+    }
+    return mask;
+}
+
+int fill_tile_set(const rbrt_hip_scene* s, rbrt_hip_scene::Lane::TileSet* S, const TraceParams& base, uint32_t list_mode, bool wide, hipStream_t cs) {
     if (S->free_recorded) HIP_TRY(hipStreamWaitEvent(cs, S->ev_free, 0));
     if (S->key_valid) HIP_TRY(hipStreamWaitEvent(cs, S->ev_lists, 0));
     TraceParams P = base;
     P.tile_cull = S->d_cull, P.tile_lists = S->d_lists, P.tile_list_mode = list_mode, P.tile_lists_wide = wide ? 1u : 0u;
     HIP_TRY(launch_primary_cull(P, cs));
+    S->entry_meshes = 0u;
+    if (s->tile_entries != 0u && S->d_entries) {
+        P.tile_entries = S->d_entries;
+        HIP_TRY(launch_tile_entries(P, cs));
+        if (s->tile_entries == 1u) S->entry_meshes = S->entries_in_range;
+    }
     HIP_TRY(hipEventRecord(S->ev_lists, cs));
-    S->key = tile_key(P, list_mode), S->key_valid = true;
+    S->key = tile_key(s, P, list_mode), S->key_valid = true;
     return RBRT_OK;
 }
 
@@ -1601,9 +1674,9 @@
     for (uint32_t li = 0; li < c.depth; ++li) {
         rbrt_hip_scene::Lane& L = s->lanes[li];
         if (L.tiles[0].key_valid || L.tiles[1].key_valid) continue;
-        if (int rc = fill_tile_set(&L.tiles[0], P, mode, false, c.stream)) return rc;
+        if (int rc = fill_tile_set(s, &L.tiles[0], P, mode, false, c.stream)) return rc;
         if (li == s->next_lane % c.depth && iso_mode != mode)
-            if (int rc = fill_tile_set(&L.tiles[1], P, iso_mode, false, c.stream)) return rc;
+            if (int rc = fill_tile_set(s, &L.tiles[1], P, iso_mode, false, c.stream)) return rc;
     }
     return RBRT_OK;
 }
@@ -1620,7 +1693,7 @@
         TraceParams P = P_call;
         uint32_t lane_no = stats ? 0u : s->next_lane % c.depth;
         if (!stats && c.depth > 1 && c.tile_pass && !c.round && !s->streaming_hint && b == 0 && !c.busy_at_call) {
-            const auto want = tile_key(P, list_mode_for(false));
+            const auto want = tile_key(s, P, list_mode_for(false));
             for (uint32_t li = 0; li < c.depth; ++li)
                 if (find_tile_set(s->lanes[li], want)) lane_no = li;
         } else if (!stats) {
@@ -1666,12 +1739,12 @@
             if (piped) HIP_TRY(hipStreamWaitEvent(ts, c.round->ev_lists, 0));
         } else if (c.tile_pass) {
             const uint32_t list_mode = list_mode_for(overlapped && !stats);
-            S = find_tile_set(L, tile_key(P, list_mode));
+            S = find_tile_set(L, tile_key(s, P, list_mode));
             if (!S) {
                 S = L.tiles[0].last_used <= L.tiles[1].last_used ? &L.tiles[0] : &L.tiles[1];
                 if (overlapped)
                     if (int rc = ensure_prep_stream(s)) return rc;
-                if (int rc = fill_tile_set(S, P, list_mode, !overlapped, overlapped ? s->prep_stream : ts)) return rc;
+                if (int rc = fill_tile_set(s, S, P, list_mode, !overlapped, overlapped ? s->prep_stream : ts)) return rc;
                 if (s->trace_launches) std::fprintf(stderr, "[rbrt_hip] tile pass on the prep stream: lane %u set %d list_mode %u\n",
                                                     unsigned(&L - s->lanes.data()), int(S - L.tiles), list_mode);
             }
@@ -1680,6 +1753,8 @@
                 std::fprintf(stderr, "[rbrt_hip] t %.3f ms launch %llu lane %u %s grid list_mode %u set %d\n", now_s() * 1e3, (unsigned long long)s->launch_no,
                              unsigned(&L - s->lanes.data()), overlapped ? "half" : "full", S->key.list_mode, int(S - L.tiles));
             P.tile_cull = S->d_cull, P.tile_lists = S->d_lists, P.tile_list_mode = S->key.list_mode;
+            if (S->entry_meshes != 0u) P.tile_entries = S->d_entries, P.tile_entry_meshes = S->entry_meshes, P.meshes = S->d_entry_meshes;
+            s->last_entries = {S->d_entries, S->d_lists, S->entry_meshes, c.n_local, S->key.entries_mode != 0u && S->d_entries != nullptr};
             if (S->key.list_mode != 0u) P.tiles_reversed = 0u;
         }
         if (s->poison_samples) HIP_TRY(hipMemsetAsync(B.d_sample_buf, 0xFF, B.sample_buf_bytes, ts));
@@ -2035,6 +2110,39 @@
     return RBRT_OK;
 }
 
+int rbrt_hip_scene_set_tile_entries(rbrt_hip_scene_t* s, int mode) {
+    if (!s) return fail(RBRT_ERR_INVALID_ARG, "set_tile_entries: null scene");
+    if (mode < 0 || mode > 2) return fail(RBRT_ERR_INVALID_ARG, "set_tile_entries: mode must be 0 (off), 1 (on) or 2 (made, never used)");
+    std::lock_guard<std::mutex> watcher_lock(s->mu);
+    s->tile_entries = uint32_t(mode);
+    return RBRT_OK;
+}
+
+int rbrt_hip_debug_tile_entries(rbrt_hip_scene_t* s, rbrt_hip_tile_entries_info_t* info, uint32_t* out_tiles, size_t n_tiles, void* out_nodes,
+                                size_t n_nodes) {
+    if (!s || !info || (n_tiles != 0 && !out_tiles) || (n_nodes != 0 && !out_nodes))
+        return fail(RBRT_ERR_INVALID_ARG, "debug_tile_entries: null argument");
+    HIP_TRY(hipSetDevice(s->device));
+    std::lock_guard<std::mutex> watcher_lock(s->mu);
+    std::memset(info, 0, sizeof(*info));
+    const auto& le = s->last_entries;
+    if (!le.made) return RBRT_OK;
+    HIP_TRY(hipDeviceSynchronize());
+    uint32_t n_work = 0;
+    HIP_TRY(hipMemcpy(&n_work, le.d_lists, sizeof(n_work), hipMemcpyDeviceToHost));
+    info->made = 1u, info->n_work = n_work, info->n_meshes = std::min<uint32_t>(s->n_meshes, kTileEntryMeshes), info->used_meshes = le.entry_meshes;
+    const size_t nt = std::min<size_t>(n_tiles, n_work);
+    if (nt != 0) HIP_TRY(hipMemcpy(out_tiles, le.d_lists + kTileListHeader, nt * sizeof(uint32_t), hipMemcpyDeviceToHost));
+    for (uint32_t m = 0; m < info->n_meshes; ++m) {
+        const size_t at = size_t(m) * n_work;
+        if (at >= n_nodes) break;
+        const size_t nn = std::min<size_t>(n_nodes - at, n_work);
+        if (nn != 0)
+            HIP_TRY(hipMemcpy(static_cast<BvhNode4*>(out_nodes) + at, le.d_entries + size_t(m) * le.n_local, nn * sizeof(BvhNode4), hipMemcpyDeviceToHost));
+    }
+    return RBRT_OK;
+}
+
 int rbrt_hip_debug_short_masks(rbrt_hip_scene_t* s, uint64_t* out_masks, size_t n, size_t* n_chunks) {
     if (!s || !n_chunks || (n != 0 && !out_masks)) return fail(RBRT_ERR_INVALID_ARG, "debug_short_masks: null argument");
     HIP_TRY(hipSetDevice(s->device));
diff --git a/rbrt_amd/csrc/device_types.h b/rbrt_amd/csrc/device_types.h
--- a/rbrt_amd/csrc/device_types.h
+++ b/rbrt_amd/csrc/device_types.h
@@ -166,7 +166,10 @@
     uint32_t env_n;
     unsigned long long* short_masks;
     uint32_t pattern_dw;
-};
+    BvhNode4* tile_entries;
+    uint32_t tile_entry_meshes;
+};
+constexpr uint32_t kTileEntryMeshes = 7;
 
 struct ResolveParams {
     uint32_t width, height, tiles_x, n_tiles;
diff --git a/rbrt_amd/csrc/kernels.hip b/rbrt_amd/csrc/kernels.hip
--- a/rbrt_amd/csrc/kernels.hip
+++ b/rbrt_amd/csrc/kernels.hip
@@ -805,19 +805,38 @@
     }
 };
 
-constexpr int kCullBlock = 64;
-constexpr uint32_t kCullLanes = 4;
-__global__ __launch_bounds__(kCullBlock, 4) void primary_cull_kernel(const TraceParams P) {
-    const uint32_t cull_world = P.tile_world > 1u ? P.tile_world : 1u;
-    const uint32_t tile_local = (blockIdx.x * kCullBlock + threadIdx.x) / kCullLanes;
-    const uint32_t tile = tile_local * cull_world + (cull_world > 1u ? P.tile_rank : 0u);
-    const uint32_t quad_lane = threadIdx.x % kCullLanes, quad_shift = threadIdx.x & ~(kCullLanes - 1u);
-    if (tile >= P.n_tiles) return;
+struct TileReach {
+    D3 pos;
+    CullSlab cols, rows;
+    CullCone cone;
+    double w_dir, org_a;
+    __device__ __forceinline__ bool box_unreachable(D3 lo, D3 hi, double slack, double far) const {
+        const D3 q = 0.5 * (lo + hi) - pos;
+        const double l = dlen(q);
+        if (cone.misses((1.0 / l) * q, l, 0.5 * dlen(hi - lo) * 1.001 + slack + org_a, 1.0)) return true;
+        const double reach = slack + org_a + w_dir * (far + org_a);
+        for (uint32_t slab = 0; slab < 2u; ++slab) {
+            const CullSlab& sl = slab ? rows : cols;
+            bool pos_side = true, neg_side = true;
+            for (uint32_t k = 0; k < 8u; ++k) {
+                const D3 v = D3{k & 1u ? hi.x : lo.x, k & 2u ? hi.y : lo.y, k & 4u ? hi.z : lo.z} - pos;
+                const double g0 = ddot(sl.n_lo, v), g1 = ddot(sl.n_hi, v);
+                pos_side = pos_side && g0 > reach && g1 > reach;
+                neg_side = neg_side && g0 < -reach && g1 < -reach;
+            }
+            if (pos_side || neg_side) return true;
+        }
+        return false;
+    }
+};
+__device__ __forceinline__ TileReach tile_reach(const TraceParams& P, uint32_t tile) {
+    TileReach R;
     uint32_t ty, tx;
     tile_xy(tile, P.tiles_x, ty, tx);
     const rbrt_camera_t& c = P.cam;
     const uint32_t W = c.img_width_pix, H = c.img_height_pix;
-    const D3 pos = d3(c.position), right = d3(c.right), up = d3(c.up), ctr = d3(c.img_center_point);
+    R.pos = d3(c.position);
+    const D3 pos = R.pos, right = d3(c.right), up = d3(c.up), ctr = d3(c.img_center_point);
     const D3 a = ctr - pos;
     const double pad = 1e-3 + double(W > H ? W : H) * (1.0 / 4194304.0);
     const uint32_t c0 = tx * RBRT_TILE, r0 = ty * RBRT_TILE;
@@ -853,26 +872,68 @@
         org_a = lens_a + tl + 16.0 * (1.0 / 16777216.0) * (dlen(pos) + lens_a + tl);
         if (!(org_a == org_a)) angle = __builtin_nan("");
     }
-    CullSlab cols, rows;
-    cols.n_lo = unit_or_nan(dcross(a + (0.001 * cm0) * right, up));
-    cols.n_hi = unit_or_nan(dcross(a + (0.001 * cm1) * right, up));
-    rows.n_lo = unit_or_nan(dcross(a - (0.001 * rm0) * up, right));
-    rows.n_hi = unit_or_nan(dcross(a - (0.001 * rm1) * up, right));
-    CullCone cone;
-    cone.mid = unit_or_nan(a + (0.0005 * (cm0 + cm1)) * right - (0.0005 * (rm0 + rm1)) * up);
+    R.cols.n_lo = unit_or_nan(dcross(a + (0.001 * cm0) * right, up));
+    R.cols.n_hi = unit_or_nan(dcross(a + (0.001 * cm1) * right, up));
+    R.rows.n_lo = unit_or_nan(dcross(a - (0.001 * rm0) * up, right));
+    R.rows.n_hi = unit_or_nan(dcross(a - (0.001 * rm1) * up, right));
+    R.cone.mid = unit_or_nan(a + (0.0005 * (cm0 + cm1)) * right - (0.0005 * (rm0 + rm1)) * up);
     double rho = 0.0;
     for (uint32_t k = 0; k < 4u; ++k) {
         const D3 u = unit_or_nan(a + (0.001 * (k & 1u ? cm1 : cm0)) * right - (0.001 * (k & 2u ? rm1 : rm0)) * up);
-        cone.corner[k] = u;
-        const double t = angle_between(cone.mid, u);
+        R.cone.corner[k] = u;
+        const double t = angle_between(R.cone.mid, u);
         rho = t > rho || !(t == t) ? t : rho;
     }
-    const double w_dir = angle + lens_beta;
+    const double w_dir = R.w_dir = angle + lens_beta;
     rho += w_dir;
     if (!(rho < 1.5)) rho = __builtin_nan("");
-    cone.cos_rho = cos(rho), cone.sin_rho = sin(rho);
-    cone.cos_w = cos(w_dir), cone.sin_w = sin(w_dir);
-
+    R.cone.cos_rho = cos(rho), R.cone.sin_rho = sin(rho);
+    R.cone.cos_w = cos(w_dir), R.cone.sin_w = sin(w_dir);
+
+    R.org_a = org_a;
+    return R;
+}
+
+struct MeshReach {
+    double far, pad_base;
+    bool finite;
+};
+__device__ __forceinline__ MeshReach mesh_reach(const TileReach& R, const DevMesh& md) {
+    MeshReach M;
+    M.far = 0.0, M.finite = true;
+    for (uint32_t k = 0; k < 8u; ++k) {
+        const D3 q = D3{double(k & 1u ? md.bbox_hi[0] : md.bbox_lo[0]), double(k & 2u ? md.bbox_hi[1] : md.bbox_lo[1]),
+                        double(k & 4u ? md.bbox_hi[2] : md.bbox_lo[2])} - R.pos;
+        const double l = dlen(q);
+        M.finite = M.finite && l < 1e30;
+        M.far = l > M.far ? l : M.far;
+    }
+    const D3 mc = d3(md.center) - R.pos;
+    const double o_inf = fmax(fmax(fabs(R.pos.x), fabs(R.pos.y)), fabs(R.pos.z));
+    M.pad_base = 64.0 * (1.0 / 16777216.0) * (dlen(mc) + double(md.radius) + o_inf + R.org_a);
+    return M;
+}
+__device__ __forceinline__ uint32_t tree_box_state(const TileReach& R, const MeshReach& M, const BvhNode4& nd, uint32_t c, float eps_frac) {
+    if (nd.child[c] == kNoChild) return 0u;
+    const D3 lo = D3{double(nd.lo_x[c]), double(nd.lo_y[c]), double(nd.lo_z[c])};
+    const D3 hi = D3{double(nd.hi_x[c]), double(nd.hi_y[c]), double(nd.hi_z[c])};
+    if (!(dlen(lo - R.pos) < 1e30 && dlen(hi - R.pos) < 1e30)) return 2u;
+    return R.box_unreachable(lo, hi, M.pad_base * (double(nd.max_e12[c]) * 1.001 * double(eps_frac) + 1.0), M.far) ? 0u : 1u;
+}
+
+constexpr int kCullBlock = 64;
+constexpr uint32_t kCullLanes = 4;
+__global__ __launch_bounds__(kCullBlock, 4) void primary_cull_kernel(const TraceParams P) {
+    const uint32_t cull_world = P.tile_world > 1u ? P.tile_world : 1u;
+    const uint32_t tile_local = (blockIdx.x * kCullBlock + threadIdx.x) / kCullLanes;
+    const uint32_t tile = tile_local * cull_world + (cull_world > 1u ? P.tile_rank : 0u);
+    const uint32_t quad_lane = threadIdx.x % kCullLanes, quad_shift = threadIdx.x & ~(kCullLanes - 1u);
+    if (tile >= P.n_tiles) return;
+    const TileReach R = tile_reach(P, tile);
+    const D3 pos = R.pos;
+    const CullSlab &cols = R.cols, &rows = R.rows;
+    const CullCone& cone = R.cone;
+    const double w_dir = R.w_dir, org_a = R.org_a;
     const uint32_t n_elem = P.n_spheres + P.n_elem_tris;
     uint32_t word = 0;
     bool all = n_elem <= 24u && P.n_meshes <= 7u && P.n_elem_tris == 0u;
@@ -896,41 +957,14 @@
         if (out) word |= 1u << e;
         else all = false;
     }
-    const auto box_unreachable = [&](D3 lo, D3 hi, double slack, double far) -> bool {
-        const D3 q = 0.5 * (lo + hi) - pos;
-        const double l = dlen(q);
-        if (cone.misses((1.0 / l) * q, l, 0.5 * dlen(hi - lo) * 1.001 + slack + org_a, 1.0)) return true;
-        const double reach = slack + org_a + w_dir * (far + org_a);
-        for (uint32_t slab = 0; slab < 2u; ++slab) {
-            const CullSlab& sl = slab ? rows : cols;
-            bool pos_side = true, neg_side = true;
-            for (uint32_t k = 0; k < 8u; ++k) {
-                const D3 v = D3{k & 1u ? hi.x : lo.x, k & 2u ? hi.y : lo.y, k & 4u ? hi.z : lo.z} - pos;
-                const double g0 = ddot(sl.n_lo, v), g1 = ddot(sl.n_hi, v);
-                pos_side = pos_side && g0 > reach && g1 > reach;
-                neg_side = neg_side && g0 < -reach && g1 < -reach;
-            }
-            if (pos_side || neg_side) return true;
-        }
-        return false;
-    };
     for (uint32_t m = 0; m < P.n_meshes && m < 7u; ++m) {
         const DevMesh& md = P.meshes[m];
-        double far = 0.0;
-        bool finite = true;
-        for (uint32_t k = 0; k < 8u; ++k) {
-            const D3 q = D3{double(k & 1u ? md.bbox_hi[0] : md.bbox_lo[0]), double(k & 2u ? md.bbox_hi[1] : md.bbox_lo[1]),
-                            double(k & 4u ? md.bbox_hi[2] : md.bbox_lo[2])} - pos;
-            const double l = dlen(q);
-            finite = finite && l < 1e30;
-            far = l > far ? l : far;
-        }
+        const MeshReach M = mesh_reach(R, md);
+        const double far = M.far;
+        const bool finite = M.finite;
         const double slack = 16.0 * (1.0 / 16777216.0) * (far + org_a);
-        const bool out = finite && box_unreachable(d3(md.bbox_lo), d3(md.bbox_hi), slack, far);
+        const bool out = finite && R.box_unreachable(d3(md.bbox_lo), d3(md.bbox_hi), slack, far);
         if (out) word |= 1u << (24u + m);
-        const D3 mc = d3(md.center) - pos;
-        const double o_inf = fmax(fmax(fabs(pos.x), fabs(pos.y)), fabs(pos.z));
-        const double pad_base = 64.0 * (1.0 / 16777216.0) * (dlen(mc) + double(md.radius) + o_inf + org_a);
         bool mesh_free = out;
         if (!out && all && finite && md.n_nodes != 0u) {
             constexpr uint32_t kCullLevels = 6;
@@ -943,14 +977,8 @@
                 const BvhNode4& nd = md.nodes[e >> 3];
                 const uint32_t c = quad_lane;
                 const int32_t link = nd.child[c];
-                uint32_t state = 0u;
-                if (link != kNoChild) {
-                    const D3 lo = D3{double(nd.lo_x[c]), double(nd.lo_y[c]), double(nd.lo_z[c])};
-                    const D3 hi = D3{double(nd.hi_x[c]), double(nd.hi_y[c]), double(nd.hi_z[c])};
-                    if (!(dlen(lo - pos) < 1e30 && dlen(hi - pos) < 1e30)) state = 2u;
-                    else if (!box_unreachable(lo, hi, pad_base * (double(nd.max_e12[c]) * 1.001 * double(P.eps_frac) + 1.0), far))
-                        state = (link >= 0 && (e & 7u) + 1u < kCullLevels) ? 1u : 2u;
-                }
+                uint32_t state = tree_box_state(R, M, nd, c, P.eps_frac);
+                if (state == 1u && !(link >= 0 && (e & 7u) + 1u < kCullLevels)) state = 2u;
                 const uint32_t open = uint32_t(__builtin_amdgcn_ballot_w64(state == 1u) >> quad_shift) & 15u;
                 const uint32_t stay = uint32_t(__builtin_amdgcn_ballot_w64(state == 2u) >> quad_shift) & 15u;
                 if (stay != 0u) mesh_free = false;
@@ -1049,8 +1077,81 @@
     if (t == kListBlock - 1) {
         P.tile_lists[0] = n_work;
         P.tile_lists[1] = n - n_work;
-        P.tile_lists[2] = n_light, P.tile_lists[3] = 0u;
-    }
+        P.tile_lists[2] = n_light, P.tile_lists[3] = n_work != 0u ? uint32_t(0x100000000ull / (uint64_t(n_work) * 64u)) : 0u;
+    }
+}
+
+constexpr uint32_t kEntryLevels = 6;
+__global__ __launch_bounds__(kCullBlock, 4) void tile_entries_kernel(const TraceParams P) {
+    const uint32_t widx = (blockIdx.x * kCullBlock + threadIdx.x) / kCullLanes;
+    const uint32_t quad_lane = threadIdx.x % kCullLanes, quad_shift = threadIdx.x & ~(kCullLanes - 1u);
+    if (widx >= P.tile_lists[0]) return;
+    const uint32_t tile_local = P.tile_lists[kTileListHeader + widx];
+    const uint32_t tile = tile_local * (P.tile_world > 1u ? P.tile_world : 1u) + (P.tile_world > 1u ? P.tile_rank : 0u);
+    const uint32_t cull_word = P.tile_cull[tile];
+    const TileReach R = tile_reach(P, tile);
+    const auto quad = [&](bool p) -> uint32_t { return uint32_t(__builtin_amdgcn_ballot_w64(p) >> quad_shift) & 15u; };
+    for (uint32_t m = 0; m < P.n_meshes && m < kTileEntryMeshes; ++m) {
+        const DevMesh& md = P.meshes[m];
+        BvhNode4* const out = P.tile_entries + (size_t(m) * P.n_local_tiles + widx);
+        const auto write_slot = [&](const BvhNode4* src, uint32_t c) {
+            const float inf = __builtin_inff();
+            out->lo_x[quad_lane] = src ? src->lo_x[c] : inf, out->lo_y[quad_lane] = src ? src->lo_y[c] : inf;
+            out->lo_z[quad_lane] = src ? src->lo_z[c] : inf, out->hi_x[quad_lane] = src ? src->hi_x[c] : -inf;
+            out->hi_y[quad_lane] = src ? src->hi_y[c] : -inf, out->hi_z[quad_lane] = src ? src->hi_z[c] : -inf;
+            out->child[quad_lane] = src ? src->child[c] : kNoChild, out->max_e12[quad_lane] = src ? src->max_e12[c] : 0.0f;
+        };
+        if (md.n_nodes == 0u || ((cull_word >> (24u + m)) & 1u)) {
+            write_slot(nullptr, 0u);
+            continue;
+        }
+        const MeshReach M = mesh_reach(R, md);
+        bool m_valid = false, m_shut = false;
+        uint32_t m_node = 0u, m_slot = 0u, m_level = 0u;
+        int32_t m_link = kNoChild;
+        bool root_copy = !M.finite;
+        uint32_t open_node = 0u, open_level = 0u, open_from = 4u;
+        while (!root_copy) {
+            const uint32_t state = tree_box_state(R, M, md.nodes[open_node], quad_lane, P.eps_frac);
+            if (quad(state == 2u) != 0u) {
+                root_copy = true;
+                break;
+            }
+            const uint32_t reach = quad(state == 1u), valid = quad(m_valid);
+            const uint32_t others = open_from < 4u ? valid & ~(1u << open_from) : valid;
+            if (uint32_t(__popc(others)) + uint32_t(__popc(reach)) > 4u) {
+                if (quad_lane == open_from) m_shut = true;
+            } else {
+                const uint32_t free_lanes = ~others & 15u, k = uint32_t(__popc(free_lanes & ((1u << quad_lane) - 1u)));
+                if (quad_lane == open_from) m_valid = false;
+                if (((free_lanes >> quad_lane) & 1u) && k < uint32_t(__popc(reach))) {
+                    uint32_t r = reach;
+                    for (uint32_t j = 0; j < k; ++j) r &= r - 1u;
+                    m_valid = true, m_shut = false;
+                    m_node = open_node, m_slot = uint32_t(__ffs(int(r))) - 1u, m_level = open_level + 1u;
+                    m_link = md.nodes[open_node].child[m_slot];
+                }
+            }
+            const bool cand = m_valid && !m_shut && m_link >= 0 && m_level < kEntryLevels;
+            uint32_t best = cand ? m_level : 99u;
+            best = min(best, uint32_t(__shfl_xor(int(best), 1, 64)));
+            best = min(best, uint32_t(__shfl_xor(int(best), 2, 64)));
+            const uint32_t pick = quad(cand && m_level == best);
+            if (pick == 0u) break;
+            open_from = uint32_t(__ffs(int(pick))) - 1u;
+            open_node = uint32_t(__shfl(m_link, int(quad_shift + open_from), 64));
+            open_level = best;
+        }
+        if (root_copy) write_slot(&md.nodes[0], quad_lane);
+        else write_slot(m_valid ? &md.nodes[m_node] : nullptr, m_slot);
+    }
+}
+
+hipError_t launch_tile_entries(const TraceParams& P, hipStream_t stream) {
+    if (!P.tile_entries || !P.tile_lists || !P.tile_cull || P.n_local_tiles == 0u || P.n_meshes == 0u) return hipSuccess;
+    const size_t threads = size_t(P.n_local_tiles) * kCullLanes;
+    hipLaunchKernelGGL(tile_entries_kernel, dim3(uint32_t((threads + kCullBlock - 1) / kCullBlock)), dim3(kCullBlock), 0, stream, P);
+    return hipGetLastError();
 }
 
 __host__ __device__ inline uint32_t local_tiles_of(uint32_t n_tiles, uint32_t rank, uint32_t world) {
```

Measured after the change: 12080 Mray-samples/s, median of 6. No clear change (+0.8%).
